# shibiaowan/SHARP

Measured on AMD Instinct MI355X. Metric: cells/sec end-to-end SHARP (fixed genes, n.RP); ARI vs reference labels, higher is better.
Workload: dtype f64

## Files before the change

include/sharp_hip.h:

```cpp
#ifndef SHARP_HIP_H
#define SHARP_HIP_H

#ifdef __cplusplus
extern "C" {
#endif

#define SHARP_OK 0
#define SHARP_ERR 1
#define SHARP_ERR_ARG 2
#define SHARP_ERR_NO_DEVICE 3
#define SHARP_WARN_RANGE 16
#define SHARP_WARN_NA_VOTE 32

const char *sharp_last_error(void);
int sharp_version(void);
int sharp_device_count(int *count);
int sharp_init(int device);
int sharp_shutdown(void);
int sharp_synchronize(void);
int sharp_reload_options(void);
int sharp_profile_enable(int on);
int sharp_profile_reset(void);
int sharp_profile_get(const char *name, double *total_ms, long long *launches);
int sharp_profile_dump(char *buf, int buflen);

int sharp_projector_create(int m, int p, int K, const double *seeds, int *handle);
int sharp_projector_destroy(int handle);
int sharp_projector_info(int handle, int *m, int *p, int *K, long long *nnz_total);
int sharp_projector_triplets(int handle, int k, int *gene, int *col, signed char *sign, long long *nnz);

int sharp_project(int proj, const double *X, int m, int n, long long ld, int log_flag, double *E);
int sharp_project_dev(int proj, const float *dX, int m, int n, long long ld, int log_flag,
                      double *dE, long long ldE);
int sharp_project_dev64(int proj, const double *dX, int m, int n, long long ld, int log_flag,
                        double *dE, long long ldE);

int sharp_get_opt_hclust(const double *mat, int n, int p, int hmethod, int N_cluster, int minN, int maxN,
                         double sil_thre, double height_Ntimes, int *f, int *v, double *msil, double *CHind,
                         double *maxsil, double *height, int *optN, int *nk, int *branch);

#define SHARP_DECISION_COLS 14
int sharp_decision_log(int enable);
int sharp_last_decisions(double *rows , int cap_rows, int *n_rows);

int sharp_getrowColor(const double *E, int n, int p, int hmethod, int indN_cluster, int minN, int maxN,
                      double sil_thre, double height_Ntimes, int *rowColor, double *maxsil);

int sharp_wMetaC(const int *nC, int N, int C, int hmethod, int enN_cluster, int minN, int maxN, double sil_thre,
                 double height_Ntimes, int *finalC, double *x0, int *ncl, double *w1_out, double *S_out, int *allC_out,
                 int *tf_out);

int sharp_sMetaC(const int *labels, const double *sE1, long long n, int p, int hmethod, int finalN_cluster, int minN,
                 int maxN, double sil_thre, double height_Ntimes, int *finalColor, int *tf_out, int *nC_out);

int sharp_SHARP_dev(const float *dX, int m, long long n, long long ld, int ensize_K, int reduced_ndim, int base_ncells,
                    int partition_ncells, int hmethod, int N_cluster, int enpN_cluster, int indN_cluster, int minN, int maxN,
                    double sil_thre, double height_Ntimes, int log_flag, int projector, double rN_seed, int *pred,
                    int *n_pred, double *viE, double *x0, int x0_cap_cols, int *x0_cols, int *p_used, int *K_used, int *path);
int sharp_SHARP_dev64(const double *dX, int m, long long n, long long ld, int ensize_K, int reduced_ndim, int base_ncells,
                      int partition_ncells, int hmethod, int N_cluster, int enpN_cluster, int indN_cluster, int minN, int maxN,
                      double sil_thre, double height_Ntimes, int log_flag, int projector, double rN_seed, int *pred,
                      int *n_pred, double *viE, double *x0, int x0_cap_cols, int *x0_cols, int *p_used, int *K_used, int *path);
int sharp_SHARP(const double *X, int m, long long n, long long ld, int ensize_K, int reduced_ndim, int base_ncells,
                int partition_ncells, int hmethod, int N_cluster, int enpN_cluster, int indN_cluster, int minN, int maxN,
                double sil_thre, double height_Ntimes, int log_flag, int projector, double rN_seed, int *pred,
                int *n_pred, double *viE, double *x0, int x0_cap_cols, int *x0_cols, int *p_used, int *K_used, int *path);

int sharp_x_storage(void);
int sharp_x_wire(void);

int sharp_last_rpinfo(int *n, int *K, int *p, int *enrp, double *indE);

int sharp_trim(void);

int sharp_csc_to_dense_dev(const int *colptr, const int *rowidx, const double *val, int m, long long n, float *dX, long long ld);
int sharp_csc_packed_expand_dev(const long long *d_colptr, const void *d_idx, int idx_bits, const void *d_val, int val_bits, int m,
                                long long n, void *dX, long long ld, int dx_is_f64);
int sharp_SHARP_csc(const int *colptr, const int *rowidx, const double *val, int m, long long n, int ensize_K, int reduced_ndim,
                    int base_ncells, int partition_ncells, int hmethod, int N_cluster, int enpN_cluster, int indN_cluster,
                    int minN, int maxN, double sil_thre, double height_Ntimes, int log_flag, int projector, double rN_seed,
                    int *pred, int *n_pred, double *viE, double *x0, int x0_cap_cols, int *x0_cols, int *p_used, int *K_used,
                    int *path);

int sharp_SHARP_unlimited_dev(const float *const *dX_blocks, const long long *ncb, const long long *ldb, int nblocks, int m,
// ... 181 lines not shown
int sharp_expr_stats_sub_csc(const int *const *colptr, const int *const *rowidx, const double *const *val, const long long *ncb, int nblocks,
                             int m, double normalize_total, int log1p, double *mean, double *var, long long *nnz, double *cell_sum,
                             const int *genes, int n_genes);
int sharp_expr_pca_transform_sub_csc(const int *const *colptr, const int *const *rowidx, const double *const *val, const long long *ncb,
                                     int nblocks, int m, double normalize_total, int log1p, const double *loadings, const double *center,
                                     const double *scale, int n_components, double *scores, const int *genes, int n_genes);
int sharp_expr_hvg_csc(const int *const *colptr, const int *const *rowidx, const double *const *val, const long long *ncb, int nblocks, int m,
                       int n_top_genes, double span, double *means, double *variances, double *variances_expected, double *variances_norm,
                       int *rank, int *highly_variable, int *genes, int *n_selected, int *q, int *degree_counts);
int sharp_hvg_loess(const double *x, const double *y, int npts, double span, double *fit, double *bandwidth, int *degree);

int sharp_harmony(const double *Z, long long n, int d, const int *batch, int n_batches, int n_clusters, double sigma, double theta, double lam,
                  int max_iter, int max_iter_cluster, int n_blocks, double epsilon_cluster, double epsilon_harmony, int init_iter, long long seed,
                  double *Z_corr, double *Y, double *objective, int *rounds, int *n_iter, int *converged, double *R);
int sharp_harmony_assign(const double *Zhat, const double *Y, const int *batch, const double *P, long long n, int d, int K, int B, long long i0,
                         long long i1, double sigma, int argmax, double *R, int *a);
int sharp_harmony_sums(const double *R, const double *X, const int *batch, long long n, int d, int K, int B, long long seed, int n_blocks, double *O,
                       double *S);
int sharp_harmony_correct(const double *Z, const double *R, const int *batch, const double *W, long long n, int d, int K, int B, double *Z_corr);
int sharp_harmony_ridge(const double *N, const double *S, int B, int K, int d, double lam, double *W);
int sharp_harmony_caps(int *slab, int *lds_tile);

int sharp_doublet_plan(long long n, double sim_doublet_ratio, int n_neighbors, long long *n_sim, int *n_neighbors_out, int *k_adj);
int sharp_doublet_pairs(long long n, long long n_sim, long long seed, long long *parents);
int sharp_doublet_synth_csc(const int *const *colptr, const int *const *rowidx, const double *const *val, const long long *ncb, int nblocks,
                            int m, const long long *parents, long long n_sim, int max_doublets_per_slab, long long capacity,
                            long long *colptr_out, int *rowidx_out, double *val_out, double *cell_sum_out);
int sharp_doublet_project_csc(const int *const *colptr, const int *const *rowidx, const double *const *val, const long long *ncb, int nblocks,
                              int m, const long long *parents, long long n_sim, double normalize_total, int log1p, const double *loadings,
                              const double *center, const double *scale, int n_components, const int *genes, int n_genes,
                              int max_doublets_per_slab, double *scores);
int sharp_doublet_neighbor_counts(const int *index, long long rows, int K, long long n_obs, int *counts);
int sharp_doublet_score_table(int k_adj, double r, double expected_doublet_rate, double *table);
int sharp_doublet_threshold(const double *scores_obs, long long n, const double *scores_sim, long long n_sim, double threshold_in,
                            double *threshold, int *found, int *predicted, double *rates, int *passes);
int sharp_scrublet_csc(const int *const *colptr, const int *const *rowidx, const double *const *val, const long long *ncb, int nblocks, int m,
                       double sim_doublet_ratio, double expected_doublet_rate, int n_neighbors, int n_prin_comps, int n_top_genes,
                       const int *genes, int n_genes, const double *fit_scores, const double *fit_loadings, const double *fit_center,
                       const double *fit_scale, double normalize_total, int log1p, int scale, double threshold, int nn_method,
                       const double *nn_args, long long seed, int max_doublets_per_slab, double *doublet_scores, double *doublet_scores_sim,
                       int *predicted, double *threshold_out, int *threshold_found, double *rates, int *n_neighbors_out, int *k_adj_out,
                       long long *parents, int *genes_out, int *n_genes_out, int *neighbor_counts, double *sim_pca);

int sharp_synth_fill_dev(unsigned seed, int m, long long cell0, int ncell, int G, int nmark,
                         float *dX, long long ld);
int sharp_synth_labels(unsigned seed, long long cell0, int ncell, int G, int *labels);

int sharp_gemm_tn_f64(const double *At, const double *Bt, double *C, int M, int N, int K, int epilogue, int symmetric, int fast);

int sharp_gemm_tn_f64_batch(int count, const int *M, const int *N, const int *K, const double *At, const double *Bt, int epilogue,
                            int symmetric, int fast, int nn_square, int want_nn, int polite, int ldc_pad, double *C, double *nn);
int sharp_row_prep_batch(int count, const int *n, const int *p, const long long *lds, const int *mode, const double *src,
                         int all_feature_rows, double *Cr, double *Ct, double *nrm, double *D);

int sharp_get_opt_hclust_batch(int count, const int *n, const int *p, const int *kind, const int *hmethod, const int *N_cluster,
                               const int *minN, const int *maxN, const double *sil_thre, const double *height_Ntimes, const double *mats,
                               int want_v, int nested, int *f, int *v, double *msil, double *CHind, double *height, int *optN, int *nk,
                               int *branch, int *rc, int *sequential);
int sharp_hclust_batch_plan(int *rows, int cap_rows, int *n_rows);

int sharp_wMetaC_batch(int count, const int *N, const int *C, const int *hmethod, const int *enN_cluster, const int *minN, const int *maxN,
                       const double *sil_thre, const double *height_Ntimes, const int *labels, const long long *cap, int *rc, int *allC,
                       int *ncl, int *finalC, double *w1, double *S, int *tf, double *x0);
int sharp_cluster_means(const double *E, long long ld, int n, int p, const int *uid, int nC, double *means, long long cap);
int sharp_ensemble_mean(const double *E, long long ldE, int n, int p, int K, double *viE, long long cap);

int sharp_dev_alloc(long long bytes, void **dptr);
int sharp_dev_free(void *dptr);
int sharp_dev_upload(void *dptr, const void *host, long long bytes);
int sharp_dev_download(void *host, const void *dptr, long long bytes);

void sharp_C_init(int *device, int *status);
void sharp_C_shutdown(int *status);
void sharp_C_trim(int *status);
void sharp_C_reload_options(int *status);
void sharp_C_device_count(int *count, int *status);
void sharp_C_last_error(char **msg, int *len);
void sharp_C_projector_create(int *m, int *p, int *K, double *seeds, int *handle, int *status);
void sharp_C_projector_destroy(int *handle, int *status);
void sharp_C_projector_triplets(int *handle, int *k, int *gene, int *col, int *sign, double *nnz, int *status);
void sharp_C_project(int *proj, double *X, int *m, int *n, int *log_flag, double *E, int *status);
void sharp_C_get_opt_hclust(double *mat, int *n, int *p, int *hmethod, int *N_cluster, int *minN, int *maxN, double *sil_thre,
                            double *height_Ntimes, int *flashmark, int *f, int *v, double *msil, double *CHind, double *maxsil,
                            double *height, int *optN, int *nk, int *branch, int *want, int *status);
void sharp_C_getrowColor(double *E, int *n, int *p, int *hmethod, int *indN_cluster, int *minN, int *maxN, double *sil_thre,
                         double *height_Ntimes, int *flashmark, int *rowColor, double *maxsil, int *status);
void sharp_C_wMetaC(int *nC, int *N, int *C, int *hmethod, int *enN_cluster, int *minN, int *maxN, double *sil_thre,
                    double *height_Ntimes, int *finalC, double *x0, int *ncl, int *want, int *status);
void sharp_C_sMetaC(int *labels, double *sE1, double *n, int *p, int *hmethod, int *finalN_cluster, int *minN, int *maxN,
                    double *sil_thre, double *height_Ntimes, int *finalColor, int *tf, int *nC, int *status);
void sharp_C_SHARP(double *X, int *m, double *n, int *ensize_K, int *reduced_ndim, int *base_ncells, int *partition_ncells, int *hmethod,
                   int *N_cluster, int *enpN_cluster, int *indN_cluster, int *minN, int *maxN, double *sil_thre, double *height_Ntimes,
                   int *flashmark, int *log_flag, int *projector, double *rN_seed, int *pred, double *viE, double *x0, int *x0_cap_cols,
                   int *info, int *want, int *status);
void sharp_C_SHARP_csc(int *colptr, int *rowidx, double *val, int *m, double *n, int *ensize_K, int *reduced_ndim, int *base_ncells,
                       int *partition_ncells, int *hmethod, int *N_cluster, int *enpN_cluster, int *indN_cluster, int *minN, int *maxN,
                       double *sil_thre, double *height_Ntimes, int *flashmark, int *log_flag, int *projector, double *rN_seed, int *pred,
                       double *viE, double *x0, int *x0_cap_cols, int *info, int *want, int *status);
void sharp_C_last_rpinfo(int *dims, int *enrp, double *indE, int *want, int *status);
void sharp_C_SHARP_unlimited(double *Xcat, int *nblocks, double *ncb, int *m, int *ensize_K, int *N_cluster, int *minN, int *maxN,
                             double *rN_seed, int *pred, double *viE, int *info, int *want, int *status);
void sharp_C_unlimited_view_dim(int *kdim, int *status);
void sharp_C_decision_log(int *enable, int *status);
void sharp_C_last_decisions(double *rows, int *cap_rows, int *n_rows, int *status);
void sharp_C_SHARP_unlimited_multi(double *Xcat, int *nblocks, double *ncb, int *m, int *ensize_K, int *N_cluster, int *minN, int *maxN,
                                   double *rN_seed, int *devices, int *ndevices, int *pred, double *viE, int *info, int *want, int *status);
// ... 103 lines not shown
```

sharp_amd/_abi.py:

```python
import ctypes as C

RETURN = {"i": C.c_int, "v": None, "s": C.c_char_p}
ARGUMENT = {"i": C.c_int, "u": C.c_uint, "l": C.c_longlong, "d": C.c_double, "p": C.c_void_p}

SIGNATURES = {
    "sharp_last_error": "s:",
    "sharp_version": "i:",
    "sharp_device_count": "i:p",
    "sharp_init": "i:i",
    "sharp_shutdown": "i:",
    "sharp_synchronize": "i:",
    "sharp_reload_options": "i:",
    "sharp_profile_enable": "i:i",
    "sharp_profile_reset": "i:",
    "sharp_profile_get": "i:ppp",
    "sharp_profile_dump": "i:pi",
    "sharp_projector_create": "i:iiipp",
    "sharp_projector_destroy": "i:i",
    "sharp_projector_info": "i:ipppp",
    "sharp_projector_triplets": "i:iipppp",
    "sharp_project": "i:ipiilip",
    "sharp_project_dev": "i:ipiilipl",
    "sharp_project_dev64": "i:ipiilipl",
    "sharp_get_opt_hclust": "i:piiiiiiddppppppppp",
    "sharp_decision_log": "i:i",
    "sharp_last_decisions": "i:pip",
    "sharp_getrowColor": "i:piiiiiiddpp",
    "sharp_wMetaC": "i:piiiiiiddppppppp",
    "sharp_sMetaC": "i:ppliiiiiddppp",
    "sharp_SHARP_dev": "i:pilliiiiiiiiiiddiidppppipppp",
    "sharp_SHARP_dev64": "i:pilliiiiiiiiiiddiidppppipppp",
    "sharp_SHARP": "i:pilliiiiiiiiiiddiidppppipppp",
    "sharp_x_storage": "i:",
    "sharp_x_wire": "i:",
    "sharp_last_rpinfo": "i:ppppp",
    "sharp_trim": "i:",
    "sharp_csc_to_dense_dev": "i:pppilpl",
    "sharp_csc_packed_expand_dev": "i:ppipiilpli",
    "sharp_SHARP_csc": "i:pppiliiiiiiiiiiddiidppppipppp",
    "sharp_SHARP_unlimited_dev": "i:pppiiiiiidppp",
    "sharp_SHARP_unlimited": "i:ppiiiiiidppp",
    "sharp_SHARP_unlimited_multi": "i:ppiiiiiidpipppp",
    "sharp_SHARP_unlimited_csc": "i:ppppiiiiiidpppp",
    "sharp_SHARP_unlimited_csc_multi": "i:ppppiiiiiidpipppp",
    "sharp_SHARP_unlimited_multi_dev": "i:pppppiiiiiidpipppp",
    "sharp_multi_timeline": "i:pip",
    "sharp_SHARP_unlimited_view": "i:ppiiiiiidpppp",
    "sharp_SHARP_unlimited_view_dev": "i:pppiiiiiidpppp",
    "sharp_unlimited_view_dim": "i:i",
    "sharp_SHARP_unlimited_viewk_dev": "i:pppiiiiiidpppip",
    "sharp_unlimited_block_dev": "i:pilliiidpppip",
    "sharp_unlimited_block_dev64": "i:pilliiidpppip",
    "sharp_unlimited_blocks_dev": "i:ppppiiiiidpppip",
    "sharp_SHARP_unlimited2": "i:ppiiiiiiiiiiiddidpppp",
    "sharp_SHARP_unlimited2_dev": "i:pppiiiiiiiiiiiddidpppp",
    "sharp_unlimited_block_view_dev": "i:pilliiidipppipp",
    "sharp_unlimited_block_viewk_dev": "i:pilliiidipppipidp",
    "sharp_unlimited_block_viewk_dev64": "i:pilliiidipppipidp",
    "sharp_unlimited_merge": "i:ppiiliiipp",
    "sharp_unlimited_next_block_dev": "i:pll",
    "sharp_marker_genes": "i:pillpidip",
    "sharp_marker_genes_dev": "i:pillpidip",
    "sharp_marker_genes_blocks_dev": "i:pppiipidip",
    "sharp_marker_genes_blocks_csc": "i:ppppiipidip",
    "sharp_tsne": "i:pliliiiiiiiddiiiddddpdppp",
    "sharp_tsne_prepare": "i:pliliiiiipp",
    "sharp_tsne_knn": "i:plilipp",
    "sharp_tsne_affinities": "i:plildlpppp",
    "sharp_tsne_gradient": "i:ppplipp",
    "sharp_tsne_bh": "i:pliliiiiiiiddiiiddddpdppp",
    "sharp_tsne_gradient_bh": "i:ppplipdpp",
    "sharp_tsne_neighbors": "i:ppliiiiddiiiddddpdppp",
    "sharp_tsne_dist": "i:piiiddiiiddddpdppp",
    "sharp_tsne_knn_dist": "i:piipp",
# ... 14 lines not shown
    "sharp_umap_transform": "i:ipllididdlppp",
    "sharp_knn_cross": "i:iplliipp",
    "sharp_umap_transform_weights": "i:ipplippp",
    "sharp_umap_transform_epochs": "i:ipplipiiididdl",
    "sharp_dist": "i:piilidp",
    "sharp_hclust_dist": "i:piippp",
    "sharp_hclust": "i:piilidippp",
    "sharp_cutree": "i:pipip",
    "sharp_silhouette_dist": "i:pipipp",
    "sharp_silhouette": "i:plilidpipp",
    "sharp_calinski_harabasz": "i:plilpiip",
    "sharp_neighbor_ranks": "i:plilipip",
    "sharp_louvain_graph": "i:ppplddiiidpipppppp",
    "sharp_louvain_neighbors": "i:ppliiddiiidpipppppp",
    "sharp_louvain_quantise": "i:ppplppp",
    "sharp_louvain_move": "i:ppplpddiip",
    "sharp_louvain_modularity": "i:pppplpdp",
    "sharp_louvain_aggregate": "i:ppplppppppp",
    "sharp_louvain_row_caps": "i:pp",
    "sharp_snn_graph": "i:plidlppppp",
    "sharp_snn_row_caps": "i:pp",
    "sharp_louvain_snn": "i:plidddiiidpipppppp",
    "sharp_expr_pca_csc": "i:ppppiiiiidiilpppppppp",
    "sharp_expr_stats_csc": "i:ppppiidipppp",
    "sharp_expr_pca_transform_csc": "i:ppppiidipppip",
    "sharp_expr_spmm_cells": "i:ppppiidiipip",
    "sharp_expr_spmm_genes": "i:ppppiidiipip",
    "sharp_expr_orth": "i:plip",
    "sharp_expr_row_caps": "i:pp",
    "sharp_expr_pca_sub_csc": "i:ppppiiiiidiilpppppppppi",
    "sharp_expr_stats_sub_csc": "i:ppppiidipppppi",
    "sharp_expr_pca_transform_sub_csc": "i:ppppiidipppippi",
    "sharp_expr_hvg_csc": "i:ppppiiidpppppppppp",
    "sharp_hvg_loess": "i:ppidppp",
    "sharp_harmony": "i:plipiidddiiiddilppppppp",
    "sharp_harmony_assign": "i:ppppliiilldipp",
    "sharp_harmony_sums": "i:pppliiilipp",
    "sharp_harmony_correct": "i:ppppliiip",
    "sharp_harmony_ridge": "i:ppiiidp",
    "sharp_harmony_caps": "i:pp",
    "sharp_doublet_plan": "i:ldippp",
    "sharp_doublet_pairs": "i:lllp",
    "sharp_doublet_synth_csc": "i:ppppiiplilpppp",
    "sharp_doublet_project_csc": "i:ppppiipldipppipiip",
    "sharp_doublet_neighbor_counts": "i:plilp",
    "sharp_doublet_score_table": "i:iddp",
    "sharp_doublet_threshold": "i:plpldppppp",
    "sharp_scrublet_csc": "i:ppppiiddiiipippppdiidiplippppppppppppp",
    "sharp_synth_fill_dev": "i:uiliiipl",
    "sharp_synth_labels": "i:uliip",
    "sharp_gemm_tn_f64": "i:pppiiiiii",
    "sharp_gemm_tn_f64_batch": "i:ipppppiiiiiiipp",
    "sharp_row_prep_batch": "i:ipppppipppp",
    "sharp_get_opt_hclust_batch": "i:ippppppppppiipppppppppp",
    "sharp_hclust_batch_plan": "i:pip",
    "sharp_wMetaC_batch": "i:ipppppppppppppppppp",
    "sharp_cluster_means": "i:pliipipl",
    "sharp_ensemble_mean": "i:pliiipl",
    "sharp_dev_alloc": "i:lp",
    "sharp_dev_free": "i:p",
    "sharp_dev_upload": "i:ppl",
    "sharp_dev_download": "i:ppl",
    "sharp_C_init": "v:pp",
    "sharp_C_shutdown": "v:p",
    "sharp_C_trim": "v:p",
    "sharp_C_reload_options": "v:p",
    "sharp_C_device_count": "v:pp",
    "sharp_C_last_error": "v:pp",
    "sharp_C_projector_create": "v:pppppp",
    "sharp_C_projector_destroy": "v:pp",
    "sharp_C_projector_triplets": "v:ppppppp",
    "sharp_C_project": "v:ppppppp",
    "sharp_C_get_opt_hclust": "v:ppppppppppppppppppppp",
    "sharp_C_getrowColor": "v:ppppppppppppp",
    "sharp_C_wMetaC": "v:pppppppppppppp",
    "sharp_C_sMetaC": "v:pppppppppppppp",
    "sharp_C_SHARP": "v:pppppppppppppppppppppppppp",
    "sharp_C_SHARP_csc": "v:pppppppppppppppppppppppppppp",
    "sharp_C_last_rpinfo": "v:ppppp",
    "sharp_C_SHARP_unlimited": "v:pppppppppppppp",
    "sharp_C_unlimited_view_dim": "v:pp",
    "sharp_C_decision_log": "v:pp",
    "sharp_C_last_decisions": "v:pppp",
    "sharp_C_SHARP_unlimited_multi": "v:pppppppppppppppp",
    "sharp_C_SHARP_unlimited_csc": "v:pppppppppppppppppp",
    "sharp_C_SHARP_unlimited2": "v:pppppppppppppppppppppp",
    "sharp_C_unlimited_merge": "v:ppppppppppp",
    "sharp_C_marker_genes": "v:ppppppppp",
    "sharp_C_tsne": "v:pppppppppppppppppppppppppp",
    "sharp_C_tsne_neighbors": "v:ppppppppppppppppppppppp",
    "sharp_C_tsne_dist": "v:pppppppppppppppppppp",
    "sharp_C_tsne_knn": "v:ppppppp",
    "sharp_C_knn_descent": "v:ppppppppppppp",
    "sharp_C_tsne_bh": "v:pppppppppppppppppppppppppp",
    "sharp_C_umap": "v:pppppppppppppppppppppp",
    "sharp_C_umap_neighbors": "v:pppppppppppppppppp",
    "sharp_C_umap_ab": "v:ppppp",
    "sharp_C_umap_model_create": "v:ppppppppppp",
    "sharp_C_umap_model_free": "v:pp",
    "sharp_C_umap_transform": "v:ppppppppppppppp",
    "sharp_C_umap_components": "v:pppppp",
    "sharp_C_umap_spectral": "v:pppppppppppppp",
    "sharp_C_umap_init_info": "v:pppppp",
    "sharp_C_dist": "v:ppppppp",
    "sharp_C_hclust_dist": "v:ppppppp",
    "sharp_C_hclust": "v:pppppppppp",
# ... 20 lines not shown
```

sharp_amd/csrc/common.hpp:

```cpp
#pragma once
#include <hip/hip_runtime.h>
#include <functional>

#include <cstdint>
#include <cstdio>
#include <map>
#include <stdexcept>
#include <string>
#include <vector>

#include "../../include/sharp_hip.h"

namespace sharp {

struct Error : std::runtime_error {
    int code;
    Error(int c, const std::string &m) : std::runtime_error(m), code(c) {}
};

void set_error(const std::string &msg);

#define SHARP_HIP_CHECK(expr)                                                                   \
    do {                                                                                        \
        hipError_t _e = (expr);                                                                 \
// ... 8 lines not shown
    } while (0)

#define SHARP_API_BEGIN try {
#define SHARP_API_END                                        \
    }                                                        \
    catch (const sharp::Error &e) {                          \
        sharp::set_error(e.what());                          \
        return e.code;                                       \
    }                                                        \
    catch (const std::exception &e) {                        \
        sharp::set_error(e.what());                          \
        return SHARP_ERR;                                    \
    }                                                        \
    return SHARP_OK;
inline int api_guarded(const std::function<void()> &step) {
    SHARP_API_BEGIN
    step();
    SHARP_API_END
}

struct XRef {
    const void *p = nullptr;
    bool f64 = false;
    int log_fix_bits = 44;
    XRef() = default;
    XRef(const float *q) : p(q), f64(false) {}
    XRef(const double *q) : p(q), f64(true) {}
    const float *f32() const { return static_cast<const float *>(p); }
    const double *d64() const { return static_cast<const double *>(p); }
};

struct Knobs {
    bool rp_dual = true;
    int rp_two_streams = -1;
    int rp_ahead = 2;
    int rp_chunk = 0;
    int rp_cp_wgs = 8;
    int rp_ap_wgs = 4;
    int rp_kernel = 0;
    int rp_pc_wgs = 2;
    int rp_pc_shape = 0;
    int x_storage = 0;
    bool block_prefetch = true;
    bool unlimited_batch = true;
    int unlimited_window_mb = 0;
    int ml_min_levels = 0;
    bool hc_mono = false, hc_seq = false;
    int hc_split = -1;
    int hc_ranges = 0, hc_wpt = 0, hc_finish_at = 15, hc_chunk = 0;
    int tail_threads = 4;
    bool tail_priority = true;
    bool dist_i8 = false;
    bool stats_sums = true;
    bool stats_lane = true;
    bool hc_tri = false;
    bool hc_prep_early = true;
    bool hc_pipe = true;
    bool mean_early = false;
    int gemm_slice = 8;
    bool proj_host = false;
    int hc_front = 0;
    bool hc_nn_gemm = true;
    bool hc_half = false;
    int host_threads = 0;
    int upload_threads = 0;
    std::vector<int> devices;
    int front_overlap = 0;
    int hc_first_chunk = 0;
    int host_group = 1;
    bool decision_log = false;
    bool free_later = true;
    bool step_marks = false;
    int rp_shape = 0;
};
const Knobs &knobs();
void reload_knobs();
void step_mark(const char *label, int id = -1);
void step_marks_dump();
#ifdef SHARP_LAB
inline const char *lab_env(const char *name) { return getenv(name); }
#endif

struct KernelStat {
    double ms = 0;
    long long launches = 0;
};

struct Ctx {
    bool ready = false;
    int device = -1;
    hipStream_t stream = nullptr;
    hipStream_t main_stream = nullptr;
    int rp_wgs_cap = 0;
    bool polite = false;
    hipStream_t stream2 = nullptr;
    std::vector<hipStream_t> aux;
    hipStream_t aux_stream(int i);
    int num_cu = 256;
    size_t lds_per_block = 65536;
    bool profiling = false;
    std::map<std::string, KernelStat> stats;
    struct Pending { hipEvent_t a, b; std::string name; hipStream_t st; };
    std::vector<Pending> pending;
    std::vector<hipEvent_t> event_pool;
    hipEvent_t get_event();
    void resolve_pending();
// ... 117 lines not shown
```

sharp_amd/csrc/driver.hip:

```cpp
#include <algorithm>
#include <cmath>
#include <cstring>
#include <numeric>
#include <random>
#include <thread>
#include <condition_variable>
#include <future>
#include <mutex>
#include <vector>

#include "driver.hpp"
#include "meta.hpp"
#include "projector.hpp"
#include "rrng.hpp"
#include "upload.hpp"

namespace sharp {

struct SharpOut {
    std::vector<int> pred;
    int n_pred = 0;
    struct View {
        double *p = nullptr;
        const double *staged = nullptr;
        hipEvent_t staged_done = nullptr;
        void download(double *h, size_t count) const {
            if (staged) {
                SHARP_HIP_CHECK(hipEventSynchronize(staged_done));
                const size_t piece = (count + 15) / 16;
                const double *src = staged;
                host_parallel_for(16, 16, [&](int t) {
                    const size_t lo = std::min(count, piece * static_cast<size_t>(t)), hi = std::min(count, lo + piece);
                    if (hi > lo) memcpy(h + lo, src + lo, (hi - lo) * sizeof(double));
                });
                return;
            }
            SHARP_HIP_CHECK(hipMemcpyAsync(h, p, count * sizeof(double), hipMemcpyDeviceToHost, ctx().stream));
            SHARP_HIP_CHECK(hipStreamSynchronize(ctx().stream));
        }
    } viE;
    std::vector<double> x0;
    int x0_cols = 0;
    int p = 0, K = 0, path = 0, rc = 0;
};

namespace {

struct DriverWs {
    DevBuf<double> E, Eb, viE_sh, viE_out;
    DevBuf<int> pos, posb;
    hipEvent_t mean_go = nullptr, mean_done = nullptr;
    hipStream_t mean_stream = nullptr;
    DevBuf<double> Ebatch;
    DevBuf<int> posbatch;
    DevBuf<double> fold_means, block_means;
    double *view_pinned = nullptr;
    size_t view_pinned_n = 0;
    hipEvent_t view_done = nullptr;
    std::vector<hipEvent_t> front_ev;
};
DriverWs &dws() { return per_slot<DriverWs>(); }

struct LastSmall { bool valid = false; int n = 0, K = 0, p = 0; long long ldE = 0; std::vector<int> enrp; };
LastSmall &last_small() { return per_slot<LastSmall>(); }

void merge_small(std::vector<int> &lab) {
    int mx = 0;
    for (int v : lab) mx = std::max(mx, v);
    std::vector<long long> cnt(mx + 1, 0);
    for (int v : lab) ++cnt[v];
    int mn = -1;
    for (int q = 1; q <= mx; ++q) if (cnt[q] > 0 && cnt[q] < 10) { mn = q; break; }
    if (mn >= 0) for (int &v : lab) if (cnt[v] < 10) v = mn;
}
int relabel_first(std::vector<int> &lab) {
    int mx = 0;
    for (int v : lab) mx = std::max(mx, v);
    std::vector<int> map(mx + 1, 0);
    int k = 0;
    for (int &v : lab) { if (!map[v]) map[v] = ++k; v = map[v]; }
    return k;
}

std::shared_ptr<Projector> projector_for(const SharpArgs &a, int m, int p, int K, const std::function<void()> *after_draw = nullptr) {
    if (a.projector) {
        auto pr = get_projector(a.projector);
        SHARP_REQUIRE(pr->m == m && pr->p == p && pr->K >= K, "rM does not match the data (genes, reduced.ndim, ensize.K)");
        return pr;
    }
    std::vector<double> seeds(K);
    for (int k = 0; k < K; ++k) seeds[k] = (a.rN_seed == 0.5) ? 0.5 : 50 + a.rN_seed + (k + 1);
    return build_projector(m, p, K, seeds.data(), after_draw);
}

__host__ __device__ inline double r_round1(double x) {
    if (!(x == x) || x == 0.0 || x - x != 0.0) return x;
    const double sgn = x < 0.0 ? -1.0 : 1.0;
    x = x < 0.0 ? -x : x;
    if (x >= 1e14) return sgn * x;
    const double x10 = 10.0 * x, i10 = floor(x10), xd = i10 / 10.0, xu = ceil(x10) / 10.0;
    const double du = xu - x, dd = x - xd;
    return sgn * ((dd < du || (dd == du && fmod(i10, 2.0) == 0.0)) ? xd : xu);
}
__global__ void round1_kernel(double *__restrict__ E, long long count) {
    for (long long q = blockIdx.x * static_cast<long long>(blockDim.x) + threadIdx.x; q < count; q += static_cast<long long>(gridDim.x) * blockDim.x)
        E[q] = r_round1(E[q]);
}
// ... 13 lines not shown
void sharp_small_dev(XRef dX, int m, int n, long long ld, const SharpArgs &a, int K, int p, HcParams base, SharpOut &out) {
    last_small().valid = false;
    auto pr = projector_for(a, m, p, K);
    const long long ldE = static_cast<long long>(pr->K) * p;
    DevBuf<double> &E = dws().E;
    E.ensure(static_cast<size_t>(n) * ldE);
    project_dev(*pr, dX, m, n, ld, a.flag, E.p, ldE, nullptr);
    std::vector<HcTask> tasks(K);
    HcParams bp = base; bp.N_cluster = a.indN;
    for (int k = 0; k < K; ++k) {
        tasks[k].d_mat = E.p + static_cast<long long>(k) * p; tasks[k].ld = ldE; tasks[k].n = n; tasks[k].p = p; tasks[k].prm = bp;
        tasks[k].prm.dec_level = 0; tasks[k].prm.dec_k = k;
    }
    std::vector<HcResult> hr;
    get_opt_hclust_batch(tasks, false, hr);
    std::vector<int> enrp(static_cast<size_t>(n) * K);
    for (int k = 0; k < K; ++k) { out.rc |= hr[k].rc; for (int i = 0; i < n; ++i) enrp[static_cast<size_t>(k) * n + i] = colour_of(hr[k].f[i]); }
    { LastSmall &L = last_small(); L.n = n; L.K = K; L.p = p; L.ldE = ldE; L.enrp = enrp; }
    WmTask wt; wt.nC = enrp.data(); wt.N = n; wt.C = K; wt.prm = base; wt.prm.N_cluster = a.N_cluster;
    wt.prm.dec_level = 1;
    std::vector<WmTask> wts{wt};
    std::vector<WmResult> wr;
    wmetac_batch(wts, a.want_x0, false, wr);
    out.rc |= wr[0].rc;
    out.pred = wr[0].finalC;
    if (a.want_viE || true) { dws().viE_out.ensure(static_cast<size_t>(n) * p); out.viE.p = dws().viE_out.p; ensemble_mean_dev(E.p, ldE, n, p, K, out.viE.p); }
    if (a.N_cluster <= 0 && n > 10000) merge_small(out.pred);
    out.n_pred = relabel_first(out.pred);
    if (a.want_x0) { out.x0 = wr[0].x0; out.x0_cols = wr[0].ncl; }
    stream_sync();
    last_small().valid = true;
}

static std::vector<int> fold_starts(int n, int ng) {
    const int T = (n + ng - 1) / ng;
    std::vector<int> st(T + 1, 0);
    if (T == 1) { st[1] = n; return st; }
    for (int t = 0; t < T - 2; ++t) st[t + 1] = (t + 1) * ng;
    const int nt = n - (T - 2) * ng;
    st[T - 1] = (T - 2) * ng + std::min(nt / 2, ng);
    st[T] = n;
    return st;
}

struct LargeFront {
    XRef dX; int m = 0, n = 0; long long ld = 0; int K = 0, p = 0, ng = 0, flag = 0, projector = 0; double rN_seed = 0; bool fpart = false;
    HcParams bp;
    bool shuffle = false;
    std::vector<int> reind, fst, pos;
    int T = 0;
    std::shared_ptr<Projector> pr;
    long long ldE = 0;
    double *E = nullptr; int *dpos = nullptr;
    std::vector<HcTask> tasks;
    std::shared_ptr<HcPrefetch> hc;
    bool matches(XRef X, int m_, int n_, long long ld_, int K_, int p_, int ng_, const SharpArgs &a, const HcParams &b) const {
        return dX.p == X.p && dX.f64 == X.f64 && m == m_ && n == n_ && ld == ld_ && K == K_ && p == p_ && ng == ng_ && flag == a.flag &&
               projector == a.projector && rN_seed == a.rN_seed && fpart == a.fpart && bp.hmethod == b.hmethod && bp.N_cluster == b.N_cluster &&
               bp.minN == b.minN && bp.maxN == b.maxN && bp.sil_thre == b.sil_thre && bp.height_Ntimes == b.height_Ntimes;
    }
};
namespace {
struct PendingFront { std::unique_ptr<LargeFront> f; hipStream_t stream = nullptr; hipEvent_t main_done = nullptr; int parity = 0;
                      unsigned long long born = 0, calls = 0; };
PendingFront &pending_front() { return per_slot<PendingFront>(); }
}

void drain_side_streams() {
    PendingFront &PF = pending_front();
    if (PF.stream) (void)hipStreamSynchronize(PF.stream);
    if (dws().mean_stream) (void)hipStreamSynchronize(dws().mean_stream);
}
void drop_pending_front() {
    PendingFront &PF = pending_front();
    if (PF.stream) (void)hipStreamSynchronize(PF.stream);
    PF.f.reset();
}

struct Shuffle { std::vector<int> reind, pos; };
static Shuffle make_shuffle(int n, bool random_seed) {
    Shuffle S;
    RRng rng(random_seed ? static_cast<uint32_t>(std::random_device{}()) : 50u);
    S.reind = rng.permutation(n);
    S.pos.assign(n, 0);
    for (int i = 0; i < n; ++i) S.pos[S.reind[i] - 1] = i;
    return S;
}
namespace {
struct ShuffleAhead { int n = 0; std::future<Shuffle> fut; };
ShuffleAhead &shuffle_ahead_slot() { return per_slot<ShuffleAhead>(); }
}
void shuffle_ahead(long long n, double rN_seed) {
    ShuffleAhead &H = shuffle_ahead_slot();
    H.n = 0; H.fut = std::future<Shuffle>();
    if (n >= 100000 || n < 5000 || rN_seed == 0.5) return;
    H.n = static_cast<int>(n);
    H.fut = std::async(std::launch::async, make_shuffle, static_cast<int>(n), false);
}

static void large_front(LargeFront &F, const SharpArgs &a, bool ahead, double *E_into = nullptr, int *pos_into = nullptr,
                        const Shuffle *same_size = nullptr) {
    const int n = F.n, m = F.m, K = F.K, p = F.p;
    F.shuffle = n < 100000;
    std::vector<int> &pos = F.pos;
    std::future<Shuffle> shuf;
    if (F.shuffle) {
        ShuffleAhead &H = shuffle_ahead_slot();
        if (same_size && a.rN_seed != 0.5 && static_cast<int>(same_size->pos.size()) == n) { F.reind = same_size->reind; pos = same_size->pos; }
        else if (H.n == n && H.fut.valid() && a.rN_seed != 0.5) { shuf = std::move(H.fut); H.n = 0; }
        else shuf = std::async(std::launch::async, make_shuffle, n, a.rN_seed == 0.5);
    } else pos.assign(n, 0);
    F.fst = fold_starts(n, F.ng);
    F.T = static_cast<int>(F.fst.size()) - 1;
    unsigned ahead_tok = 0u;
    const bool may_go_ahead = !a.projector && !ahead && knobs().rp_ahead > 0;
    const std::function<void()> start_compaction = [&] { if (may_go_ahead && !ahead_tok) ahead_tok = rp_compact_ahead(F.dX, m, n, F.ld, a.flag); };
    if (knobs().rp_ahead >= 2) start_compaction();
    { HostTimer ht("projector_build"); F.pr = projector_for(a, m, p, K, &start_compaction); }
    F.ldE = static_cast<long long>(F.pr->K) * p;
    if (shuf.valid()) { Shuffle S = shuf.get(); F.reind = std::move(S.reind); pos = std::move(S.pos); }
    if (E_into) {
        F.E = E_into; F.dpos = F.shuffle ? pos_into : nullptr;
        if (F.shuffle) SHARP_HIP_CHECK(hipMemcpyAsync(pos_into, pos.data(), static_cast<size_t>(n) * sizeof(int), hipMemcpyHostToDevice, ctx().stream));
    } else {
        DevBuf<double> &E = ahead ? dws().Eb : dws().E;
        { HostTimer ht("alloc_E"); E.ensure(static_cast<size_t>(n) * F.ldE); }
        DevBuf<int> &dpos = ahead ? dws().posb : dws().pos;
        if (F.shuffle) { dpos.ensure(n); dpos.upload(pos.data(), n); }
        F.E = E.p; F.dpos = F.shuffle ? dpos.p : nullptr;
    }
    project_dev(*F.pr, F.dX, m, n, F.ld, a.flag, F.E, F.ldE, F.dpos, ahead_tok);
    if (a.fpart) {
        Ctx &c = ctx();
        hipLaunchKernelGGL(round1_kernel, dim3(c.num_cu * 8), dim3(256), 0, c.stream, F.E, static_cast<long long>(n) * F.ldE);
        launch_check("round1_kernel");
    }
    F.tasks.assign(static_cast<size_t>(K) * F.T, HcTask());
    for (int k = 0; k < K; ++k)
        for (int t = 0; t < F.T; ++t) {
            HcTask &tk = F.tasks[static_cast<size_t>(k) * F.T + t];
            tk.d_mat = F.E + static_cast<long long>(F.fst[t]) * F.ldE + static_cast<long long>(k) * p;
            tk.ld = F.ldE; tk.n = F.fst[t + 1] - F.fst[t]; tk.p = p; tk.prm = F.bp;
            tk.prm.dec_level = 0; tk.prm.dec_k = k; tk.prm.dec_fold = t;
        }
}

static void enqueue_ensemble_mean(const double *E, long long ldE, int n, int p, int K, double *viE_sh, hipEvent_t after) {
    Ctx &c = ctx();
    hipEvent_t &mean_done = dws().mean_done;
    hipStream_t &ms = dws().mean_stream;
    if (!mean_done) {
        SHARP_HIP_CHECK(hipEventCreateWithFlags(&mean_done, hipEventDisableTiming));
        SHARP_HIP_CHECK(hipEventCreateWithFlags(&dws().mean_go, hipEventDisableTiming));
        int lo = 0, hi = 0;
        SHARP_HIP_CHECK(hipDeviceGetStreamPriorityRange(&lo, &hi));
        SHARP_HIP_CHECK(hipStreamCreateWithPriority(&ms, hipStreamNonBlocking, hi));
    }
    SHARP_HIP_CHECK(hipEventRecord(dws().mean_go, c.stream));
    SHARP_HIP_CHECK(hipStreamWaitEvent(ms, dws().mean_go, 0));
    if (after) SHARP_HIP_CHECK(hipStreamWaitEvent(ms, after, 0));
    {
        StreamScope scope(ms);
        ensemble_mean_dev(E, ldE, n, p, K, viE_sh);
    }
    SHARP_HIP_CHECK(hipEventRecord(mean_done, ms));
}

static void large_tail(const LargeFront &F, const SharpArgs &a, int K, int p, const HcParams &base, const HcResult *hr, SharpOut &out) {
    const int n = F.n, T = F.T;
    const bool shuffle = F.shuffle;
    const std::vector<int> &reind = F.reind, &fst = F.fst;
    const long long ldE = F.ldE;
    struct { double *p; } E{F.E};
    struct { int *p; } dpos{F.dpos};
    DevBuf<double> &viE_sh = dws().viE_sh;
    viE_sh.ensure(static_cast<size_t>(n) * p);
    hipEvent_t &mean_done = dws().mean_done;
    if (!hc_after_last_agglomeration_fired()) enqueue_ensemble_mean(E.p, ldE, n, p, K, viE_sh.p, nullptr);
    bool view_sent = false;
    if (a.view_to_host && !a.fpart) {
        DriverWs &W = dws();
        const size_t cnt = static_cast<size_t>(n) * p;
        if (W.view_pinned_n < cnt) {
            if (W.view_pinned) (void)hipHostFree(W.view_pinned);
            W.view_pinned = nullptr; W.view_pinned_n = 0;
            SHARP_HIP_CHECK(hipHostMalloc(reinterpret_cast<void **>(&W.view_pinned), cnt * sizeof(double), hipHostMallocDefault));
            W.view_pinned_n = cnt;
        }
        if (!W.view_done) SHARP_HIP_CHECK(hipEventCreateWithFlags(&W.view_done, hipEventDisableTiming));
        W.viE_out.ensure(cnt);
        {
            StreamScope scope(W.mean_stream);
            if (shuffle) {
                hipLaunchKernelGGL(gather_rows_kernel, dim3(ctx().num_cu * 8), dim3(256), 0, W.mean_stream, viE_sh.p, dpos.p, static_cast<long long>(n), p, W.viE_out.p);
                launch_check("gather_rows_kernel");
            } else {
                SHARP_HIP_CHECK(hipMemcpyAsync(W.viE_out.p, viE_sh.p, cnt * 8, hipMemcpyDeviceToDevice, W.mean_stream));
            }
            SHARP_HIP_CHECK(hipMemcpyAsync(W.view_pinned, W.viE_out.p, cnt * 8, hipMemcpyDeviceToHost, W.mean_stream));
        }
        SHARP_HIP_CHECK(hipEventRecord(W.view_done, W.mean_stream));
        out.viE.p = W.viE_out.p; out.viE.staged = W.view_pinned; out.viE.staged_done = W.view_done;
        view_sent = true;
    }
    std::vector<std::vector<int>> enrp(T);
    for (int q = 0; q < K * T; ++q) out.rc |= hr[q].rc;
    {
    HostTimer ht("tail_enrp");
    host_parallel_for(T, 16, [&](int t) {
        const int nt = fst[t + 1] - fst[t];
        enrp[t].resize(static_cast<size_t>(nt) * K);
        for (int k = 0; k < K; ++k) {
            const HcResult &r = hr[static_cast<size_t>(k) * T + t];
            for (int i = 0; i < nt; ++i) enrp[t][static_cast<size_t>(k) * nt + i] = colour_of(r.f[i]);
        }
    });
    }
    std::vector<WmTask> wts(T);
    for (int t = 0; t < T; ++t) {
        wts[t].nC = enrp[t].data(); wts[t].N = fst[t + 1] - fst[t]; wts[t].C = K;
        wts[t].prm = base; wts[t].prm.N_cluster = a.enpN;
        wts[t].prm.dec_level = 1; wts[t].prm.dec_fold = t;
    }
    std::vector<WmResult> wr;
    { HostTimer ht("wmetac_total"); wmetac_batch(wts, a.want_x0, false, wr); }
    step_mark("  tail: per-fold wMetaC done, folds", T);
    SHARP_HIP_CHECK(hipStreamWaitEvent(ctx().stream, mean_done, 0));
    std::vector<int> Slab(n);
    std::vector<int> stf;
    std::vector<int> uid(n);
    int nCu = 0;
// ... 49 lines not shown
        out.x0.assign(static_cast<size_t>(n) * sn, 0.0);
        out.x0_cols = sn;
        for (int t = 0; t < T; ++t) {
            const int nt = fst[t + 1] - fst[t], ncl = wr[t].ncl;
            for (int q = 0; q < ncl; ++q) {
                const int dstc = stf[col0[t] + q] - 1;
                for (int i = 0; i < nt; ++i) {
                    const int cell = shuffle ? reind[fst[t] + i] - 1 : fst[t] + i;
                    out.x0[static_cast<size_t>(dstc) * n + cell] += wr[t].x0[static_cast<size_t>(q) * nt + i];
                }
            }
        }
    }
    if (!view_sent) {
        dws().viE_out.ensure(static_cast<size_t>(n) * p); out.viE.p = dws().viE_out.p;
        if (shuffle) {
            Ctx &c = ctx();
            hipLaunchKernelGGL(gather_rows_kernel, dim3(c.num_cu * 8), dim3(256), 0, c.stream, viE_sh.p, dpos.p, static_cast<long long>(n), p, out.viE.p);
            launch_check("gather_rows_kernel");
        } else {
            SHARP_HIP_CHECK(hipMemcpyAsync(out.viE.p, viE_sh.p, static_cast<size_t>(n) * p * 8, hipMemcpyDeviceToDevice, ctx().stream));
        }
    }
    if (a.N_cluster <= 0 && n > 10000) merge_small(out.pred);
    out.n_pred = relabel_first(out.pred);
    stream_sync();
}

static void sharp_large_dev_body(XRef dX, int m, int n, long long ld, const SharpArgs &a, int K, int p, int ng, HcParams base, SharpOut &out);
void sharp_large_dev(XRef dX, int m, int n, long long ld, const SharpArgs &a, int K, int p, int ng, HcParams base, SharpOut &out) {
    try {
        sharp_large_dev_body(dX, m, n, ld, a, K, p, ng, base, out);
    } catch (...) {
        drop_pending_front();
        rp_compact_ahead_drop();
        if (ctx_unchecked().stream2) (void)hipStreamSynchronize(ctx_unchecked().stream2);
        if (ctx_unchecked().stream) (void)hipStreamSynchronize(ctx_unchecked().stream);
        throw;
    }
}
static void sharp_large_dev_body(XRef dX, int m, int n, long long ld, const SharpArgs &a, int K, int p, int ng, HcParams base, SharpOut &out) {
    HostTimer ht_all("sharp_large_total");
    last_small().valid = false;
    HcParams bp = base; bp.N_cluster = a.indN;
    if (a.fpart) bp.maxN = 40;
    std::unique_ptr<LargeFront> Fp;
    PendingFront &PF = pending_front();
    const unsigned long long call_no = ++PF.calls;
    if (PF.f) {
        if (PF.born + 1 == call_no && PF.f->matches(dX, m, n, ld, K, p, ng, a, bp)) {
            Fp = std::move(PF.f);
            std::swap(dws().E, dws().Eb);
            std::swap(dws().pos, dws().posb);
        } else {
            SHARP_HIP_CHECK(hipStreamSynchronize(PF.stream));
            PF.f.reset();
        }
    }
    if (!Fp) {
        Fp.reset(new LargeFront);
        Fp->dX = dX; Fp->m = m; Fp->n = n; Fp->ld = ld; Fp->K = K; Fp->p = p; Fp->ng = ng; Fp->flag = a.flag; Fp->projector = a.projector;
        Fp->rN_seed = a.rN_seed; Fp->fpart = a.fpart; Fp->bp = bp;
        large_front(*Fp, a, false);
    }
    LargeFront &F = *Fp;
    hipEvent_t after_agglo = nullptr;
    if (F.hc && a.next_dX.p) { HostTimer ht("base_clustering_total"); after_agglo = hc_prefetch_agglomerate(*F.hc); }
    if (a.next_dX.p && a.projector && knobs().block_prefetch) {
        const int nn = static_cast<int>(a.next_n);
        const int Tn = (nn + ng - 1) / ng;
        if (a.next_n >= 5000 && a.next_n < (1LL << 31) && static_cast<long long>(K) * Tn <= ctx().num_cu && Tn > 1) {
            std::unique_ptr<LargeFront> N(new LargeFront);
            N->dX = a.next_dX; N->m = m; N->n = nn; N->ld = a.next_ld; N->K = K; N->p = p; N->ng = ng; N->flag = a.flag;
            N->projector = a.projector; N->rN_seed = a.rN_seed; N->fpart = a.fpart; N->bp = bp;
            if (a.maxN <= 0 && !a.fpart) N->bp.maxN = std::max(40, (nn + 4999) / 5000);
            try {
            if (!PF.stream) {
                int lo = 0, hi = 0;
                SHARP_HIP_CHECK(hipDeviceGetStreamPriorityRange(&lo, &hi));
                SHARP_HIP_CHECK(hipStreamCreateWithPriority(&PF.stream, hipStreamNonBlocking, lo));
            }
            {
                if (!F.hc) {
                    if (!PF.main_done) SHARP_HIP_CHECK(hipEventCreateWithFlags(&PF.main_done, hipEventDisableTiming));
                    SHARP_HIP_CHECK(hipEventRecord(PF.main_done, ctx().stream));
                    SHARP_HIP_CHECK(hipStreamWaitEvent(PF.stream, PF.main_done, 0));
                }
                StreamScope scope(PF.stream);
                struct Polite { Polite() { ctx().polite = true; } ~Polite() { ctx_unchecked().polite = false; } } polite;
                if (after_agglo) SHARP_HIP_CHECK(hipStreamWaitEvent(PF.stream, after_agglo, 0));
                large_front(*N, a, true);
                if (hc_prefetch_possible(N->tasks)) N->hc = hc_prefetch_begin(N->tasks, PF.parity ^= 1);
            }
            if (N->hc) { PF.f = std::move(N); PF.born = call_no; }
            else SHARP_HIP_CHECK(hipStreamSynchronize(PF.stream));
            } catch (...) {
                if (PF.stream) (void)hipStreamSynchronize(PF.stream);
                (void)hipGetLastError();
                PF.f.reset();
            }
        }
    }
    std::vector<HcResult> hr;
    {
        HostTimer ht("base_clustering_total");
        if (F.hc) { hc_set_after_last_agglomeration(nullptr); hc_prefetch_stamp_block(*F.hc, a.block); hc_prefetch_finish(*F.hc, false, hr); }
        else {
            dws().viE_sh.ensure(static_cast<size_t>(n) * p);
            const double *Ep = F.E;
            const long long ldEp = F.ldE;
            double *vsh = dws().viE_sh.p;
            if (knobs().mean_early) hc_set_after_last_agglomeration([=](hipEvent_t ev) { enqueue_ensemble_mean(Ep, ldEp, n, p, K, vsh, ev); });
            else hc_set_after_last_agglomeration(nullptr);
            for (HcTask &tk : F.tasks) tk.prm.dec_block = a.block;
            try { get_opt_hclust_batch(F.tasks, false, hr); } catch (...) { hc_set_after_last_agglomeration(nullptr); throw; }
        }
    }
    large_tail(F, a, K, p, base, hr.data(), out);
    hc_set_after_last_agglomeration(nullptr);
}

void sharp_front_dev(XRef dX, int m, long long n_, long long ld, SharpArgs a, SharpOut &out) {
    SHARP_REQUIRE(dX.p, "No expression data is provided!");
    SHARP_REQUIRE(n_ >= 3 && n_ < (1LL << 31) && m >= 2, "SHARP: need at least 3 cells and 2 genes");
    const int n = static_cast<int>(n_);
    if (a.rN_seed != 0.5) SHARP_REQUIRE(std::fmod(a.rN_seed, 1.0) == 0.0, "The rN.seed should be an integer!");
    int p = a.reduced_ndim > 0 ? a.reduced_ndim : static_cast<int>(std::ceil(std::log2(static_cast<double>(n)) / (0.2 * 0.2)));
    int base_ncells = a.base_ncells > 0 ? a.base_ncells : 5000;
    int part = a.partition_ncells > 0 ? a.partition_ncells : 2000;
    HcParams base;
    base.hmethod = a.hmethod > 0 ? a.hmethod : 1;
    base.minN = a.minN > 0 ? a.minN : 2;
    base.maxN = a.maxN > 0 ? a.maxN : std::max(40, (n + 4999) / 5000);
    base.sil_thre = a.sil_thre >= 0 ? a.sil_thre : 0.35;
    base.height_Ntimes = a.height_Ntimes > 0 ? a.height_Ntimes : 2.0;
    base.dec_block = a.block;
    int K = a.K;
    if (a.N_cluster > 0 && n < base_ncells) {
        a.indN = a.N_cluster;
        base_ncells = (n + 1) / 2;
        part = (n + 1) / 2;
        if (K <= 0) K = 15;
    }
    if (a.fpart) {
        if (K <= 0) K = 5;
        SHARP_REQUIRE(part >= 3 && part <= kHcMaxN, "partition.ncells must be between 3 and 16384");
        out.path = 1;
        sharp_large_dev(dX, m, n, ld, a, K, p, part, base, out);
    } else if (n < base_ncells) {
        if (K <= 0) K = 15;
        SHARP_REQUIRE(n <= kHcMaxN, "SHARP_small: more than 16384 cells in one unpartitioned clustering task");
        out.path = 0;
        sharp_small_dev(dX, m, n, ld, a, K, p, base, out);
    } else {
        if (K <= 0) K = 5;
        SHARP_REQUIRE(part >= 3 && part <= kHcMaxN, "partition.ncells must be between 3 and 16384");
        out.path = 1;
        sharp_large_dev(dX, m, n, ld, a, K, p, part, base, out);
    }
    out.p = p; out.K = K;
}

struct ViewProj { std::shared_ptr<Projector> pr; int p = 0, kdim = 0; double seed = 0; DevBuf<double> out, pad; };

static void unlimited_block_summary(const SharpOut &o, long long nb, int p, BlockTable &t, double *viE_host, const ViewCall &view) {
// ... 90 lines not shown
            SHARP_HIP_CHECK(hipStreamSynchronize(ctx().stream));
            ctx().resolve_pending();
        } catch (...) {
            Ctx &hc = ctx_unchecked();
            if (hc.stream) (void)hipStreamSynchronize(hc.stream);
            if (hc.stream2) (void)hipStreamSynchronize(hc.stream2);
            try { drain_side_streams(); } catch (...) {}
            std::lock_guard<std::mutex> lk(mu);
            if (!err) err = std::current_exception();
        }
    }
    void may_run(int r) {
        { std::lock_guard<std::mutex> lk(mu); ready = r; }
        cv.notify_all();
    }
    void finish() {
        { std::lock_guard<std::mutex> lk(mu); stop = true; }
        cv.notify_all();
        for (std::thread &t : helpers) if (t.joinable()) t.join();
    }
    void join(std::exception_ptr window_err) {
        finish();
        if (prof) {
            for (int s : tslot) {
                bind_slot(s);
                std::map<std::string, KernelStat> ts;
                ts.swap(ctx_unchecked().stats);
                bind_slot(owner);
                for (const auto &kv : ts) { KernelStat &d = mc.stats[kv.first]; d.ms += kv.second.ms; d.launches += kv.second.launches; }
            }
        }
        if (window_err) std::rethrow_exception(window_err);
        if (err) std::rethrow_exception(err);
    }
};
}

void unlimited_batch_window(const XRef *dX, const long long *ncb, const long long *ldb, int b0, int b1, int m, int p, int proj, int K,
                            double rN_seed, double *const *viE_of, const ViewCall &view, BlockTable *tables, const int *gids) {
    FreeLater park_frees;
    PendingFront &PF = pending_front();
    hc_set_after_last_agglomeration(nullptr);
    if (PF.f) { SHARP_HIP_CHECK(hipStreamSynchronize(PF.stream)); PF.f.reset(); }
    const int nbk = b1 - b0;
    std::vector<std::unique_ptr<LargeFront>> F(nbk);
    std::vector<SharpArgs> A(nbk);
    std::vector<HcParams> base(nbk);
    long long rows = 0;
    for (int q = 0; q < nbk; ++q) rows += ncb[b0 + q];
    const long long ldE = static_cast<long long>(get_projector(proj)->K) * p;
    DriverWs &W = dws();
    W.Ebatch.ensure(static_cast<size_t>(rows) * ldE);
    W.posbatch.ensure(static_cast<size_t>(rows));
    last_small().valid = false;
    std::vector<HcTask> tasks;
    std::vector<size_t> first(nbk + 1, 0);
    std::vector<long long> row0(nbk + 1, 0);
#ifdef SHARP_LAB
    const int fo = knobs().front_overlap;
#else
    constexpr int fo = 0;
#endif
    for (int q = 0; q < nbk; ++q) {
        const int n = static_cast<int>(ncb[b0 + q]);
        SharpArgs &a = A[q];
        a.K = K; a.reduced_ndim = p; a.flag = 1; a.projector = proj; a.rN_seed = rN_seed; a.want_viE = true;
        HcParams &bs = base[q];
        bs.hmethod = 1; bs.minN = 2; bs.maxN = std::max(40, (n + 4999) / 5000); bs.sil_thre = 0.35; bs.height_Ntimes = 2.0;
        a.block = gids ? gids[b0 + q] : b0 + q; bs.dec_block = a.block;
        HcParams bp = bs; bp.N_cluster = a.indN;
        F[q].reset(new LargeFront);
        LargeFront &f = *F[q];
        f.dX = dX[b0 + q]; f.m = m; f.n = n; f.ld = ldb[b0 + q]; f.K = K; f.p = p; f.ng = 2000; f.flag = a.flag; f.projector = proj;
        f.rN_seed = rN_seed; f.fpart = false; f.bp = bp;
        row0[q + 1] = row0[q] + n;
    }
    int fronts_done = 0;
    Shuffle same_size;
    const auto front_of = [&](int q) {
        if (fo >= 2 && q >= 2) ctx().rp_wgs_cap = 1;
        large_front(*F[q], A[q], false, W.Ebatch.p + row0[q] * ldE, W.posbatch.p + row0[q], &same_size);
        ctx().rp_wgs_cap = 0;
        if (F[q]->shuffle && static_cast<int>(same_size.pos.size()) != F[q]->n) { same_size.reind = F[q]->reind; same_size.pos = F[q]->pos; }
    };
    std::function<hipEvent_t(size_t)> prepare;
    if (fo <= 0) {
        for (int q = 0; q < nbk; ++q) {
            front_of(q);
            tasks.insert(tasks.end(), F[q]->tasks.begin(), F[q]->tasks.end());
            first[q + 1] = tasks.size();
            for (size_t i = first[q]; i < first[q + 1]; ++i) tasks[i].prm.dec_block = A[q].block;
        }
        fronts_done = nbk;
    } else {
        for (int q = 0; q < nbk; ++q) {
            const LargeFront &f = *F[q];
            const std::vector<int> fst = fold_starts(f.n, f.ng);
            const int T = static_cast<int>(fst.size()) - 1;
            const double *E0 = W.Ebatch.p + row0[q] * ldE;
            for (int k = 0; k < K; ++k)
                for (int t = 0; t < T; ++t) {
                    HcTask tk;
                    tk.d_mat = E0 + static_cast<long long>(fst[t]) * ldE + static_cast<long long>(k) * p;
                    tk.ld = ldE; tk.n = fst[t + 1] - fst[t]; tk.p = p; tk.prm = f.bp;
                    tk.prm.dec_level = 0; tk.prm.dec_k = k; tk.prm.dec_fold = t; tk.prm.dec_block = A[q].block;
                    tasks.push_back(tk);
                }
            first[q + 1] = tasks.size();
        }
        prepare = [&](size_t upto) -> hipEvent_t {
            while (fronts_done < nbk && first[fronts_done] < upto) {
                const int q = fronts_done++;
                front_of(q);
                SHARP_REQUIRE(F[q]->tasks.size() == first[q + 1] - first[q] && F[q]->tasks[0].d_mat == tasks[first[q]].d_mat, "SHARP_unlimited: a block's tasks are not where its front put them");
                while (W.front_ev.size() <= static_cast<size_t>(q)) { hipEvent_t e; SHARP_HIP_CHECK(hipEventCreateWithFlags(&e, hipEventDisableTiming)); W.front_ev.push_back(e); }
                SHARP_HIP_CHECK(hipEventRecord(W.front_ev[q], ctx().stream));
            }
            return W.front_ev[fronts_done - 1];
        };
    }
    std::vector<HcResult> hr;
    const std::function<void(int)> tail_of = [&](int q) {
        SharpOut o;
        o.path = 1;
        step_mark("tail begins, block", b0 + q);
        large_tail(*F[q], A[q], K, p, base[q], hr.data() + first[q], o);
        o.p = p; o.K = K;
        step_mark("tail's labels ready, block", b0 + q);
        unlimited_block_summary(o, ncb[b0 + q], p, tables[q], viE_of ? viE_of[b0 + q] : nullptr, view);
        step_mark("tail delivered, block", b0 + q);
        F[q].reset();
    };
    std::unique_ptr<TailHelpers> helpers;
    if (knobs().tail_threads > 0 && nbk >= 2) helpers.reset(new TailHelpers(nbk, tail_of));
// ... 84 lines not shown
    return sharp_run_block(r, m, n, ld, ensize_K, reduced_ndim, base_ncells, partition_ncells, hmethod, N_cluster, enpN_cluster,
                           indN_cluster, minN, maxN, sil_thre, height_Ntimes, log_flag, projector, rN_seed, pred, n_pred, viE, x0,
                           x0_cap_cols, x0_cols, p_used, K_used, path);
}

int sharp_SHARP(const double *X, int m, long long n, long long ld, int ensize_K, int reduced_ndim, int base_ncells,
                int partition_ncells, int hmethod, int N_cluster, int enpN_cluster, int indN_cluster, int minN, int maxN,
                double sil_thre, double height_Ntimes, int log_flag, int projector, double rN_seed, int *pred, int *n_pred,
                double *viE, double *x0, int x0_cap_cols, int *x0_cols, int *p_used, int *K_used, int *path) {
    HostBlock &hb = host_block();
    const int rc = api_guarded([&] {
        ctx();
        if (!X || ld < m || n < 1) throw sharp::Error(SHARP_ERR_ARG, "No expression data is provided!");
        upload_block(X, m, n, ld, hb);
    });
    if (rc != SHARP_OK) return rc;
    return sharp_run_block(hb.ref(), m, n, hb.ld, ensize_K, reduced_ndim, base_ncells, partition_ncells, hmethod, N_cluster, enpN_cluster,
                           indN_cluster, minN, maxN, sil_thre, height_Ntimes, log_flag, projector, rN_seed, pred, n_pred, viE, x0,
                           x0_cap_cols, x0_cols, p_used, K_used, path);
}

int sharp_x_storage(void) { return upload_last_storage(); }
int sharp_x_wire(void) { return upload_last_wire(); }

int sharp_last_rpinfo(int *n, int *K, int *p, int *enrp, double *indE) {
    SHARP_API_BEGIN
    ctx();
    LastSmall &L = last_small();
    SHARP_REQUIRE(L.valid, "sharp_last_rpinfo: the last SHARP call did not take the SHARP_small path (allrpinfo exists there only, R/SHARP.R:446)");
    if (n) *n = L.n;
    if (K) *K = L.K;
    if (p) *p = L.p;
    if (enrp) std::copy(L.enrp.begin(), L.enrp.end(), enrp);
    if (indE) {
        const size_t w = static_cast<size_t>(L.K) * L.p * sizeof(double);
        SHARP_HIP_CHECK(hipMemcpy2DAsync(indE, w, dws().E.p, static_cast<size_t>(L.ldE) * sizeof(double), w, static_cast<size_t>(L.n),
                                         hipMemcpyDeviceToHost, ctx().stream));
        stream_sync();
    }
    SHARP_API_END
}

int sharp_trim(void) {
    SHARP_API_BEGIN
    ctx();
    for_each_ready_slot([] {
        SHARP_HIP_CHECK(hipDeviceSynchronize());
        drop_pending_front();
        host_block().release();
        { HostBlockPair &hp = per_slot<HostBlockPair>(); for (HostBlock &h : hp.hb) h.release(); }
        upload_release_staging();
        dws().Ebatch.release();
        dws().posbatch.release();
        if (dws().view_pinned) { (void)hipHostFree(dws().view_pinned); dws().view_pinned = nullptr; dws().view_pinned_n = 0; }
        rp_pc_trim();
        rp_trim();
        if (cur_slot() != 0) { hc_release_workspaces(); dws().E.release(); dws().Eb.release(); dws().viE_sh.release(); dws().viE_out.release(); }
    });
    pool_clear();
    SHARP_API_END
}

int sharp_csc_to_dense_dev(const int *colptr, const int *rowidx, const double *val, int m, long long n, float *dX, long long ld) {
    SHARP_API_BEGIN
    ctx();
    SHARP_REQUIRE(dX && ld >= m && m > 0 && n >= 0, "sharp_csc_to_dense_dev: bad block");
    upload_csc_into_f32(colptr, rowidx, val, m, n, dX, ld);
    SHARP_API_END
}

int sharp_csc_packed_expand_dev(const long long *d_colptr, const void *d_idx, int idx_bits, const void *d_val, int val_bits, int m,
                                long long n, void *dX, long long ld, int dx_is_f64) {
    SHARP_API_BEGIN
    ctx();
    SHARP_REQUIRE(d_colptr && dX && m > 0 && n >= 0 && ld >= m, "sharp_csc_packed_expand_dev: bad block");
    SHARP_REQUIRE((idx_bits == 16 && m <= 65536) || idx_bits == 32, "sharp_csc_packed_expand_dev: row indices of 16 (at most 65 536 genes) or 32 bits");
    SHARP_REQUIRE(val_bits == 8 || val_bits == 16 || val_bits == 32 || val_bits == 64, "sharp_csc_packed_expand_dev: values of 8 or 16 (unsigned integers), 32 (float) or 64 (double) bits");
    SHARP_REQUIRE(val_bits != 64 || dx_is_f64, "sharp_csc_packed_expand_dev: 64-bit values need an fp64 block");
    expand_packed_csc_dev(d_colptr, d_idx, idx_bits, d_val, val_bits, m, n, dX, ld, dx_is_f64 != 0);
    SHARP_API_END
}

int sharp_SHARP_csc(const int *colptr, const int *rowidx, const double *val, int m, long long n, int ensize_K, int reduced_ndim,
                    int base_ncells, int partition_ncells, int hmethod, int N_cluster, int enpN_cluster, int indN_cluster, int minN,
                    int maxN, double sil_thre, double height_Ntimes, int log_flag, int projector, double rN_seed, int *pred,
                    int *n_pred, double *viE, double *x0, int x0_cap_cols, int *x0_cols, int *p_used, int *K_used, int *path) {
    HostBlock &hb = host_block();
    const int rc = api_guarded([&] {
        ctx();
        if (m <= 0 || n <= 0) throw sharp::Error(SHARP_ERR_ARG, "No expression data is provided!");
        upload_block_csc(colptr, rowidx, val, m, n, hb);
    });
    if (rc != SHARP_OK) return rc;
    return sharp_run_block(hb.ref(), m, n, hb.ld, ensize_K, reduced_ndim, base_ncells, partition_ncells, hmethod, N_cluster, enpN_cluster,
                           indN_cluster, minN, maxN, sil_thre, height_Ntimes, log_flag, projector, rN_seed, pred, n_pred, viE, x0,
                           x0_cap_cols, x0_cols, p_used, K_used, path);
}

}
```

sharp_amd/csrc/hclust.hip:

```cpp
#include "hclust_task.hpp"

#include <algorithm>
#include <array>
#include <climits>
#include <cmath>
#include <cstring>
#include <limits>

#include "linalg.hpp"

namespace sharp {

namespace {

template <typename T>
struct PinnedBuf {
    T *p = nullptr;
    size_t n = 0;
    PinnedBuf() = default;
    PinnedBuf(const PinnedBuf &) = delete;
    PinnedBuf &operator=(const PinnedBuf &) = delete;
    ~PinnedBuf() { if (p) (void)hipHostFree(p); }
    void ensure(size_t count) {
        if (count <= n) return;
// ... 72 lines not shown
    bool mid_recorded = false;
    struct Range { int t0, t1; int off[5], cnt[5]; int off8 = 0; bool any_sym, any_feat; };
    std::vector<Range> ranges;
};
enum : int { PH_DIST = 1, PH_AGGLO = 2, PH_STATS = 4, PH_ALL = 7 };
struct PipeEvents {
    hipEvent_t in = nullptr, out[8] = {nullptr}, gemm[6] = {nullptr}, hc[6] = {nullptr}, done[6] = {nullptr}, prep[6] = {nullptr};
};
PipeEvents &pipe_events() {
    PipeEvents &e = per_slot<PipeEvents>();
    if (!e.in) {
        SHARP_HIP_CHECK(hipEventCreateWithFlags(&e.in, hipEventDisableTiming));
        for (auto &x : e.out) SHARP_HIP_CHECK(hipEventCreateWithFlags(&x, hipEventDisableTiming));
        for (int q = 0; q < 6; ++q) {
            SHARP_HIP_CHECK(hipEventCreateWithFlags(&e.gemm[q], hipEventDisableTiming));
            SHARP_HIP_CHECK(hipEventCreateWithFlags(&e.hc[q], hipEventDisableTiming));
            SHARP_HIP_CHECK(hipEventCreateWithFlags(&e.done[q], hipEventDisableTiming));
            SHARP_HIP_CHECK(hipEventCreateWithFlags(&e.prep[q], hipEventDisableTiming));
        }
    }
    return e;
}

struct BatchPlan { std::vector<std::array<int, kHcPlanCols>> rows; };
BatchPlan &batch_plan() { return per_slot<BatchPlan>(); }
void plan_add(ChunkJob &J, bool nested) {
    std::vector<std::array<int, kHcPlanCols>> &rows = batch_plan().rows;
    J.plan_row = static_cast<int>(rows.size());
    rows.push_back({static_cast<int>(J.i0), static_cast<int>(J.i1), J.slot, J.pipe, J.split, J.NS, J.ml, J.max_n, J.max_kpad, 0, 0,
                    J.max_n > HR_MAXN, nested, J.max_nk, 0, 0});
}

void setup_chunk(const std::vector<HcTask> &tasks, ChunkJob &J) {
    Ctx &c = ctx();
    Workspace &W = ws(J.slot);
    Workspace &W0 = ws(J.scratch_slot);
    PipeEvents &EV = pipe_events();
    const size_t i0 = J.i0;
    const int T = J.T = static_cast<int>(J.i1 - J.i0);
    std::vector<HcMeta> &metas = J.metas;
    metas.assign(T, HcMeta());
    hipStream_t chunk_stream = J.pipe ? c.aux_stream(J.slot) : c.stream;
    if (J.pipe) SHARP_HIP_CHECK(hipStreamWaitEvent(chunk_stream, J.input_ready ? J.input_ready : EV.in, 0));
    StreamScope chunk_scope(chunk_stream);
    long long oD = 0, oD0 = 0, oCr = 0, oCt = 0, oN = 0, oM = 0, oLab = 0, oK = 0, oCS = 0, oQ = 0, oOut = 0;
    int max_n = 0, max_p = 0, max_nk = 0, max_kpad = 0;
    for (int t = 0; t < T; ++t) {
        const HcTask &tk = tasks[i0 + t];
        HcMeta &M = metas[t];
        SHARP_REQUIRE(tk.n >= 3, "get_opt_hclust: need at least 3 observations");
        SHARP_REQUIRE(tk.n <= kHcMaxN, "get_opt_hclust: more than 16384 observations in one clustering task is not supported");
        SHARP_REQUIRE(tk.prm.hmethod >= 1 && tk.prm.hmethod <= 8, "get_opt_hclust: unknown agglomeration method");
        M.n = tk.n; M.p = tk.symmetric ? tk.n : tk.p; M.nld = static_cast<int>(rup(tk.n, 128));
        M.method = tk.prm.hmethod; M.symmetric = tk.symmetric ? (tk.distance ? 2 : 1) : 0; M.pad0 = 0;
        if (tk.prm.N_cluster > 0) {
            SHARP_REQUIRE(tk.prm.N_cluster >= 2, "The given N.cluster is less than 2, which is not suitable for clustering!");
            SHARP_REQUIRE(tk.prm.N_cluster <= tk.n - 1, "N.cluster must be smaller than the number of observations");
            M.kmin = M.kmax = tk.prm.N_cluster;
        } else {
            M.kmin = tk.prm.minN;
            M.kmax = std::min(tk.prm.maxN, tk.n - 1);
            SHARP_REQUIRE(M.kmin >= 2 && M.kmax >= M.kmin, "get_opt_hclust: empty range of cluster numbers (minN.cluster..maxN.cluster)");
        }
        M.nk = M.kmax - M.kmin + 1;
        M.kpad = static_cast<int>(rup(M.kmax, 16));
        M.oD = oD; oD += static_cast<long long>(M.nld) * M.nld;
        M.oD0 = oD0; if (M.symmetric == 1) oD0 += static_cast<long long>(M.nld) * M.nld;
        M.oCr = oCr; if (M.symmetric != 2) oCr += static_cast<long long>(M.n) * M.p;
        M.oCt = oCt; if (M.symmetric != 2) oCt += rup(M.p, 16) * M.nld;
        M.oNrm = oN; oN += M.n;
        M.oM = oM; oM += M.n;
        M.oLab = oLab; oLab += static_cast<long long>(M.nk) * M.n;
        M.oH = M.oT = M.oG = oK; oK += static_cast<long long>(M.nld) * M.kpad;
        M.oCSt = oCS; oCS += static_cast<long long>(M.p) * M.kpad;
        M.oQ = oQ; oQ += static_cast<long long>(M.kpad) * M.kpad;
        M.oOut = oOut; oOut += 2LL * M.nk;
        max_n = std::max(max_n, M.n); max_p = std::max(max_p, M.p); max_nk = std::max(max_nk, M.nk);
        max_kpad = std::max(max_kpad, M.kpad);
    }
    J.oOut = oOut; J.oM = oM; J.oLab = oLab; J.max_n = max_n; J.max_p = max_p; J.max_nk = max_nk; J.max_kpad = max_kpad;
    SHARP_REQUIRE(max_nk > ml_min_levels() ||
                  stats_lds_bytes(max_n, std::max(max_kpad, 64)) <= ST_LDS_MAX,
                  "get_opt_hclust: this many observations with this many candidate cluster numbers does not fit the silhouette kernel "
                  "(LDS: 8 B per observation rounded up to a power of two + 36 B per candidate cluster)");
    { HostTimer ht("hc_workspace_alloc");
    W.D.ensure(oD); W0.S0.ensure(oD); W0.S1.ensure(oD); W.D0.ensure(std::max<long long>(oD0, 1)); W.Cr.ensure(oCr); W.Ct.ensure(oCt); W.nrm.ensure(oN);
    W.height.ensure(oM); W.ia.ensure(oM); W.ib.ensure(oM); W.lab.ensure(oLab);
    W.H.ensure(oK); W.T.ensure(oK); W.G.ensure(oK); W.CSt.ensure(oCS); W.Q.ensure(oQ); W.out.ensure(oOut); }
    { HostTimer ht("hc_workspace_alloc");
    W.meta.ensure(T); W.prep.ensure(T); W.gemm.ensure(5 * static_cast<size_t>(T)); W.status.ensure(T); }
    {
        bool parts = knobs().hc_nn_gemm;
#ifdef SHARP_LAB
        if (knobs().dist_i8 && max_p <= 8192) parts = false;
#endif
        long long oNN = 0;
        if (parts) for (int t = 0; t < T; ++t) if (!metas[t].symmetric && metas[t].nld <= 2048) oNN += static_cast<long long>(metas[t].nld / 128) * metas[t].nld;
        if (oNN > 0) {
            W.nnp.ensure(oNN);
            oNN = 0;
            for (int t = 0; t < T; ++t) if (!metas[t].symmetric && metas[t].nld <= 2048) { metas[t].nn = W.nnp.p + oNN; oNN += static_cast<long long>(metas[t].nld / 128) * metas[t].nld; }
        }
    }
    W.meta.upload(metas.data(), T);

    int NS = T >= 194 ? 2 : 1;
    {
        const bool split = knobs().hc_split >= 0 ? knobs().hc_split == 1 : (T <= kHcSplitMaxTasks && max_n >= kHcSplitMinObs);
        J.split = split;
        if (!knobs().hc_seq && ((!knobs().hc_mono && split) || max_n > HR_MAXN)) NS = 1;
    }
    if (knobs().hc_ranges > 0) NS = std::max(1, std::min(8, knobs().hc_ranges));
    if (J.pipe || J.one_range) NS = 1;
    if (J.max_nk > ml_min_levels()) NS = 1;
    NS = std::min(NS, T);
    std::vector<RowPrepTask> &prep = J.prep;
    prep.assign(T, RowPrepTask());
    for (int t = 0; t < T; ++t) {
        const HcTask &tk = tasks[i0 + t];
        const HcMeta &M = metas[t];
        prep[t] = RowPrepTask{tk.d_mat, tk.ld, M.n, M.p, M.nld, static_cast<int>(rup(M.p, 16)), M.symmetric, W.Cr.p + M.oCr,
                              W.Ct.p + M.oCt, W.nrm.p + M.oNrm, W.D.p + M.oD};
    }
    W.prep.upload(prep.data(), T);
    typedef ChunkJob::Range Range;
    J.NS = NS;
    std::vector<Range> &ranges = J.ranges;
    ranges.assign(NS, Range());
    std::vector<GemmTask> &g = J.g;
    g.clear();
    g.reserve(5 * static_cast<size_t>(T));
    for (int s = 0; s < NS; ++s) {
        Range &R = ranges[s];
        R.t0 = static_cast<int>(static_cast<long long>(T) * s / NS);
        R.t1 = static_cast<int>(static_cast<long long>(T) * (s + 1) / NS);
        R.any_sym = R.any_feat = false;
        for (int kind = 0; kind < 5; ++kind) {
            R.off[kind] = static_cast<int>(g.size());
            for (int t = R.t0; t < R.t1; ++t) {
                const HcMeta &M = metas[t];
                R.any_sym |= M.symmetric != 0; R.any_feat |= M.symmetric == 0;
                switch (kind) {
                    case 0:
                        if (!M.symmetric) g.push_back(GemmTask{W.Ct.p + M.oCt, W.Ct.p + M.oCt, W.D.p + M.oD, M.n, M.n, M.p, M.nld, M.nld, M.nld, 1, 1, 1,
                                                               const_cast<double *>(M.nn), M.method == 8});
                        break;
                    case 1:
                        g.push_back(GemmTask{W.Cr.p + M.oCr, W.H.p + M.oH, W.CSt.p + M.oCSt, M.p, M.kpad, M.n, M.p, M.kpad, M.kpad, 0, 0, 0});
                        break;
                    case 2:
                        g.push_back(GemmTask{W.CSt.p + M.oCSt, W.Ct.p + M.oCt, W.G.p + M.oG, M.kpad, M.n, M.p, M.kpad, M.nld, M.nld, 0, 0, 0});
                        break;
                    case 3:
                        g.push_back(GemmTask{W.CSt.p + M.oCSt, W.CSt.p + M.oCSt, W.Q.p + M.oQ, M.kpad, M.kpad, M.p, M.kpad, M.kpad, M.kpad, 0, 0, 0});
                        break;
                    default:
                        if (M.symmetric == 1) g.push_back(GemmTask{W.H.p + M.oH, W.D0.p + M.oD0, W.T.p + M.oT, M.kpad, M.n, M.n, M.kpad, M.nld, M.nld, 0, 0, 0});
                        break;
                }
            }
            R.cnt[kind] = static_cast<int>(g.size()) - R.off[kind];
        }
    }
#ifdef SHARP_LAB
    J.i8 = knobs().dist_i8 && max_p <= 8192;
    if (J.i8) {
        std::vector<DistI8Task> d8;
        size_t oSl = 0, oSc = 0;
        for (int t = 0; t < T; ++t) if (!metas[t].symmetric) { oSl += dist_i8_slice_bytes(metas[t].nld, metas[t].p); oSc += metas[t].nld; }
        W.sl.ensure(std::max<size_t>(oSl, 1)); W.slscale.ensure(std::max<size_t>(oSc, 1));
        oSl = 0; oSc = 0;
        for (int s = 0; s < NS; ++s) {
            ranges[s].off8 = static_cast<int>(d8.size());
            for (int t = ranges[s].t0; t < ranges[s].t1; ++t) {
                const HcMeta &M = metas[t];
// ... 54 lines not shown
        hipStream_t st = NS > 1 ? c.aux_stream(s) : chunk_stream;
        StreamScope scope(st);
        const HcMeta *dmeta = W.meta.p + R.t0;
        const HcAggloRange agglo{dmeta, Ts, max_n, W.D.p, W0.S0.p, W0.S1.p, W.ia.p, W.ib.p, W.height.p, W.status.p + R.t0};
        auto launch_sequential = [&](bool fallback_only) {
            KernelTimer tm("hclust_sequential");
            unsigned char *gstate = nullptr;
            if (max_n > kHcLdsMaxN) {
                const size_t stride = hc_seq_state_bytes(max_n);
                W.seqstate.ensure(static_cast<size_t>(J.T) * stride);
                gstate = W.seqstate.p + static_cast<size_t>(R.t0) * stride;
            }
            hclust_sequential(agglo, fallback_only ? agglo.status : nullptr, gstate);
        };
        if (phases & PH_DIST) {
        if (NS > 1) SHARP_HIP_CHECK(hipStreamWaitEvent(st, ev_in, 0));
        if (J.pipe && !J.first) SHARP_HIP_CHECK(hipStreamWaitEvent(st, knobs().hc_prep_early ? EV.prep[J.prev_slot] : EV.gemm[J.prev_slot], 0));
        row_prep_batched(W.prep.p + R.t0, Ts, max_n, max_p, !R.any_sym);
        if (J.pipe) SHARP_HIP_CHECK(hipEventRecord(EV.prep[J.slot], st));
        if (J.pipe && !J.first) SHARP_HIP_CHECK(hipStreamWaitEvent(st, EV.gemm[J.prev_slot], 0));
#ifdef SHARP_LAB
        if (R.cnt[0] && J.i8) dist_i8_batched(W.i8.p + R.off8, R.cnt[0], max_n);
        else
#endif
        if (R.cnt[0]) gemm_tn_f64_batched(W.gemm.p + R.off[0], R.cnt[0], max_n, max_n, "corr_dist_gemm", true, true);
        if (J.pipe) SHARP_HIP_CHECK(hipEventRecord(EV.gemm[J.slot], st));
        if (R.any_sym) {
            KernelTimer tm("copy_d");
            hclust_copy_d(dmeta, Ts, W.D.p, W.D0.p);
        }
        }
        if (phases & PH_AGGLO) {
        if (J.pipe && !J.first) SHARP_HIP_CHECK(hipStreamWaitEvent(st, EV.hc[J.prev_slot], 0));
        {
            const bool use_rnn = !knobs().hc_seq;
            KernelTimer tm("hclust");
            HcAggloDid did;
            if (use_rnn && hclust_bulk_synchronous(agglo, J.split, W0.img, W0.remaining, J.mid_event, J.mid_round, &did)) J.mid_recorded = true;
            if (!use_rnn || !(J.pipe && J.has_next)) launch_sequential(use_rnn);
            else J.seq_pending = true;
            if (J.plan_row >= 0 && s == 0) {
                std::array<int, kHcPlanCols> &row = batch_plan().rows[J.plan_row];
                row[9] = J.seq_pending; row[10] = did.form; row[14] = did.wpt; row[15] = did.finish_at;
            }
        }
        if (J.pipe) SHARP_HIP_CHECK(hipEventRecord(EV.hc[J.slot], st));
        if (J.pipe && knobs().step_marks)
            SHARP_HIP_CHECK(hipLaunchHostFunc(st, [](void *) { step_mark("    (device) an agglomeration ends"); }, nullptr));
        }
        if (!(phases & PH_STATS)) continue;
        if (J.pipe && J.has_next) SHARP_HIP_CHECK(hipStreamWaitEvent(st, EV.gemm[J.next_slot], 0));
        if (J.pipe && J.next2_slot >= 0) SHARP_HIP_CHECK(hipStreamWaitEvent(st, EV.gemm[J.next2_slot], 0));
        if (J.seq_pending) { launch_sequential(true); J.seq_pending = false; }
        const HcStatsRange stats{dmeta, Ts, max_n, max_p, J.max_nk, max_kpad, R.any_sym, W.gemm.p, R.off, R.cnt, W.ia.p, W.ib.p, W.lab.p,
                                 W.H.p, W.Cr.p, W.CSt.p, W.T.p, W.G.p, W.Q.p, W.nrm.p, W.out.p};
        const HcManyLevels many{&J.metas, &J.mlmetas, W.mlmeta.p, J.oM, J.ml_off, J.ml_cnt, J.mlt_off, J.mlt_cnt, W.mlr1.p, W.mlr2.p, W.mlcntF.p,
                                W.mlcn2m.p, W.mlB.p, W.mlcn2F.p, W.mltot2.p, W.mlS.p};
        hclust_level_stats(stats, J.ml ? &many : nullptr);
        if (NS > 1) {
            SHARP_HIP_CHECK(hipEventRecord(ev_out[s], st));
            SHARP_HIP_CHECK(hipStreamWaitEvent(main_stream, ev_out[s], 0));
        }
    }
    if (J.pipe && (phases & PH_STATS)) SHARP_HIP_CHECK(hipEventRecord(EV.done[J.slot], chunk_stream));
    if (J.pipe && (phases & PH_STATS) && knobs().step_marks)
        SHARP_HIP_CHECK(hipLaunchHostFunc(chunk_stream, [](void *) { step_mark("    (device) a chunk's statistics end"); }, nullptr));
}

void finish_chunk(const std::vector<HcTask> &tasks, ChunkJob &J, bool want_v, std::vector<HcResult> &out, bool want_status) {
    Ctx &c = ctx();
    Workspace &W = ws(J.slot);
    const size_t i0 = J.i0;
    const int T = J.T;
    const long long oOut = J.oOut, oM = J.oM, oLab = J.oLab;
    const std::vector<HcMeta> &metas = J.metas;
    if (J.pipe) SHARP_HIP_CHECK(hipStreamWaitEvent(c.stream, pipe_events().done[J.slot], 0));
    W.h_out.ensure(std::max<long long>(oOut, 1)); W.h_height.ensure(std::max<long long>(oM, 1));
    double *h_out = W.h_out.p, *h_height = W.h_height.p;
    if (c.profiling || want_status) {
        std::vector<int> st(T, 1);
        if (!knobs().hc_seq) W.status.download(st.data(), T);
        int fallback = 0;
        for (int v : st) fallback += v != 0;
        if (c.profiling) {
            c.stats["host:hclust_tasks_bulk_synchronous"].launches += T - fallback;
            c.stats["host:hclust_tasks_sequential"].launches += fallback;
        }
        if (want_status) for (int t = 0; t < T; ++t) out[i0 + t].sequential = st[t] != 0;
    }
    HostTimer ht_tail("hc_download_select");
    W.out.download(h_out, oOut);
    W.height.download(h_height, oM);
    std::vector<int> chosen(T);
    std::vector<long long> poff(T);
    long long ptot = 0;
    for (int t = 0; t < T; ++t) { poff[t] = ptot; ptot += metas[t].n; }
    host_parallel_for(T, T >= 16 ? 16 : 1, [&](int t) {
        const HcTask &tk = tasks[i0 + t];
        const HcMeta &M = metas[t];
        HcResult &R = out[i0 + t];
        R.rc = 0; R.nk = M.nk;
        R.msil.assign(h_out + M.oOut, h_out + M.oOut + M.nk);
        R.CHind.assign(h_out + M.oOut + M.nk, h_out + M.oOut + 2 * M.nk);
        R.height.assign(h_height + M.oM, h_height + M.oM + M.n - 1);
        int oind = 1;
        if (tk.prm.N_cluster > 0) {
            R.branch = 0; R.maxsil = R.msil[0];
            R.CHind[0] = std::numeric_limits<double>::quiet_NaN();
// ... 446 lines not shown
```

sharp_amd/csrc/hclust_stats.hip:

```cpp
#include "hclust_task.hpp"

#include <algorithm>
#include <vector>

#include "linalg.hpp"

namespace sharp {

__global__ __launch_bounds__(HC_THREADS) void cutree_kernel(const HcMeta *__restrict__ metas, const int *__restrict__ ia_all,
                                                            const int *__restrict__ ib_all, int *__restrict__ lab_all) {
    const HcMeta M = metas[blockIdx.x];
    const int n = M.n;
    const int *ia = ia_all + M.oM, *ib = ib_all + M.oM;
    int *lab = lab_all + M.oLab;
    extern __shared__ __attribute__((aligned(16))) unsigned char sm[];
    unsigned char *lds_cursor = sm;
    CUTREE_ARRAYS(LDS_CARVE, n)
    const int tid = threadIdx.x;
    for (int i = tid; i < n; i += HC_THREADS) { absorbed[i] = 0x7fffffff; parent[i] = static_cast<uint16_t>(i); }
    __syncthreads();
    for (int s = tid; s < n - 1; s += HC_THREADS) { absorbed[ib[s] - 1] = s; parent[ib[s] - 1] = static_cast<uint16_t>(ia[s] - 1); }
    __syncthreads();
    const int chunk = (n + HC_THREADS - 1) / HC_THREADS;
    for (int L = 0; L < M.nk; ++L) {
        const int k = M.kmin + L;
        const int nm = n - k;
        const int b0 = tid * chunk, b1 = min(n, b0 + chunk);
        int local = 0;
        for (int i = b0; i < b1; ++i) local += (absorbed[i] >= nm);
        int inc = local;
        const int lane = tid & 63, w = tid >> 6;
#pragma unroll
        for (int o = 1; o < 64; o <<= 1) { const int t = __shfl_up(inc, o); if (lane >= o) inc += t; }
        if (lane == 63) wsum[w] = inc;
        __syncthreads();
        if (tid == 0) { int run = 0; for (int q = 0; q < HC_THREADS / 64; ++q) { const int t = wsum[q]; wsum[q] = run; run += t; } }
        __syncthreads();
        int run = wsum[w] + inc - local;
        for (int i = b0; i < b1; ++i) { if (absorbed[i] >= nm) rank[i] = static_cast<uint16_t>(++run); }
        __syncthreads();
        for (int i = tid; i < n; i += HC_THREADS) {
            int r = i;
            while (absorbed[r] < nm) r = parent[r];
            lab[static_cast<long long>(L) * n + i] = rank[r];
        }
        __syncthreads();
    }
}

__global__ void onehot_kernel(const HcMeta *__restrict__ metas, const int *__restrict__ lab_all, double *__restrict__ H_all) {
    const HcMeta M = metas[blockIdx.y];
    const int *lab = lab_all + M.oLab + static_cast<long long>(M.nk - 1) * M.n;
    double *H = H_all + M.oH;
    const long long tot = static_cast<long long>(M.n) * M.kpad;
    for (long long q = blockIdx.x * static_cast<long long>(blockDim.x) + threadIdx.x; q < tot;
         q += static_cast<long long>(gridDim.x) * blockDim.x) {
        const int i = static_cast<int>(q / M.kpad), c = static_cast<int>(q % M.kpad);
        H[q] = (lab[i] == c + 1) ? 1.0 : 0.0;
    }
}

__global__ __launch_bounds__(64 * SS_WAVES) void cluster_sums_kernel(const HcMeta *__restrict__ metas, const int *__restrict__ lab_all,
                                                                     const double *__restrict__ Cr_all, double *__restrict__ CSt_all) {
    const HcMeta M = metas[blockIdx.y];
    const int j0 = blockIdx.x * 64;
    if (j0 >= M.p) return;
    extern __shared__ __attribute__((aligned(16))) unsigned char ss_sm[];
    double *acc = reinterpret_cast<double *>(ss_sm);
    const int tid = threadIdx.x, lane = tid & 63;
    const int wave = __builtin_amdgcn_readfirstlane(tid >> 6);
    const int kpad = M.kpad, n = M.n, p = M.p;
    for (int q = tid; q < SS_WAVES * kpad * 64; q += 64 * SS_WAVES) acc[q] = 0.0;
    __syncthreads();
    const int *lab = lab_all + M.oLab + static_cast<long long>(M.nk - 1) * n;
    const double *Cr = Cr_all + M.oCr;
    const int j = j0 + lane;
    const bool live = j < p;
    double *mine = acc + static_cast<size_t>(wave) * kpad * 64 + lane;
    int i = wave;
    for (; i + 3 * SS_WAVES < n; i += 4 * SS_WAVES) {
        double x[4];
        int c[4];
#pragma unroll
        for (int u = 0; u < 4; ++u) {
            c[u] = __builtin_amdgcn_readfirstlane(lab[i + u * SS_WAVES]) - 1;
            x[u] = live ? Cr[static_cast<long long>(i + u * SS_WAVES) * p + j] : 0.0;
        }
#pragma unroll
        for (int u = 0; u < 4; ++u) mine[c[u] * 64] += x[u];
    }
    for (; i < n; i += SS_WAVES) {
        const int c = __builtin_amdgcn_readfirstlane(lab[i]) - 1;
        mine[c * 64] += live ? Cr[static_cast<long long>(i) * p + j] : 0.0;
    }
    __syncthreads();
    double *CSt = CSt_all + M.oCSt;
    for (int q = tid; q < kpad * 64; q += 64 * SS_WAVES) {
        const int c = q >> 6, l = q & 63;
        if (j0 + l >= p) continue;
        double v = acc[c * 64 + l];
#pragma unroll
        for (int w = 1; w < SS_WAVES; ++w) v += acc[(w * kpad + c) * 64 + l];
        CSt[static_cast<long long>(j0 + l) * kpad + c] = v;
    }
}

__global__ void copy_d_kernel(const HcMeta *__restrict__ metas, const double *__restrict__ Dall, double *__restrict__ D0all) {
    const HcMeta M = metas[blockIdx.y];
    if (M.symmetric != 1) return;
    const long long tot = static_cast<long long>(M.n) * M.nld;
    const double *D = Dall + M.oD;
    double *D0 = D0all + M.oD0;
    for (long long q = blockIdx.x * static_cast<long long>(blockDim.x) + threadIdx.x; q < tot;
         q += static_cast<long long>(gridDim.x) * blockDim.x)
        D0[q] = D[q];
}


__global__ __launch_bounds__(ST_THREADS) void stats_kernel(const HcMeta *__restrict__ metas, const int *__restrict__ lab_all,
                                                           const double *__restrict__ T_all, const double *__restrict__ G_all,
                                                           const double *__restrict__ Q_all, const double *__restrict__ nrm_all,
                                                           double *__restrict__ out_all, int count, int max_nk, int kcap) {
    const long long B = blockIdx.x;
    const long long per_group = 8LL * max_nk;
    const int zt = static_cast<int>(B / per_group) * 8 + static_cast<int>(B % 8);
    if (zt >= count) return;
    const HcMeta M = metas[zt];
    const int L = static_cast<int>((B % per_group) / 8);
    if (L >= M.nk) return;
    const int n = M.n, k = M.kmin + L, kf = M.kmax, kpad = M.kpad;
    const int *lab = lab_all + M.oLab + static_cast<long long>(L) * n;
    const int *labF = lab_all + M.oLab + static_cast<long long>(M.nk - 1) * n;
    const double *T = T_all + M.oT, *G = G_all + M.oG, *Q = Q_all + M.oQ, *nrm = nrm_all + M.oNrm;
    extern __shared__ __attribute__((aligned(16))) unsigned char sm[];
    int npow2 = 1; while (npow2 < n) npow2 <<= 1;
    double *sil = reinterpret_cast<double *>(sm);
    double *part = sil + npow2;
    double *cn2 = part + ST_THREADS;
    double *ctot = cn2 + kcap;
    int *cnt = reinterpret_cast<int *>(ctot + kcap);
    int *cntF = cnt + kcap;
    int *fm = cntF + kcap;
    int *start = fm + kcap;
    int *order = start + kcap + 1;
    const int tid = threadIdx.x;
    for (int c = tid; c < kcap; c += ST_THREADS) { cnt[c] = 0; cntF[c] = 0; }
    __syncthreads();
    for (int i = tid; i < n; i += ST_THREADS) {
        atomicAdd(&cnt[lab[i] - 1], 1);
        atomicAdd(&cntF[labF[i] - 1], 1);
// ... 318 lines not shown

void many_levels_stats(const HcStatsRange &r, const HcManyLevels &ml) {
    Ctx &c = ctx();
    hipStream_t st = c.stream;
    const int T = r.tasks, max_n = r.max_n, max_kpad = r.max_kpad;
    if (r.cnt[3]) gemm_tn_f64_batched(r.gemm + r.off[3], r.cnt[3], max_kpad, max_kpad, "cluster_gram_gemm");
    gemm_tn_f64_batched(r.gemm + ml.ml_off, ml.ml_cnt, max_n, max_kpad, "row_cluster_dot_gemm");
    if (ml.mlt_cnt) gemm_tn_f64_batched(r.gemm + ml.mlt_off, ml.mlt_cnt, max_n, max_kpad, "dist_cluster_sums_gemm");
    std::vector<int> h_ia(ml.oM), h_ib(ml.oM);
    SHARP_HIP_CHECK(hipMemcpyAsync(h_ia.data(), r.ia, ml.oM * sizeof(int), hipMemcpyDeviceToHost, st));
    SHARP_HIP_CHECK(hipMemcpyAsync(h_ib.data(), r.ib, ml.oM * sizeof(int), hipMemcpyDeviceToHost, st));
    SHARP_HIP_CHECK(hipStreamSynchronize(st));
    const std::vector<HcMeta> &metas = *ml.metas;
    const std::vector<MlMeta> &mlmetas = *ml.mlmetas;
    long long tot_levels = 0;
    for (int t = 0; t < T; ++t) tot_levels += metas[t].nk;
    std::vector<int> h_r1(tot_levels, 0), h_r2(tot_levels, 0);
    for (int t = 0; t < T; ++t) {
        const HcMeta &M = metas[t];
        const int *ia = h_ia.data() + M.oM, *ib = h_ib.data() + M.oM;
        std::vector<int> fin(M.n, 0);
        std::vector<char> absorbed(M.n, 0);
        for (int q = 0; q < M.n - M.kmax; ++q) absorbed[ib[q] - 1] = 1;
        int f = 0;
        for (int i = 0; i < M.n; ++i) if (!absorbed[i]) fin[i] = f++;
        for (int L = M.nk - 2; L >= 0; --L) {
            const int q = M.n - 1 - (M.kmin + L);
            h_r1[mlmetas[t].oMerge + L] = fin[ia[q] - 1];
            h_r2[mlmetas[t].oMerge + L] = fin[ib[q] - 1];
        }
    }
    SHARP_HIP_CHECK(hipMemcpyAsync(ml.r1, h_r1.data(), tot_levels * sizeof(int), hipMemcpyHostToDevice, st));
    SHARP_HIP_CHECK(hipMemcpyAsync(ml.r2, h_r2.data(), tot_levels * sizeof(int), hipMemcpyHostToDevice, st));
    KernelTimer tm("sil_ch_stats");
    const size_t lds_p = ml_prep_lds_bytes(max_kpad);
    allow_dynamic_lds(ml_prep_kernel, lds_p);
    hipLaunchKernelGGL(ml_prep_kernel, dim3(T), dim3(1024), lds_p, st, r.metas, ml.dml, r.lab, r.Q, ml.r1, ml.r2,
                       ml.cn2m, ml.B, ml.cntF, ml.cn2F, ml.tot2);
    launch_check("ml_prep_kernel");
    const size_t lds_c = ml_cells_lds_bytes(max_kpad);
    allow_dynamic_lds(ml_cells_kernel, lds_c);
    const size_t lds_l = ml_level_lds_bytes(max_n);
    allow_dynamic_lds(ml_level_kernel, lds_l);
    for (int t = 0; t < T; ++t) {
        const HcMeta &M = metas[t];
        const int blocks = std::min((M.n + ML_WAVES - 1) / ML_WAVES, c.num_cu * std::max(1, static_cast<int>(HR_LDS_CU / std::max<size_t>(lds_c, 1))));
        hipLaunchKernelGGL(ml_cells_kernel, dim3(blocks), dim3(64 * ML_WAVES), lds_c, st, r.metas, ml.dml, t, r.lab, r.T, r.G, r.nrm,
                           ml.r1, ml.r2, ml.cn2m, ml.cntF, ml.cn2F, ml.S);
        hipLaunchKernelGGL(ml_level_kernel, dim3(M.nk), dim3(ST_THREADS), lds_l, st, r.metas, ml.dml, t, ml.S, ml.B, r.out);
    }
    launch_check("ml_cells_kernel");
}

}

void hclust_level_stats(const HcStatsRange &r, const HcManyLevels *ml) {
    hipStream_t st = ctx().stream;
    const int Ts = r.tasks, max_n = r.max_n, max_p = r.max_p, max_nk = r.max_nk, max_kpad = r.max_kpad;
    {
        const size_t lds = cutree_lds_bytes(max_n);
        allow_dynamic_lds(cutree_kernel, lds);
        KernelTimer tm("cutree");
        hipLaunchKernelGGL(cutree_kernel, dim3(Ts), dim3(HC_THREADS), lds, st, r.metas, r.ia, r.ib, r.lab);
        launch_check("cutree_kernel");
    }
    const bool sums = knobs().stats_sums && !ml && max_kpad <= SS_KMAX;
    if (!sums || r.any_sym) {
        KernelTimer tm("onehot");
        hipLaunchKernelGGL(onehot_kernel, dim3(64, Ts), dim3(256), 0, st, r.metas, r.lab, r.H);
        launch_check("onehot_kernel");
    }
    if (sums) {
        KernelTimer tm("cluster_sums_gemm");
        const size_t lds = cluster_sums_lds_bytes(max_kpad);
        allow_dynamic_lds(cluster_sums_kernel, lds);
        hipLaunchKernelGGL(cluster_sums_kernel, dim3((max_p + 63) / 64, Ts), dim3(64 * SS_WAVES), lds, st, r.metas, r.lab, r.Cr, r.CSt);
        launch_check("cluster_sums_kernel");
    } else if (r.cnt[1]) gemm_tn_f64_batched(r.gemm + r.off[1], r.cnt[1], max_p, max_kpad, "cluster_sums_gemm");
    if (ml) { many_levels_stats(r, *ml); return; }
    if (r.cnt[2]) gemm_tn_f64_batched(r.gemm + r.off[2], r.cnt[2], max_kpad, max_n, "row_cluster_dot_gemm");
    if (r.cnt[3]) gemm_tn_f64_batched(r.gemm + r.off[3], r.cnt[3], max_kpad, max_kpad, "cluster_gram_gemm");
    if (r.cnt[4]) gemm_tn_f64_batched(r.gemm + r.off[4], r.cnt[4], max_kpad, max_n, "dist_cluster_sums_gemm");
    const int kcap = std::max(max_kpad, 64);
    const bool lane_form = knobs().stats_lane && max_kpad <= 64;
    const size_t lds = lane_form ? stats_lane_lds_bytes(max_n, kcap) : stats_lds_bytes(max_n, kcap);
    const auto kern = lane_form ? stats_lane_kernel : stats_kernel;
    allow_dynamic_lds(kern, lds);
    KernelTimer tm("sil_ch_stats");
    const long long blocks = static_cast<long long>((Ts + 7) / 8) * 8 * max_nk;
    hipLaunchKernelGGL(kern, dim3(static_cast<unsigned>(blocks)), dim3(ST_THREADS), lds, st, r.metas, r.lab, r.T,
                       r.G, r.Q, r.nrm, r.out, Ts, max_nk, kcap);
    launch_check("stats_kernel");
}

}
```

sharp_amd/csrc/hclust_task.hpp:

```cpp
#pragma once
#include <algorithm>

#include "hclust.hpp"

namespace sharp {

#define SHARP_HC_LOCAL __attribute__((visibility("hidden")))

struct HcMeta {
    int n, p, nld, kmin, kmax, nk, kpad, method;
    int symmetric, pad0;
    long long oD, oD0;
    long long oCr, oCt, oNrm;
    long long oM;
    long long oLab;
    long long oH, oT, oG;
    long long oCSt, oQ;
    long long oOut;
    const double *nn;
};
struct MlMeta {
    long long oS;
    long long oMerge;
    long long oFin;
};

constexpr int HC_THREADS = 512;
constexpr double HC_INF = 1.0e300;
constexpr int HR_MAXN = 4096;
constexpr size_t HR_LDS_CU = 160 * 1024;
constexpr int ST_THREADS = 512;
constexpr size_t ST_LDS_MAX = 160 * 1024;
constexpr int SS_WAVES = 2, SS_KMAX = 144;
constexpr int ML_WAVES = 3;

template <typename K>
static inline void allow_dynamic_lds(K kern, size_t bytes) {
    SHARP_HIP_CHECK(hipFuncSetAttribute(reinterpret_cast<const void *>(kern), hipFuncAttributeMaxDynamicSharedMemorySize, static_cast<int>(bytes)));
}

__host__ __device__ inline int hc_npow2(int n) { int p = 1; while (p < n) p <<= 1; return p; }

#define LDS_CARVE(type, name, count) \
    [[maybe_unused]] type *name = reinterpret_cast<type *>(lds_cursor); lds_cursor = reinterpret_cast<unsigned char *>(name + (count));
#define LDS_COUNT(type, name, count) lds_bytes += sizeof(type) * static_cast<size_t>(count);

#define HC_SEQ_STATE_ARRAYS(X, n, nal)                                                                                      \
    X(double, disnn, nal)                                                                                                   \
    X(double, pv, 32)                                                                                                       \
    X(int, nn, nal)                                                                                                         \
    X(int, membr, nal)                                                                                                      \
    X(int, list, nal)                                                                                                       \
    X(int, pi, 32)                                                                                                          \
    X(int, cnt, 2)                                                                                                          \
    X(unsigned char, flag, n)
#define HC_SEQ_SCRATCH_ARRAYS(X, n)                                                                                         \
    X(unsigned char, flag_pad, (((n) + 7) & ~7) - (n))                             \
    X(double, pvB, 32)                                                                                                      \
    X(int, piB, 32)
inline size_t hc_seq_state_bytes(int max_n) {
    const int nal = (max_n + 1) & ~1;
    size_t lds_bytes = 0;
    HC_SEQ_STATE_ARRAYS(LDS_COUNT, max_n, nal)
    HC_SEQ_SCRATCH_ARRAYS(LDS_COUNT, max_n)
    const size_t slack = 32 - (((max_n + 7) & ~7) - max_n);
    return (lds_bytes + slack + 15) / 16 * 16;
}

#define HR_STATE_ARRAYS(X, nal, nwave)                                                                                      \
    X(double, dnnA, 2 * (nal))                                          \
    X(uint16_t, cidA, 2 * (nal))                                                    \
    X(uint16_t, cszA, 2 * (nal))                                                                \
    X(uint16_t, nn, nal)                                                                                                    \
    X(uint16_t, partner, nal)                                                     \
    X(uint16_t, pseq, nal)                                                               \
    X(uint16_t, oldidx, nal)                                                                    \
    X(uint16_t, newidx, nal)                                                        \
    X(uint16_t, plist, nal)                                                                 \
    X(uint16_t, colmap, nal)           \
    X(int, ctl, 16)                             \
                                         \
    X(int, wsum, (nwave) + 1)                                                                                               \
    X(unsigned char, tie, nal)
inline size_t hr_image_bytes(int max_n) {
    const int nal = (max_n + 3) & ~3;
    size_t lds_bytes = 0;
    HR_STATE_ARRAYS(LDS_COUNT, nal, 1024 / 64)
    const size_t slack = 64;
    return std::max((lds_bytes + slack + 15) / 16 * 16, static_cast<size_t>(hc_npow2(max_n - 1)) * 16);
}

#define CUTREE_ARRAYS(X, n)                                                                                                 \
    X(int, absorbed, n)                                             \
    X(int, wsum, HC_THREADS / 64 + 1)                                                                                       \
    X(uint16_t, parent, n)                                                                      \
    X(uint16_t, rank, n)
inline size_t cutree_lds_bytes(int max_n) {
    size_t lds_bytes = 0;
    CUTREE_ARRAYS(LDS_COUNT, max_n)
    return lds_bytes + 16;
}

inline size_t cluster_sums_lds_bytes(int kpad) { return static_cast<size_t>(SS_WAVES) * kpad * 64 * 8; }

inline size_t stats_lds_bytes(int max_n, int kcap) {
    int npow2 = 1; while (npow2 < max_n) npow2 <<= 1;
    return static_cast<size_t>(npow2) * 8 + ST_THREADS * 8 + 2 * static_cast<size_t>(kcap) * 8 + (5 * static_cast<size_t>(kcap) + 8) * 4;
}

#define ML_PREP_ARRAYS(X, kf)                                                                                               \
    X(double, cn2, kf)                                                                                                      \
    X(double, ctot, kf)                                                                                                     \
    X(double, part, 1024)                                                                                                   \
    X(int, cnt, kf)
inline size_t ml_prep_lds_bytes(int kpad) {
    size_t lds_bytes = 0;
    ML_PREP_ARRAYS(LDS_COUNT, kpad)
    return lds_bytes + 64;
}

#define ML_CELLS_ARRAYS(X, kf)                                                                                              \
    X(double, st, kf)                        \
    X(double, sg, kf)                                                         \
    X(uint16_t, cnt, kf)                                                                                                    \
    X(uint16_t, live, kf)                                                 \
    X(uint16_t, pos, kf)
__host__ __device__ inline size_t ml_cells_wave_bytes(int kf) {
    size_t lds_bytes = 0;
    ML_CELLS_ARRAYS(LDS_COUNT, kf)
    return (lds_bytes + 15) & ~static_cast<size_t>(15);
}
inline size_t ml_cells_lds_bytes(int kpad) { return ml_cells_wave_bytes(kpad) * ML_WAVES; }

#define ML_LEVEL_ARRAYS(X, npow2)                                                                                           \
    X(double, sil, npow2)                                                                                                   \
    X(double, part, ST_THREADS)
inline size_t ml_level_lds_bytes(int max_n) {
    const int npow2 = hc_npow2(max_n);
    size_t lds_bytes = 0;
    ML_LEVEL_ARRAYS(LDS_COUNT, npow2)
    return lds_bytes;
}

struct HcAggloRange {
    const HcMeta *metas;
    int tasks, max_n;
    double *D, *S0, *S1;
    int *ia, *ib;
    double *height;
    int *status;
};
struct HcAggloDid {
    int form = 0;
    int wpt = 0;
    int finish_at = 0;
};
SHARP_HC_LOCAL bool hclust_bulk_synchronous(const HcAggloRange &r, bool split, DevBuf<unsigned char> &img, DevBuf<int> &remaining,
                                            hipEvent_t mid_event, int mid_round, HcAggloDid *did = nullptr);
SHARP_HC_LOCAL void hclust_sequential(const HcAggloRange &r, const int *only_if, unsigned char *gstate);

struct GemmTask;
struct HcStatsRange {
    const HcMeta *metas;
    int tasks, max_n, max_p, max_nk, max_kpad;
    bool any_sym;
    const GemmTask *gemm;
    const int *off, *cnt;
    const int *ia, *ib;
    int *lab;
    double *H, *Cr, *CSt, *T, *G, *Q, *nrm, *out;
};
struct HcManyLevels {
    const std::vector<HcMeta> *metas;
    const std::vector<MlMeta> *mlmetas;
    const MlMeta *dml;
    long long oM;
    int ml_off, ml_cnt, mlt_off, mlt_cnt;
    int *r1, *r2, *cntF;
    double *cn2m, *B, *cn2F, *tot2, *S;
};
SHARP_HC_LOCAL void hclust_copy_d(const HcMeta *metas, int tasks, const double *D, double *D0);
SHARP_HC_LOCAL void hclust_level_stats(const HcStatsRange &r, const HcManyLevels *ml);
SHARP_HC_LOCAL void hclust_pack_labels(const HcMeta *metas, int tasks, const int *lab, const int *chosen, const long long *dst_off, int *dst);

SHARP_HC_LOCAL void select_level(const HcParams &prm, int n, int nk, const double *msil, const double *CH, const double *height,
                                 int &oind, int &branch, int &rc);
SHARP_HC_LOCAL double host_ch_euclid(const double *y, int n, int p, const int *cl, int g);

}
```

sharp_amd/csrc/linalg.hip:

```cpp
#include "linalg.hpp"
#include "graph.hpp"

#include <algorithm>
#include <cstring>
#include <string>
#include <type_traits>
#include <vector>

namespace sharp {

typedef __attribute__((address_space(1))) const double *gcdp;
typedef __attribute__((address_space(1))) double *gdp;


typedef double v4f64 __attribute__((ext_vector_type(4)));

__device__ __forceinline__ void lds_barrier() { asm volatile("s_waitcnt lgkmcnt(0)\n\ts_barrier" ::: "memory"); }

constexpr int GT = 64, GK = 16, GLD = 80;

__global__ __launch_bounds__(256) void gemm_tn_f64_kernel(const GemmTask *__restrict__ tasks) {
    const GemmTask t = tasks[blockIdx.z];
    const int m0 = blockIdx.y * GT, n0 = blockIdx.x * GT;
    if (m0 >= t.M || n0 >= t.N) return;
// ... 222 lines not shown
        for (int i = 0; i < 4; ++i) {
            const bool mirror = t.symmetric && (n0 > m0 || wn * 2 + j > wm * 4 + i);
#pragma unroll
            for (int r = 0; r < 4; ++r) {
                const int row = m0 + wr + i * 16 + (lane >> 4) + 4 * r;
                if (i < ni && j < nj && mirror && row < t.M && col < t.N) {
                    const double v = acc[i][j][r];
                    b = fmin(b, t.nn_square ? v * v : v);
                }
            }
        }
        b = fmin(b, __shfl_xor(b, 16));
        b = fmin(b, __shfl_xor(b, 32));
        if (lane < 16) cols_s[wm * FT + wc + j * 16 + lane] = b;
    }
    __syncthreads();
    if (tid < FT) {
        double b = fmin(fmin(rows_s[tid], rows_s[FT + tid]), fmin(rows_s[2 * FT + tid], rows_s[3 * FT + tid]));
        if (ti == tj) b = fmin(b, fmin(cols_s[tid], cols_s[FT + tid]));
        if (m0 + tid < t.M) ((gdp)t.nn)[static_cast<long long>(tj) * t.ldc + m0 + tid] = b;
    } else if (tid < 2 * FT && ti != tj) {
        const int cc = tid - FT;
        if (n0 + cc < t.N) ((gdp)t.nn)[static_cast<long long>(ti) * t.ldc + n0 + cc] = fmin(cols_s[cc], cols_s[FT + cc]);
    }
}

void gemm_tn_f64_batched(const GemmTask *d_tasks, int count, int max_M, int max_N, const char *timer_name, bool fast, bool symmetric) {
    if (count <= 0 || max_M <= 0 || max_N <= 0) return;
    Ctx &c = ctx();
    KernelTimer tm(timer_name);
    for (int z0 = 0; z0 < count; z0 += 65535) {
        const int nz = std::min(65535, count - z0);
        if (fast) {
            const int ntm = (max_M + FT - 1) / FT, ntn = (max_N + FT - 1) / FT;
            const int tiles_max = symmetric ? ntn * (ntn + 1) / 2 : ntm * ntn;
            const long long blocks = static_cast<long long>((nz + 7) / 8) * 8 * tiles_max;
            long long slice = blocks;
            if (c.polite) {
                const int per_cu = knobs().gemm_slice;
                if (per_cu > 0) slice = static_cast<long long>(c.num_cu) * per_cu;
            }
            for (long long b0 = 0; b0 < blocks; b0 += slice)
                hipLaunchKernelGGL(gemm_tn_f64_fast_kernel, dim3(static_cast<unsigned>(std::min(slice, blocks - b0))), dim3(512), 0, c.stream,
                                   d_tasks + z0, nz, tiles_max, b0);
        }
        else
            hipLaunchKernelGGL(gemm_tn_f64_kernel, dim3((max_N + GT - 1) / GT, (max_M + GT - 1) / GT, nz), dim3(256), 0, c.stream,
                               d_tasks + z0);
        launch_check("gemm_tn_f64_kernel");
    }
}

constexpr int RP_MAXV = 8;

__device__ __forceinline__ bool fused_rows(const RowPrepTask &t) { return t.mode == 0 && t.p <= 64 * RP_MAXV; }

__global__ __launch_bounds__(256) void row_prep_kernel(const RowPrepTask *__restrict__ tasks, int skip_fused) {
    const RowPrepTask t = tasks[blockIdx.y];
    const int lane = threadIdx.x & 63;
    const int row = blockIdx.x * 4 + (threadIdx.x >> 6);
    if (row >= t.n) return;
    gcdp x = (gcdp)t.src + static_cast<long long>(row) * t.lds;
    gdp cr = (gdp)t.Cr + static_cast<long long>(row) * t.p;
    const int p = t.p;
    if (fused_rows(t) && skip_fused) return;
    if (t.mode == 2) {
        gdp drow = (gdp)t.D + static_cast<long long>(row) * t.nld;
        for (int q = lane; q < p; q += 64) drow[q] = q == row ? 0.0 : x[q];
        return;
    }
    if (t.mode == 0 && p <= 64 * RP_MAXV) {
        double xv[RP_MAXV];
#pragma unroll
        for (int u = 0; u < RP_MAXV; ++u) { const int q = lane + 64 * u; xv[u] = x[q < p ? q : 0]; }
        double s = 0.0;
#pragma unroll
        for (int u = 0; u < RP_MAXV; ++u) if (lane + 64 * u < p) s += xv[u];
        const double mean = wave_sum(s) / p;
        double ss = 0.0;
#pragma unroll
        for (int u = 0; u < RP_MAXV; ++u) if (lane + 64 * u < p) { const double c = xv[u] - mean; ss += c * c; }
        const double sd = sqrt(wave_sum(ss) / static_cast<double>(p - 1 > 1 ? p - 1 : 1));
        double s2 = 0.0;
#pragma unroll
        for (int u = 0; u < RP_MAXV; ++u) if (lane + 64 * u < p) { xv[u] = (xv[u] - mean) / sd; s2 += xv[u]; }
        const double mean2 = wave_sum(s2) / p;
        double n2 = 0.0;
#pragma unroll
        for (int u = 0; u < RP_MAXV; ++u) if (lane + 64 * u < p) { xv[u] -= mean2; n2 += xv[u] * xv[u]; }
        const double nr = sqrt(wave_sum(n2));
#pragma unroll
        for (int u = 0; u < RP_MAXV; ++u) if (lane + 64 * u < p) cr[lane + 64 * u] = xv[u] / nr;
        if (lane == 0) ((gdp)t.nrm)[row] = 1.0;
        return;
    }
    double s = 0.0;
    for (int q = lane; q < p; q += 64) s += x[q];
    const double mean = wave_sum(s) / p;
    if (t.mode == 0) {
        double ss = 0.0;
        for (int q = lane; q < p; q += 64) { const double c = x[q] - mean; ss += c * c; }
        const double sd = sqrt(wave_sum(ss) / static_cast<double>(p - 1 > 1 ? p - 1 : 1));
        double s2 = 0.0;
        for (int q = lane; q < p; q += 64) s2 += (x[q] - mean) / sd;
        const double mean2 = wave_sum(s2) / p;
        double n2 = 0.0;
        for (int q = lane; q < p; q += 64) { const double c = (x[q] - mean) / sd - mean2; n2 += c * c; }
        const double nr = sqrt(wave_sum(n2));
        for (int q = lane; q < p; q += 64) cr[q] = ((x[q] - mean) / sd - mean2) / nr;
        if (lane == 0) ((gdp)t.nrm)[row] = 1.0;
    } else {
        double n2 = 0.0;
        for (int q = lane; q < p; q += 64) { const double c = x[q] - mean; n2 += c * c; cr[q] = c; }
        const double nr = sqrt(wave_sum(n2));
        if (lane == 0) ((gdp)t.nrm)[row] = nr;
        gdp drow = (gdp)t.D + static_cast<long long>(row) * t.nld;
        for (int q = lane; q < p; q += 64) {
            double d;
            if (q == row) d = 0.0;
            else if (q < row) d = 1.0 - x[q];
            else d = 1.0 - ((gcdp)t.src)[static_cast<long long>(q) * t.lds + row];
            drow[q] = d;
        }
    }
}

__global__ __launch_bounds__(256) void transpose_kernel(const RowPrepTask *__restrict__ tasks, int skip_fused) {
    const RowPrepTask t = tasks[blockIdx.z];
    if ((fused_rows(t) && skip_fused) || t.mode == 2) return;
    __shared__ double tile[32][33];
    const int r0 = blockIdx.y * 32, q0 = blockIdx.x * 32;
    if (r0 >= t.nld || q0 >= t.p_pad) return;
    const int tx = threadIdx.x & 31, ty = threadIdx.x >> 5;
    for (int j = ty; j < 32; j += 8) {
        const int r = r0 + j, q = q0 + tx;
        tile[j][tx] = (r < t.n && q < t.p) ? ((gcdp)t.Cr)[static_cast<long long>(r) * t.p + q] : 0.0;
    }
    __syncthreads();
    for (int j = ty; j < 32; j += 8) {
        const int q = q0 + j, r = r0 + tx;
        if (q < t.p_pad && r < t.nld) ((gdp)t.Ct)[static_cast<long long>(q) * t.nld + r] = (r < t.n && q < t.p) ? tile[tx][j] : 0.0;
    }
}

constexpr int RT_ROWS = 16;
__global__ __launch_bounds__(256) void row_prep_t_kernel(const RowPrepTask *__restrict__ tasks) {
    const RowPrepTask t = tasks[blockIdx.y];
    const int r0 = blockIdx.x * RT_ROWS;
    if (!fused_rows(t) || r0 >= t.nld) return;
    extern __shared__ double rt_tile[];
    const int p = t.p, ldt = t.p_pad + 1;
    const int lane = threadIdx.x & 63, wave = threadIdx.x >> 6;
    for (int i = wave; i < RT_ROWS; i += 4) {
        const int row = r0 + i;
        double *trow = rt_tile + i * ldt;
        if (row >= t.n) {
            for (int q = lane; q < t.p_pad; q += 64) trow[q] = 0.0;
            continue;
        }
        gcdp x = (gcdp)t.src + static_cast<long long>(row) * t.lds;
        gdp cr = (gdp)t.Cr + static_cast<long long>(row) * t.p;
        double xv[RP_MAXV];
#pragma unroll
        for (int u = 0; u < RP_MAXV; ++u) { const int q = lane + 64 * u; xv[u] = x[q < p ? q : 0]; }
        double s = 0.0;
#pragma unroll
        for (int u = 0; u < RP_MAXV; ++u) if (lane + 64 * u < p) s += xv[u];
        const double mean = wave_sum(s) / p;
        double ss = 0.0;
#pragma unroll
        for (int u = 0; u < RP_MAXV; ++u) if (lane + 64 * u < p) { const double c = xv[u] - mean; ss += c * c; }
        const double sd = sqrt(wave_sum(ss) / static_cast<double>(p - 1 > 1 ? p - 1 : 1));
        double s2 = 0.0;
#pragma unroll
        for (int u = 0; u < RP_MAXV; ++u) if (lane + 64 * u < p) { xv[u] = (xv[u] - mean) / sd; s2 += xv[u]; }
        const double mean2 = wave_sum(s2) / p;
        double n2 = 0.0;
#pragma unroll
        for (int u = 0; u < RP_MAXV; ++u) if (lane + 64 * u < p) { xv[u] -= mean2; n2 += xv[u] * xv[u]; }
        const double nr = sqrt(wave_sum(n2));
#pragma unroll
        for (int u = 0; u < RP_MAXV; ++u) {
            const int q = lane + 64 * u;
            if (q < p) { const double v = xv[u] / nr; cr[q] = v; trow[q] = v; }
            else if (q < t.p_pad) trow[q] = 0.0;
        }
        if (lane == 0) ((gdp)t.nrm)[row] = 1.0;
    }
    __syncthreads();
    const int i = threadIdx.x & (RT_ROWS - 1);
    for (int q = threadIdx.x / RT_ROWS; q < t.p_pad; q += 256 / RT_ROWS)
        ((gdp)t.Ct)[static_cast<long long>(q) * t.nld + r0 + i] = rt_tile[i * ldt + q];
}

void row_prep_batched(const RowPrepTask *d_tasks, int count, int max_n, int max_p, bool all_feature_rows) {
    if (count <= 0 || max_n <= 0) return;
    Ctx &c = ctx();
    KernelTimer tm("row_prep");
    const bool fused = max_p <= 64 * RP_MAXV;
    for (int z0 = 0; z0 < count; z0 += 65535) {
        const int nz = std::min(65535, count - z0);
        const int nld_max = (max_n + 127) / 128 * 128;
        if (fused) {
            const size_t lds = static_cast<size_t>(RT_ROWS) * ((max_p + 15) / 16 * 16 + 1) * sizeof(double);
            SHARP_HIP_CHECK(hipFuncSetAttribute(reinterpret_cast<const void *>(row_prep_t_kernel), hipFuncAttributeMaxDynamicSharedMemorySize,
                                                static_cast<int>(lds)));
            hipLaunchKernelGGL(row_prep_t_kernel, dim3(nld_max / RT_ROWS, nz), dim3(256), lds, c.stream, d_tasks + z0);
            launch_check("row_prep_t_kernel");
            if (all_feature_rows) continue;
        }
        hipLaunchKernelGGL(row_prep_kernel, dim3((max_n + 3) / 4, nz), dim3(256), 0, c.stream, d_tasks + z0, fused ? 1 : 0);
        launch_check("row_prep_kernel");
        hipLaunchKernelGGL(transpose_kernel, dim3((max_p + 15 + 31) / 32, (nld_max + 31) / 32, nz), dim3(256), 0, c.stream, d_tasks + z0, fused ? 1 : 0);
        launch_check("transpose_kernel");
    }
}

}

using namespace sharp;

extern "C" {

int sharp_gemm_tn_f64(const double *At, const double *Bt, double *C, int M, int N, int K, int epilogue, int symmetric, int fast) {
    SHARP_API_BEGIN
    ctx();
    SHARP_REQUIRE(At && Bt && C && M > 0 && N > 0 && K > 0, "sharp_gemm_tn_f64: bad arguments");
    SHARP_REQUIRE(!symmetric || (M == N), "sharp_gemm_tn_f64: symmetric needs M == N");
    const long long lda = fast ? (M + 127) / 128 * 128 : M, ldb = fast ? (N + 127) / 128 * 128 : N;
    const int Kp = fast ? (K + 15) / 16 * 16 : K;
    std::vector<double> ha(static_cast<size_t>(Kp) * lda, 0.0), hb(static_cast<size_t>(Kp) * ldb, 0.0);
    for (int k = 0; k < K; ++k) {
        for (int i = 0; i < M; ++i) ha[static_cast<size_t>(k) * lda + i] = At[static_cast<size_t>(k) * M + i];
        for (int j = 0; j < N; ++j) hb[static_cast<size_t>(k) * ldb + j] = Bt[static_cast<size_t>(k) * N + j];
    }
    DevBuf<double> dA(ha.size()), dB(hb.size()), dC(static_cast<size_t>(M) * N);
    dA.upload(ha.data(), ha.size());
// ... 45 lines not shown
    std::vector<size_t> oA(count + 1, 0), oB(count + 1, 0), dA(count + 1, 0), dB(count + 1, 0), oC(count + 1, 0), oNN(count + 1, 0);
    int max_M = 0, max_N = 0;
    for (int t = 0; t < count; ++t) {
        SHARP_REQUIRE(M[t] >= 1 && N[t] >= 1 && K[t] >= 1, w + ": M, N and K of every task must be at least 1");
        SHARP_REQUIRE(!symmetric || M[t] == N[t], w + ": symmetric needs M == N in every task");
        const size_t lda = fast ? rup_ll(M[t], 128) : M[t], ldb = fast ? rup_ll(N[t], 128) : N[t], Kp = fast ? rup_ll(K[t], 16) : K[t];
        const size_t ldc = ldc_pad ? rup_ll(N[t], 128) : N[t];
        oA[t + 1] = oA[t] + static_cast<size_t>(K[t]) * M[t];
        oB[t + 1] = oB[t] + static_cast<size_t>(K[t]) * N[t];
        dA[t + 1] = dA[t] + Kp * lda;
        dB[t + 1] = dB[t] + (symmetric ? 0 : Kp * ldb);
        oC[t + 1] = oC[t] + static_cast<size_t>(M[t]) * ldc;
        oNN[t + 1] = oNN[t] + (want_nn ? ldc / 128 * ldc : 0);
        max_M = std::max(max_M, M[t]); max_N = std::max(max_N, N[t]);
    }
    SHARP_REQUIRE(dA[count] + dB[count] + oC[count] + oNN[count] <= (size_t(1) << 31), w + ": more than 16 GB of operands and results");
    std::vector<double> ha(dA[count], 0.0), hb(dB[count], 0.0);
    for (int t = 0; t < count; ++t) {
        const size_t lda = fast ? rup_ll(M[t], 128) : M[t], ldb = fast ? rup_ll(N[t], 128) : N[t];
        for (int k = 0; k < K[t]; ++k) {
            std::copy_n(At + oA[t] + static_cast<size_t>(k) * M[t], M[t], ha.data() + dA[t] + k * lda);
            if (!symmetric) std::copy_n(Bt + oB[t] + static_cast<size_t>(k) * N[t], N[t], hb.data() + dB[t] + k * ldb);
        }
    }
    DevBuf<double> bufA(ha.size()), bufB(hb.size()), bufC, bufNN;
    bufA.upload(ha.data(), ha.size());
    if (!hb.empty()) bufB.upload(hb.data(), hb.size());
    alloc_sentinel(bufC, oC[count]);
    alloc_sentinel(bufNN, oNN[count]);
    std::vector<GemmTask> tasks(count);
    for (int t = 0; t < count; ++t) {
        const long long lda = fast ? rup_ll(M[t], 128) : M[t], ldb = fast ? rup_ll(N[t], 128) : N[t];
        const long long ldc = ldc_pad ? rup_ll(N[t], 128) : N[t];
        const double *a = bufA.p + dA[t];
        tasks[t] = GemmTask{a, symmetric ? a : bufB.p + dB[t], bufC.p + oC[t], M[t], N[t], K[t], lda, symmetric ? lda : ldb, ldc,
                            epilogue, symmetric, fast, want_nn ? bufNN.p + oNN[t] : nullptr, nn_square};
    }
    DevBuf<GemmTask> dt(count);
    dt.upload(tasks.data(), count);
    {
        struct Polite {
            const bool on;
            explicit Polite(bool o) : on(o) { if (on) ctx().polite = true; }
            ~Polite() { if (on) ctx_unchecked().polite = false; }
        } scope(polite != 0);
        gemm_tn_f64_batched(dt.p, count, max_M, max_N, "test_gemm_batch", fast != 0, symmetric != 0);
    }
    bufC.download(C, oC[count]);
    if (want_nn) bufNN.download(nn, oNN[count]);
    stream_sync();
    SHARP_API_END
}

int sharp_row_prep_batch(int count, const int *n, const int *p, const long long *lds, const int *mode, const double *src,
                         int all_feature_rows, double *Cr, double *Ct, double *nrm, double *D) {
    SHARP_API_BEGIN
    ctx();
    const std::string w = "sharp_row_prep_batch";
    SHARP_REQUIRE(count >= 1, w + ": count must be at least 1");
    SHARP_REQUIRE(n && p && lds && mode && src && Cr && Ct && nrm && D, w + ": null argument");
    std::vector<size_t> oS(count + 1, 0), oCr(count + 1, 0), oCt(count + 1, 0), oN(count + 1, 0), oD(count + 1, 0);
    int max_n = 0, max_p = 0;
    for (int t = 0; t < count; ++t) {
        SHARP_REQUIRE(n[t] >= 1 && p[t] >= 1 && lds[t] >= p[t], w + ": every task needs n >= 1, p >= 1 and lds >= p");
        SHARP_REQUIRE(mode[t] >= 0 && mode[t] <= 2, w + ": mode must be 0, 1 or 2");
        SHARP_REQUIRE(mode[t] == 0 || n[t] == p[t], w + ": modes 1 and 2 take a square matrix (n == p)");
        SHARP_REQUIRE(!all_feature_rows || (mode[t] == 0 && p[t] <= 64 * RP_MAXV), w + ": all_feature_rows needs mode 0 and p <= 512 in every task");
        const size_t nld = rup_ll(n[t], 128), p_pad = rup_ll(p[t], 16);
        oS[t + 1] = oS[t] + static_cast<size_t>(n[t]) * lds[t];
        oCr[t + 1] = oCr[t] + static_cast<size_t>(n[t]) * p[t];
        oCt[t + 1] = oCt[t] + p_pad * nld;
        oN[t + 1] = oN[t] + n[t];
        oD[t + 1] = oD[t] + nld * nld;
        max_n = std::max(max_n, n[t]); max_p = std::max(max_p, p[t]);
    }
    SHARP_REQUIRE(oS[count] + oCr[count] + oCt[count] + oD[count] <= (size_t(1) << 31), w + ": more than 16 GB of inputs and results");
    DevBuf<double> dS(oS[count]), dCr, dCt, dN, dD;
    dS.upload(src, oS[count]);
    alloc_sentinel(dCr, oCr[count]);
    alloc_sentinel(dCt, oCt[count]);
    alloc_sentinel(dN, oN[count]);
    alloc_sentinel(dD, oD[count]);
    std::vector<RowPrepTask> tasks(count);
    for (int t = 0; t < count; ++t)
        tasks[t] = RowPrepTask{dS.p + oS[t], lds[t], n[t], p[t], static_cast<int>(rup_ll(n[t], 128)), static_cast<int>(rup_ll(p[t], 16)), mode[t],
                               dCr.p + oCr[t], dCt.p + oCt[t], dN.p + oN[t], dD.p + oD[t]};
    DevBuf<RowPrepTask> dt(count);
    dt.upload(tasks.data(), count);
    row_prep_batched(dt.p, count, max_n, max_p, all_feature_rows != 0);
    dCr.download(Cr, oCr[count]);
    dCt.download(Ct, oCt[count]);
    dN.download(nrm, oN[count]);
    dD.download(D, oD[count]);
    SHARP_API_END
}

}
```

sharp_amd/csrc/linalg.hpp:

```cpp
#pragma once
#include "common.hpp"

namespace sharp {

struct GemmTask {
    const double *At;
    const double *Bt;
    double *C;
    int M, N, K;
    long long lda, ldb, ldc;
    int epilogue;
    int symmetric;
    int fast;
    double *nn = nullptr;
    int nn_square = 0;
};

void gemm_tn_f64_batched(const GemmTask *d_tasks, int count, int max_M, int max_N, const char *timer_name, bool fast = false,
                         bool symmetric = false);

struct RowPrepTask {
    const double *src;
    long long lds;
    int n, p, nld;
    int p_pad;
    int mode;
    double *Cr;
    double *Ct;
    double *nrm;
    double *D;
};
void row_prep_batched(const RowPrepTask *d_tasks, int count, int max_n, int max_p, bool all_feature_rows = false);


#ifdef SHARP_LAB
constexpr int kDistI8Slices = 7;
struct DistI8Task {
    const double *Cr;
    double *D;
    signed char *sl;
    double *scale;
    int n, p, nld, ksteps;
};
size_t dist_i8_slice_bytes(int nld, int p);
void dist_i8_batched(const DistI8Task *d_tasks, int count, int max_n);
void dist_i8_slices(const DistI8Task *d_tasks, int count, int max_n);
void dist_i8_products(const DistI8Task *d_tasks, int count, int max_n);
#endif

}
```

sharp_amd/csrc/projector.hpp:

```cpp
#pragma once
#include <cstdint>
#include <memory>
#include <vector>

#include "common.hpp"

namespace sharp {

struct ProjectorGroup {
    int k0 = 0, kcount = 0;
    int ncomp = 0;
    long long nnz = 0;
    double mean_len = 0;
    int max_len = 0;
    int gw = 16;
    int slots = 4;
    int span() const { return slots * gw; }
    int neg_base = 0;
    int acc_slots() const { return neg_base ? 2 * neg_base : ncomp; }
    long long nseg = 0;
    DevBuf<uint16_t> ent;
    int novf = 0;
    DevBuf<uint32_t> ovf_gene;
    DevBuf<uint2> ovf_info;
// ... 12 lines not shown
    DevBuf<uint32_t> d_hits;
    DevBuf<unsigned int> d_nhits;
    std::vector<unsigned int> h_nhits;
    long long nnz_total() const { long long s = 0; for (auto &g : groups) s += g.nnz; return s; }
    ~Projector() { if (device_built) (void)hipDeviceSynchronize(); }
    Projector() = default;
    Projector(const Projector &) = delete;
    Projector &operator=(const Projector &) = delete;
};

constexpr uint32_t kCodeNeg = 4u, kCodeMore = 2u, kCodePad = 0xfff8u;
constexpr int kDumpSlots = 16;
constexpr int kMaxCompPerGroup = 8191 - kDumpSlots;
__host__ __device__ inline uint16_t pad_code(int ncomp, uint32_t l) { return static_cast<uint16_t>((static_cast<uint32_t>(ncomp) + l) << 3); }
__host__ __device__ inline bool lane_live(uint32_t pair01) { return pair01 < (kCodePad << 16); }

int dual_neg_base(int ncomp);
inline int code_lanes(int np, int nn, int slots) { return (np + slots - 1) / slots + (nn + slots - 1) / slots; }

#ifdef __HIPCC__
template <int SLOTS> struct RowWord;
template <> struct RowWord<4> { uint32_t x, y; };
template <> struct RowWord<2> { uint32_t x; };
template <int SLOTS>
__device__ __forceinline__ RowWord<SLOTS> load_row_word(const void *p) {
    RowWord<SLOTS> r;
    if constexpr (SLOTS == 4) { const uint2 t = *reinterpret_cast<const uint2 *>(p); r.x = t.x; r.y = t.y; }
    else r.x = *reinterpret_cast<const uint32_t *>(p);
    return r;
}
template <uint32_t ACC_LDS, int SLOTS, bool SIGNED>
__device__ __forceinline__ void scatter_row_word(RowWord<SLOTS> c, unsigned long long v) {
    typedef __attribute__((address_space(3))) unsigned long long lds_u64;
    if (lane_live(c.x)) {
        uint32_t w[SLOTS];
        w[0] = c.x & 0xfff8u;
        w[1] = SIGNED ? ((c.x >> 16) & 0xfff8u) : (c.x >> 16);
        if constexpr (SLOTS == 4) {
            w[2] = SIGNED ? (c.y & 0xfff8u) : (c.y & 0xffffu);
            w[3] = SIGNED ? ((c.y >> 16) & 0xfff8u) : (c.y >> 16);
        }
#pragma unroll
        for (int q = 0; q < SLOTS; ++q)
            __hip_atomic_fetch_add(reinterpret_cast<lds_u64 *>(static_cast<uintptr_t>(ACC_LDS + w[q])), v, __ATOMIC_RELAXED, __HIP_MEMORY_SCOPE_WORKGROUP);
    }
}
__device__ __forceinline__ uint32_t lds_address(const void *p) {
    return static_cast<uint32_t>(reinterpret_cast<uintptr_t>((__attribute__((address_space(3))) const void *)p));
}
#endif

constexpr int RP_FIX_BITS = 44;
std::shared_ptr<Projector> build_projector(int m, int p, int K, const double *seeds, const std::function<void()> *after_draw = nullptr);
void project_dev(const Projector &pr, XRef dX, int m, int n, long long ld, int log_flag, double *dE, long long ldE,
                 const int *d_row_map, unsigned ahead_token = 0);
unsigned rp_compact_ahead(XRef dX, int m, int n, long long ld, int log_flag);
void rp_compact_ahead_drop();
void rp_trim();
bool rp_pc_eligible(XRef X, int m, long long ld);
void project_dev_pc(const Projector &pr, const ProjectorGroup &g, XRef dX, int m, int n, long long ld, int log_flag, int fix_bits,
                    double *dE, long long ldE, const int *d_row_map);
void rp_pc_trim();
void project_dev_dense(const Projector &pr, XRef dX, int m, int n, long long ld, int log_flag, double *dE, long long ldE,
                       const int *d_row_map);
float device_absmax(XRef X, int m, long long n, long long ld);
XRef dev64_ref(const double *dX, int m, long long n, long long ld);
int register_projector(std::shared_ptr<Projector> pr);
std::shared_ptr<Projector> get_projector(int handle);
void drop_projector(int handle);

}
```

sharp_amd/csrc/rp.hip:

```cpp
#include "projector.hpp"
#include "upload.hpp"

#include <cmath>
#include <cstring>
#include <cstdlib>
#include <string>

namespace sharp {

constexpr int RP_THREADS = 512;
constexpr int RP_NV = 2;
constexpr int RP_STEP = RP_THREADS * 4 * RP_NV;
constexpr int RP_CAP = 2048;

struct __attribute__((aligned(16))) NzSlot {
    uint32_t gene;
    uint32_t xbits;
    long long fix;
};

template <bool VEC>
__device__ __forceinline__ float4 rp_load4(const float *col, int g0, int gend) {
    float4 v = make_float4(0.f, 0.f, 0.f, 0.f);
    if (VEC) {
        if (g0 + 3 < gend) {
            typedef float f4 __attribute__((ext_vector_type(4)));
            const f4 t = __builtin_nontemporal_load(reinterpret_cast<const f4 *>(col + g0));
            return make_float4(t.x, t.y, t.z, t.w);
        }
    }
    if (g0 < gend) v.x = col[g0];
    if (g0 + 1 < gend) v.y = col[g0 + 1];
    if (g0 + 2 < gend) v.z = col[g0 + 2];
    if (g0 + 3 < gend) v.w = col[g0 + 3];
    return v;
}

struct RpStepVals { float4 v[RP_NV]; };

template <bool VEC>
__device__ __forceinline__ RpStepVals rp_load_step(const float *col, int s, int step_len, int m, int tid) {
    RpStepVals r;
    const int g_begin = s * step_len;
    const int g_end = min(m, g_begin + step_len);
#pragma unroll
    for (int j = 0; j < RP_NV; ++j) r.v[j] = rp_load4<VEC>(col, g_begin + 4 * (tid + j * RP_THREADS), g_end);
    return r;
}

template <int GW, int SLOTS, bool VEC>
__global__ __launch_bounds__(RP_THREADS, 4) void rp_scatter_kernel(
    const float *__restrict__ X, int m, int n, long long ld, int log_flag, double fix_scale, double inv_fix,
// ... 178 lines not shown
    mx.zero();
    {
        KernelTimer t("rp_absmax");
        hipLaunchKernelGGL(absmax64_kernel, dim3(c.num_cu * 4), dim3(256), 0, c.stream, dX, m, static_cast<int>(n), ld, mx.p);
        launch_check("absmax64_kernel");
    }
    unsigned long long bits = 0;
    mx.download(&bits, 1);
    double f;
    memcpy(&f, &bits, 8);
    SHARP_REQUIRE(std::isfinite(f), "SHARP: the expression block holds NA / NaN / Inf");
    if (f > 3.4028234663852886e38) r.log_fix_bits = 41;
    return r;
}

template <int GW, int SLOTS, bool VEC>
static void launch_rp(const ProjectorGroup &g, const Projector &pr, const float *dX, int m, int n, long long ld,
                      int log_flag, int fix_bits, double *dE, long long ldE, const int *row_map) {
    Ctx &c = ctx();
    const size_t lds = RP_CAP * sizeof(NzSlot) + static_cast<size_t>(g.acc_slots() + kDumpSlots) * 8;
    const int nsteps = (m + RP_STEP - 1) / RP_STEP;
    const int step_len = ((m + nsteps - 1) / nsteps + 3) / 4 * 4;
    auto kern = rp_scatter_kernel<GW, SLOTS, VEC>;
    {
        hipFuncAttributes fa;
        SHARP_HIP_CHECK(hipFuncGetAttributes(&fa, reinterpret_cast<const void *>(kern)));
        SHARP_REQUIRE(fa.sharedSizeBytes == 0, "rp_scatter_kernel: static LDS in front of the dynamic block");
    }
    SHARP_HIP_CHECK(hipFuncSetAttribute(reinterpret_cast<const void *>(kern), hipFuncAttributeMaxDynamicSharedMemorySize,
                                        static_cast<int>(lds)));
    int per_cu = 1;
    SHARP_HIP_CHECK(hipOccupancyMaxActiveBlocksPerMultiprocessor(&per_cu, reinterpret_cast<const void *>(kern), RP_THREADS, lds));
    per_cu = std::max(1, std::min(per_cu, 4));
    long long blocks = std::min<long long>(n, static_cast<long long>(c.num_cu) * per_cu);
    const double fix_scale = std::ldexp(1.0, fix_bits), inv_fix = std::ldexp(1.0, -fix_bits);
    const double out_scale = 1.0 / std::sqrt(static_cast<double>(pr.p));
    KernelTimer t("rp_stage");
    hipLaunchKernelGGL(kern, dim3(static_cast<unsigned>(blocks)), dim3(RP_THREADS), lds, c.stream, dX, m, n, ld, log_flag,
                       fix_scale, inv_fix, pr.val, out_scale, g.ent.p, g.ovf_slot.p, g.ovf_info.p, g.novf, g.ncomp, g.neg_base, dE, ldE, g.k0 * pr.p,
                       nsteps, step_len, row_map);
    launch_check("rp_scatter_kernel");
}

#ifdef SHARP_LAB
void project_dev_split(const Projector &pr, const ProjectorGroup &g, XRef dX, int m, int n, long long ld, int log_flag,
                       int fix_bits, double *dE, long long ldE, const int *d_row_map, unsigned ahead_token);
#else
unsigned rp_compact_ahead(XRef, int, int, long long, int) { return 0; }
void rp_compact_ahead_drop() {}
void rp_trim() {}
#endif

void project_dev(const Projector &pr, XRef X, int m, int n, long long ld, int log_flag, double *dE, long long ldE,
                 const int *d_row_map, unsigned ahead_token) {
    struct DropAhead { ~DropAhead() { rp_compact_ahead_drop(); } } drop_ahead;
    const float *dX = X.f32();
    SHARP_REQUIRE(m == pr.m, "project: gene count differs from the projector's");
    SHARP_REQUIRE(ld >= m, "project: leading dimension smaller than m");
    SHARP_REQUIRE(ldE >= static_cast<long long>(pr.K) * pr.p, "project: ldE smaller than K*p");
    if (n <= 0) return;
    ctx();
    {
        if (knobs().rp_kernel == 2 || (knobs().rp_kernel == 0 && m <= 16)) {
            project_dev_dense(pr, X, m, n, ld, log_flag, dE, ldE, d_row_map);
            return;
        }
    }
    int fix_bits = std::min(RP_FIX_BITS, X.log_fix_bits);
    if (!log_flag) {
        const float f = device_absmax(X, m, n, ld);
        SHARP_REQUIRE(std::isfinite(f), "project: non-finite expression value");
        int e = 0;
        std::frexp(static_cast<double>(f), &e);
        fix_bits = std::min(52, 62 - 12 - std::max(e, 0));
    }
    const bool vec = (ld % (X.f64 ? 2 : 4) == 0) && ((reinterpret_cast<uintptr_t>(X.p) & 15u) == 0);
    SHARP_REQUIRE(!X.f64 || (vec && m >= 8 && m <= (1 << 20)), "project: an fp64 block must be 16-byte aligned with an even leading dimension");
    for (const auto &g : pr.groups) {
        const int gw = g.gw;
#define SHARP_RP_CASE(GWV, SL)                                                                          \
    if (vec) launch_rp<GWV, SL, true>(g, pr, dX, m, n, ld, log_flag, fix_bits, dE, ldE, d_row_map);      \
    else launch_rp<GWV, SL, false>(g, pr, dX, m, n, ld, log_flag, fix_bits, dE, ldE, d_row_map)
        const bool fused = knobs().rp_kernel == 1;
        if (rp_pc_eligible(X, m, ld)) {
            project_dev_pc(pr, g, X, m, n, ld, log_flag, fix_bits, dE, ldE, d_row_map);
            continue;
        }
#ifdef SHARP_LAB
        if (vec && m >= 8 && m <= (1 << 20) && (X.f64 || !fused)) {
            project_dev_split(pr, g, X, m, n, ld, log_flag, fix_bits, dE, ldE, d_row_map, ahead_token);
            continue;
        }
#else
        (void)fused; (void)ahead_token;
#endif
        SHARP_REQUIRE(!X.f64, "project: an fp64 block needs at least 17 genes (the producer / consumer kernel) or the dense form");
        if (gw == 16 && g.slots == 4) { SHARP_RP_CASE(16, 4); }
        else if (gw == 16) { SHARP_RP_CASE(16, 2); }
        else if (gw == 8) { SHARP_RP_CASE(8, 4); }
        else { SHARP_RP_CASE(4, 4); }
#undef SHARP_RP_CASE
    }
}

__host__ __device__ inline uint32_t synth_mix(uint32_t x) {
    x ^= x >> 16; x *= 0x7feb352du; x ^= x >> 15; x *= 0x846ca68bu; x ^= x >> 16;
    return x;
}
__host__ __device__ inline int synth_cluster(uint32_t seed, uint32_t cell, int G) {
    const uint32_t h = synth_mix(cell * 0x9e3779b9u + seed * 0x85ebca6bu + 0x1234567u);
    unsigned long long tot = 0, cur = 1ull << 20;
    for (int c = 0; c < G; ++c) { tot += cur; cur = cur * 82 / 100; }
    const unsigned long long u = (static_cast<unsigned long long>(h) * tot) >> 32;
    unsigned long long acc = 0;
    cur = 1ull << 20;
    for (int c = 0; c < G; ++c) { acc += cur; if (u < acc) return c; cur = cur * 82 / 100; }
    return G - 1;
}
__host__ __device__ inline float synth_value(uint32_t seed, uint32_t gene, uint32_t cell, int cl, int G, int nmark) {
    const uint32_t hg = synth_mix(gene * 0x27d4eb2fu + seed);
    const uint32_t h = synth_mix(synth_mix(gene * 0x9e3779b1u + seed) ^ (cell * 0x85ebca77u + 0xc2b2ae3du));
    const uint32_t u = h >> 8;
    const bool marker = (static_cast<int>(gene / static_cast<uint32_t>(nmark)) == cl) && (gene < static_cast<uint32_t>(G * nmark));
    const uint32_t lvl = hg & 3u;
    const uint32_t z_base[4] = {16106127u, 15770583u, 15435038u, 14763950u};
    const uint32_t z_mark[4] = {3355443u, 2516582u, 2013266u, 1677722u};
    const uint32_t z = marker ? z_mark[lvl] : z_base[lvl];
    if (u < z) return 0.0f;
    uint32_t r = synth_mix(h ^ 0x68bc21ebu);
    int cnt = 1;
    const uint32_t thr = marker ? 0xD0000000u : 0x50000000u;
    while (r < thr && cnt < 64) { ++cnt; r = synth_mix(r + 0x9e3779b9u); }
    return static_cast<float>(cnt);
}

__global__ void synth_fill_kernel(uint32_t seed, int m, long long cell0, int ncell, int G, int nmark, float *X, long long ld) {
    const long long cell = blockIdx.y;
    if (cell >= ncell) return;
    const uint32_t gcell = static_cast<uint32_t>(cell0 + cell);
    const int cl = synth_cluster(seed, gcell, G);
    float *col = X + cell * ld;
    for (int g = blockIdx.x * blockDim.x + threadIdx.x; g < m; g += gridDim.x * blockDim.x)
        col[g] = synth_value(seed, static_cast<uint32_t>(g), gcell, cl, G, nmark);
}

}

using namespace sharp;

extern "C" {

int sharp_project_dev(int proj, const float *dX, int m, int n, long long ld, int log_flag, double *dE, long long ldE) {
    SHARP_API_BEGIN
    auto pr = get_projector(proj);
    project_dev(*pr, dX, m, n, ld, log_flag, dE, ldE, nullptr);
    SHARP_API_END
}

int sharp_project_dev64(int proj, const double *dX, int m, int n, long long ld, int log_flag, double *dE, long long ldE) {
    SHARP_API_BEGIN
    auto pr = get_projector(proj);
    project_dev(*pr, dev64_ref(dX, m, n, ld), m, n, ld, log_flag, dE, ldE, nullptr);
    SHARP_API_END
}

int sharp_project(int proj, const double *X, int m, int n, long long ld, int log_flag, double *E) {
    SHARP_API_BEGIN
    auto pr = get_projector(proj);
    SHARP_REQUIRE(X && E, "sharp_project: null buffer");
    SHARP_REQUIRE(ld >= m, "sharp_project: ld < m");
    HostBlock hb;
    upload_block(X, m, n, ld, hb);
    const long long ldE = static_cast<long long>(pr->K) * pr->p;
    DevBuf<double> dE(static_cast<size_t>(ldE) * n);
    project_dev(*pr, hb.ref(), m, n, hb.ld, log_flag, dE.p, ldE, nullptr);
    dE.download(E, static_cast<size_t>(ldE) * n);
    SHARP_API_END
}

int sharp_synth_fill_dev(unsigned seed, int m, long long cell0, int ncell, int G, int nmark, float *dX, long long ld) {
    SHARP_API_BEGIN
    SHARP_REQUIRE(G >= 1 && G <= 64 && nmark >= 1 && ld >= m, "sharp_synth_fill_dev: bad arguments");
    if (ncell > 0) {
        Ctx &c = ctx();
        KernelTimer t("synth_fill");
        for (int c0 = 0; c0 < ncell; c0 += 65535) {
            const int nc = std::min(65535, ncell - c0);
            hipLaunchKernelGGL(synth_fill_kernel, dim3((m + 1023) / 1024, nc), dim3(256), 0, c.stream, seed, m, cell0 + c0, nc,
                               G, nmark, dX + static_cast<long long>(c0) * ld, ld);
            launch_check("synth_fill_kernel");
        }
    }
    SHARP_API_END
}

int sharp_synth_labels(unsigned seed, long long cell0, int ncell, int G, int *labels) {
    SHARP_API_BEGIN
    for (int i = 0; i < ncell; ++i) labels[i] = synth_cluster(seed, static_cast<uint32_t>(cell0 + i), G);
    SHARP_API_END
}

}
```

sharp_amd/csrc/rp3.hip:

```cpp
#include "rp_shared.hpp"

#include <cmath>
#include <cstdlib>

namespace sharp {

constexpr int PC_TAB = 1024;
constexpr uint32_t kPcGeneMask = 0xfffffu, kPcFull = 0x80000000u, kPcOne = 0x3F800000u;
constexpr uint32_t kPcBadMask = 0xFC00FFFFu;
typedef __attribute__((address_space(3))) uint32_t pc_lds_u32;
typedef __attribute__((address_space(1))) uint32_t pc_glb_u32;
typedef __attribute__((address_space(1))) long long pc_glb_i64;
typedef __attribute__((address_space(3))) long long pc_lds_i64;
__device__ __forceinline__ void pc_put_word(uint32_t *lst, uint32_t *swb, uint32_t lcap, uint32_t pos, uint32_t word) {
    if (pos < lcap) *(pc_lds_u32 *)(lst + pos) = word;
    else *(pc_glb_u32 *)(swb + pos) = word;
}
__device__ __forceinline__ uint32_t pc_get_word(const uint32_t *lst, const uint32_t *swb, uint32_t lcap, uint32_t pos) {
    uint32_t w;
    if (pos < lcap) w = *(const pc_lds_u32 *)(lst + pos);
    else w = __builtin_nontemporal_load((const pc_glb_u32 *)(swb + pos));
    return w;
}

__global__ void rp_pc_fixtab_kernel(double fix_scale, int log_flag, long long *__restrict__ tab) {
    const int i = blockIdx.x * blockDim.x + threadIdx.x;
    if (i >= PC_TAB) return;
    const double x = static_cast<double>(__uint_as_float((static_cast<uint32_t>(i) << 16) + kPcOne));
    const double f = log_flag == 2 ? log10(1.0 + x) : (log_flag ? log2(1.0 + x) : x);
    tab[i] = __double2ll_rn(f * fix_scale);
}

struct PcParams {
    const void *X;
    int m;
    long long ld;
    long long cell0;
    int ncell, log_flag;
    double fix_scale;
    const long long *fixtab;
    const uint16_t *ent;
    unsigned int dummy_seg;
    const uint2 *ovf_slot;
    int ncomp, neg_base;
    double inv_fix, val, out_scale;
    double *E;
    long long ldE;
    int comp0;
    const int *row_map;
    int lcap;
    int cap;
    uint32_t *sw;
    long long *st;
};

typedef uint32_t pc_u4 __attribute__((ext_vector_type(4)));
template <typename T> struct PcUnit { pc_u4 r[CpLayout<T>::LOADS]; };
__device__ __forceinline__ float pc_val(const PcUnit<float> &u, int q) { return __uint_as_float(u.r[q >> 2][q & 3]); }
__device__ __forceinline__ double pc_val(const PcUnit<double> &u, int q) {
    return __hiloint2double(static_cast<int>(u.r[q >> 1][2 * (q & 1) + 1]), static_cast<int>(u.r[q >> 1][2 * (q & 1)]));
}
template <typename T>
__device__ __forceinline__ void pc_issue(PcUnit<T> &u, const T *unit, int lim, int lane) {
    constexpr int V = CpLayout<T>::VEC, L = CpLayout<T>::LOADS;
#define SHARP_PC_LD(j, base, imm) asm volatile("global_load_dwordx4 %0, %1, %2 offset:%3 nt" : "=v"(u.r[j]) : "v"(voff), "s"(base), "n"(imm))
    if (lim >= CP_UNIT) {
        const uint32_t voff = static_cast<uint32_t>(lane) * 16u;
        SHARP_PC_LD(0, unit, 0); SHARP_PC_LD(1, unit, 1024); SHARP_PC_LD(2, unit, 2048); SHARP_PC_LD(3, unit, 3072);
        if constexpr (L == 8) {
            const T *hi = unit + 4096 / static_cast<int>(sizeof(T));
            SHARP_PC_LD(4, hi, 0); SHARP_PC_LD(5, hi, 1024); SHARP_PC_LD(6, hi, 2048); SHARP_PC_LD(7, hi, 3072);
        }
    } else {
#pragma unroll
        for (int j = 0; j < L; ++j) {
            const int g = V * (lane + 64 * j);
            const uint32_t voff = static_cast<uint32_t>(g + V - 1 < lim ? g : 0) * static_cast<uint32_t>(sizeof(T));
            SHARP_PC_LD(j, unit, 0);
        }
    }
#undef SHARP_PC_LD
}
template <int N>
__device__ __forceinline__ void pc_wait(PcUnit<float> &u) {
    asm volatile("s_waitcnt vmcnt(%4)" : "+v"(u.r[0]), "+v"(u.r[1]), "+v"(u.r[2]), "+v"(u.r[3]) : "n"(N));
}
template <int N>
__device__ __forceinline__ void pc_wait(PcUnit<double> &u) {
    asm volatile("s_waitcnt vmcnt(%8)" : "+v"(u.r[0]), "+v"(u.r[1]), "+v"(u.r[2]), "+v"(u.r[3]), "+v"(u.r[4]), "+v"(u.r[5]), "+v"(u.r[6]), "+v"(u.r[7]) : "n"(N));
}

template <typename T, int GW, int SLOTS, int MODE, int PC_THREADS, int NP, int D>
__global__ __launch_bounds__(PC_THREADS, 2 * (PC_THREADS / 64) / 4) void rp_pc_kernel(const PcParams P) {
    extern __shared__ __attribute__((aligned(16))) unsigned char smem[];
    constexpr bool DUAL = MODE == 1;
    constexpr bool WIDE = std::is_same<T, double>::value;
    constexpr int PC_NW = PC_THREADS / 64;
    constexpr int NC = PC_NW - NP, SPAN = SLOTS * GW, U = GW;
    typedef RowWord<SLOTS> Row;
    unsigned long long *acc = reinterpret_cast<unsigned long long *>(smem);
    const int tid = threadIdx.x, lane = tid & 63;
    const int wave = __builtin_amdgcn_readfirstlane(tid >> 6);
    const int nslots = (DUAL ? 2 * P.neg_base : P.ncomp) + kDumpSlots;
    uint32_t *ctl = reinterpret_cast<uint32_t *>(acc + nslots);
    uint32_t *lists = ctl + 8;
    long long *lterms = reinterpret_cast<long long *>(lists + 2 * P.lcap);
    for (int c = tid; c < nslots; c += PC_THREADS) acc[c] = 0ull;
    if (tid < 8) ctl[tid] = 0u;
    __syncthreads();
    const int G = static_cast<int>(gridDim.x);
    const int nmine = (P.ncell - static_cast<int>(blockIdx.x) + G - 1) / G;
    auto cell_of = [&](int j) __attribute__((always_inline)) -> long long { return P.cell0 + static_cast<long long>(blockIdx.x) + static_cast<long long>(j) * G; };
    uint32_t *const sw = P.sw + static_cast<size_t>(blockIdx.x) * 2 * P.cap;
    long long *const st = P.st + static_cast<size_t>(blockIdx.x) * 2 * P.cap;

    auto cell_end = [&](int it) __attribute__((always_inline)) {
        asm volatile("s_waitcnt lgkmcnt(0)\n\ts_barrier" ::: "memory");
        if (it >= 0 && wave >= NP) {
            const long long row = static_cast<long long>(static_cast<int>(ctl[2]));
            double *erow = P.E + row * P.ldE + P.comp0;
            for (int c = tid - NP * 64; c < P.ncomp; c += PC_THREADS - NP * 64) {
                long long a = static_cast<long long>(atomicExch(&acc[c], 0ull));
                if constexpr (DUAL) a -= static_cast<long long>(atomicExch(&acc[P.neg_base + c], 0ull));
                __builtin_nontemporal_store(P.out_scale * (P.val * (static_cast<double>(a) * P.inv_fix)), &erow[c]);
            }
            if (tid == NP * 64) ctl[it & 1] = 0u;
        }
        asm volatile("s_waitcnt lgkmcnt(0)\n\ts_barrier" ::: "memory");
    };

    if (wave >= NP) {
        const int cw = wave - NP;
        const int lg = lane % GW;
        const unsigned char *entb = reinterpret_cast<const unsigned char *>(P.ent);
        cell_end(-1);
        const uint32_t *lst = lists;
        const uint32_t *swb = sw;
        const long long *stb = st;
        const long long *ltm = lterms;
        int nnz = 0, nb = 0;
        const int gcap = P.lcap;
        uint32_t gC = 0u, gL = 0u, wR = 0u;
        long long fC = 0ll, fL = 0ll;
        Row cd[U], cdn[U];
        auto load_word = [&](int bt) __attribute__((always_inline)) -> uint32_t {
            const int e = (bt << 6) + lane;
            const int ec = e < nnz ? e : 0;
            if ((bt << 6) + 64 <= gcap) return *(const pc_lds_u32 *)(lst + ec);
            return pc_get_word(lst, swb, static_cast<uint32_t>(gcap), static_cast<uint32_t>(ec));
        };
        auto decode = [&](int bt, uint32_t w, uint32_t &g, long long &f) __attribute__((always_inline)) {
            const int e = (bt << 6) + lane;
            long long ff = P.fixtab[(w >> 20) & 0x3ffu];
            if (__ballot((w & kPcFull) != 0u) != 0ull) {
                if (w & kPcFull) {
                    const int ec = e < nnz ? e : 0;
                    if constexpr (WIDE) {
                        long long bits;
                        if (ec < gcap) bits = *(const pc_lds_i64 *)(ltm + ec);
                        else bits = __builtin_nontemporal_load((const pc_glb_i64 *)(stb + ec));
                        const double x = __longlong_as_double(bits);
                        const double fv = P.log_flag == 2 ? log10(1.0 + x) : (P.log_flag ? log2(1.0 + x) : x);
                        ff = __double2ll_rn(fv * P.fix_scale);
                    } else {
                        ff = __builtin_nontemporal_load((const pc_glb_i64 *)(stb + ec));
                    }
                }
            }
            g = e < nnz ? (w & kPcGeneMask) : P.dummy_seg;
            f = e < nnz ? ff : 0ll;
        };
        auto load_lists = [&](uint32_t g, Row (&dst)[U]) __attribute__((always_inline)) {
            const uint32_t gofs = g * static_cast<uint32_t>(SPAN * 2);
            static_for<U>([&](auto uc) {
                constexpr int u = decltype(uc)::value;
                dst[u] = load_row_word<SLOTS>(entb + (group_bcast<GW, u>(gofs) + static_cast<uint32_t>(2 * SLOTS * lg)));
            });
// ... 233 lines not shown
#define SHARP_PC_A_NP 2
#define SHARP_PC_A_D 3
#endif
    const int threads = shape_b ? SHARP_PC_B_THREADS : 512;
    const void *kern = nullptr;
    if constexpr (std::is_same<T, double>::value) kern = reinterpret_cast<const void *>(rp_pc_kernel<T, GW, SLOTS, MODE, 512, 2, 2>);
    else kern = shape_b ? reinterpret_cast<const void *>(rp_pc_kernel<T, GW, SLOTS, MODE, SHARP_PC_B_THREADS, SHARP_PC_B_NP, SHARP_PC_B_D>)
                        : reinterpret_cast<const void *>(rp_pc_kernel<T, GW, SLOTS, MODE, 512, SHARP_PC_A_NP, SHARP_PC_A_D>);
    const size_t acc_bytes = static_cast<size_t>(g.acc_slots() + kDumpSlots) * 8 + 32;
    const size_t budget = 80 * 1024;
    SHARP_REQUIRE(acc_bytes + 2 * 64 * 12 <= budget, "rp_pc_kernel: the accumulators leave no LDS for the entry lists");
    constexpr bool wide = std::is_same<T, double>::value;
    const size_t per_entry = wide ? 12 : 4;
    int lcap = static_cast<int>((budget - acc_bytes) / (2 * per_entry) / 64 * 64);
    lcap = std::min(lcap, (P.m + 63) / 64 * 64);
    P.lcap = lcap;
    const size_t lds = acc_bytes + static_cast<size_t>(lcap) * 2 * per_entry;
    SHARP_HIP_CHECK(hipFuncSetAttribute(kern, hipFuncAttributeMaxDynamicSharedMemorySize, static_cast<int>(lds)));
    {
        hipFuncAttributes fa;
        SHARP_HIP_CHECK(hipFuncGetAttributes(&fa, kern));
        SHARP_REQUIRE(fa.sharedSizeBytes == 0, "rp_pc_kernel: static LDS in front of the accumulators");
    }
    int per_cu = 1;
    SHARP_HIP_CHECK(hipOccupancyMaxActiveBlocksPerMultiprocessor(&per_cu, kern, threads, lds));
    per_cu = std::max(1, std::min(per_cu, 2));
    per_cu = std::min(per_cu, std::max(1, knobs().rp_pc_wgs));
    if (c.rp_wgs_cap > 0) per_cu = std::min(per_cu, c.rp_wgs_cap);
    const int grid = c.num_cu * per_cu;
    P.cap = (P.m + 3) / 4 * 4;
    W.sw.ensure(static_cast<size_t>(c.num_cu) * 2 * 2 * P.cap);
    W.st.ensure(static_cast<size_t>(c.num_cu) * 2 * 2 * P.cap);
    P.sw = W.sw.p;
    P.st = W.st.p;
    const long long slice = c.polite ? static_cast<long long>(grid) * 16 : static_cast<long long>(n);
    for (long long c0 = 0; c0 < n; c0 += slice) {
        P.cell0 = c0;
        P.ncell = static_cast<int>(std::min<long long>(slice, n - c0));
        const int blocks = std::min(P.ncell, grid);
        void *args[] = {&P};
        SHARP_HIP_CHECK(hipLaunchKernel(kern, dim3(static_cast<unsigned>(blocks)), dim3(static_cast<unsigned>(threads)), args, lds, st));
        launch_check("rp_pc_kernel");
    }
}
}

bool rp_pc_eligible(XRef X, int m, long long ld) {
    const bool vec = (ld % (X.f64 ? 2 : 4) == 0) && ((reinterpret_cast<uintptr_t>(X.p) & 15u) == 0);
    const int k = knobs().rp_kernel;
    return (k == 0 || k == 3 || k == 4 || (X.f64 && k != 2)) && vec && m > 16 && m <= (1 << 20);
}

void project_dev_pc(const Projector &pr, const ProjectorGroup &g, XRef dX, int m, int n, long long ld, int log_flag, int fix_bits,
                    double *dE, long long ldE, const int *d_row_map) {
    Ctx &c = ctx();
    PcWs &W = pws();
    const double fix_scale = std::ldexp(1.0, fix_bits), inv_fix = std::ldexp(1.0, -fix_bits);
    if (W.fixtab.n == 0 || W.fixtab_key != fix_scale || W.fixtab_mode != log_flag) {
        W.fixtab.ensure(PC_TAB);
        hipLaunchKernelGGL(rp_pc_fixtab_kernel, dim3(PC_TAB / 256), dim3(256), 0, c.stream, fix_scale, log_flag, W.fixtab.p);
        launch_check("rp_pc_fixtab_kernel");
        W.fixtab_key = fix_scale;
        W.fixtab_mode = log_flag;
    }
    PcParams P;
    P.X = dX.p; P.m = m; P.ld = ld; P.cell0 = 0; P.ncell = n; P.log_flag = log_flag; P.fix_scale = fix_scale; P.fixtab = W.fixtab.p;
    P.ent = g.ent.p; P.dummy_seg = static_cast<unsigned int>(g.nseg); P.ovf_slot = g.ovf_slot.p; P.ncomp = g.ncomp; P.neg_base = g.neg_base;
    P.inv_fix = inv_fix; P.val = pr.val; P.out_scale = 1.0 / std::sqrt(static_cast<double>(pr.p));
    P.E = dE; P.ldE = ldE; P.comp0 = g.k0 * pr.p; P.row_map = d_row_map;
    P.lcap = 0; P.cap = 0; P.sw = nullptr; P.st = nullptr;
    KernelTimer t("rp_stage");
    KernelTimer t2("rp_pc");
    const int mode = g.neg_base > 0 ? 1 : 0;
#define SHARP_PCL(TT, GWV, SL, MD) launch_pc<TT, GWV, SL, MD>(g, pr, P, n, c.stream)
#define SHARP_PCM(TT, GWV, SL) { if (mode == 1) SHARP_PCL(TT, GWV, SL, 1); else SHARP_PCL(TT, GWV, SL, 0); }
#define SHARP_PCT(TT)                                        \
    if (g.gw == 16 && g.slots == 4) SHARP_PCM(TT, 16, 4)     \
    else if (g.gw == 16) SHARP_PCM(TT, 16, 2)                \
    else if (g.gw == 8) SHARP_PCM(TT, 8, 4)                  \
    else SHARP_PCM(TT, 4, 4)
    if (dX.f64) { SHARP_PCT(double) } else { SHARP_PCT(float) }
#undef SHARP_PCM
#undef SHARP_PCT
#undef SHARP_PCL
}

void rp_pc_trim() {
    PcWs &W = pws();
    W.sw.release();
    W.st.release();
}

}
```

sharp_amd/csrc/runtime.hip:

```cpp
#include <cstring>
#include <ctime>
#include <atomic>
#include <condition_variable>
#include <exception>
#include <pthread.h>
#include <mutex>
#include <thread>
#include <unistd.h>
#include <sstream>
#include <tuple>
#include <vector>
#include <cstdio>

#include "common.hpp"

namespace sharp {

static thread_local std::string g_last_error;
static thread_local int t_slot = 0;
static Ctx g_ctxs[kMaxSlots];

void set_error(const std::string &msg) { g_last_error = msg; }

int cur_slot() { return t_slot; }
// ... 239 lines not shown
        std::lock_guard<std::mutex> lk(P.mu);
        if (P.held + cap_bytes <= kPoolMaxHeld) { P.blocks.insert({{dev, cap_bytes}, p}); P.held += cap_bytes; return; }
    }
    (void)hipFree(p);
}
void pool_clear() {
    BlockPool &P = block_pool();
    std::lock_guard<std::mutex> lk(P.mu);
    for (auto &kv : P.blocks) (void)hipFree(kv.second);
    P.blocks.clear(); P.held = 0;
}

HostTimer::HostTimer(const char *n) : name(n), t0(0), on(false) {
    Ctx &c = ctx_unchecked();
    if (c.ready && c.profiling) { on = true; t0 = now_s(); }
}
HostTimer::~HostTimer() {
    if (!on) return;
    Ctx &c = ctx_unchecked();
    auto &s = c.stats[std::string("host:") + name];
    s.ms += (now_s() - t0) * 1e3;
    s.launches += 1;
}

}

namespace sharp {
static Knobs read_knobs() {
    Knobs v;
    auto env = [](const char *name) { return getenv(name); };
    auto num = [&](const char *name, int dflt) { const char *e = env(name); return e && *e ? atoi(e) : dflt; };
    if (const char *kv = env("SHARP_RP_KERNEL")) v.rp_kernel = !strcmp(kv, "fused") ? 1 : !strcmp(kv, "dense") ? 2 : !strcmp(kv, "pc") ? 4 : 0;
    if (const char *xs = env("SHARP_X_STORAGE")) v.x_storage = !strcmp(xs, "fp32") ? 32 : !strcmp(xs, "fp64") ? 64 : 0;
    v.host_threads = num("SHARP_HOST_THREADS", 0);
    v.upload_threads = num("SHARP_UPLOAD_THREADS", 0);
    v.tail_threads = num("SHARP_TAIL_THREADS", 4);
    v.unlimited_batch = num("SHARP_UNLIMITED_BATCH", 1) != 0;
    v.unlimited_window_mb = num("SHARP_UNLIMITED_WINDOW_MB", 0);
    v.block_prefetch = num("SHARP_NO_BLOCK_PREFETCH", 0) == 0;
    v.decision_log = num("SHARP_DECISION_LOG", 0) != 0;
    v.host_group = num("SHARP_HOST_GROUP", 1);
    v.step_marks = num("SHARP_STEP_MARKS", 0) != 0;
    v.hc_seq = num("SHARP_HC_SEQ", 0) == 1;
    v.hc_mono = num("SHARP_HC_MONO", 0) == 1;
    v.hc_split = num("SHARP_HC_SPLIT", -1);
    v.hc_pipe = num("SHARP_HC_PIPE", 1) != 0;
    v.hc_chunk = num("SHARP_HC_CHUNK", 0);
    v.hc_first_chunk = num("SHARP_HC_FIRST_CHUNK", 0);
    v.hc_ranges = num("SHARP_HC_RANGES", 0);
    v.hc_wpt = num("SHARP_HC_WPT", 0);
    v.hc_finish_at = num("SHARP_HC_FINISH_AT", 15);
    v.hc_nn_gemm = num("SHARP_HC_NN_GEMM", 1) != 0;
    v.stats_lane = num("SHARP_STATS_LANE", 1) != 0;
    v.ml_min_levels = num("SHARP_ML_MIN_LEVELS", 0);
    v.proj_host = num("SHARP_PROJ_HOST", 0) == 1;
    v.rp_pc_wgs = std::max(1, num("SHARP_RP_PC_WGS", 2));
    v.gemm_slice = num("SHARP_GEMM_SLICE", 8);
#ifdef SHARP_LAB
    if (const char *kv = env("SHARP_RP_KERNEL")) { if (!strcmp(kv, "sparse")) v.rp_kernel = 3; else if (!strcmp(kv, "split")) v.rp_kernel = 5; }
    v.rp_dual = num("SHARP_RP_DUAL", 1) != 0;
    { const int ser = num("SHARP_RP_SERIAL", -1); v.rp_two_streams = ser < 0 ? -1 : (ser == 0 ? 1 : 0); }
    v.rp_chunk = num("SHARP_RP_CHUNK", 0);
    v.rp_ahead = num("SHARP_RP_AHEAD", 2);
    v.rp_cp_wgs = std::max(1, num("SHARP_RP_CP_WGS", 8));
    v.rp_ap_wgs = std::max(1, num("SHARP_RP_AP_WGS", 4));
    v.rp_shape = num("SHARP_RP_SHAPE", 0);
    if (const char *ps = env("SHARP_RP_PC_SHAPE")) v.rp_pc_shape = (*ps == 'a' || *ps == 'A') ? 1 : (*ps == 'b' || *ps == 'B') ? 2 : 0;
    v.mean_early = num("SHARP_MEAN_EARLY", 0) != 0;
    v.hc_prep_early = num("SHARP_HC_PREP_EARLY", 1) != 0;
    v.hc_tri = num("SHARP_HC_TRI", 0) != 0;
    v.hc_front = num("SHARP_HC_FRONT", 0);
    v.hc_half = num("SHARP_HC_HALF", 0) != 0;
    v.stats_sums = num("SHARP_STATS_SUMS", 1) != 0;
    v.dist_i8 = num("SHARP_DIST_I8", 0) != 0;
    v.free_later = num("SHARP_FREE_LATER", 1) != 0;
    v.front_overlap = num("SHARP_FRONT_OVERLAP", 0);
    v.tail_priority = num("SHARP_TAIL_PRIORITY", 1) != 0;
#endif
    if (const char *dl = env("SHARP_DEVICES")) {
        for (const char *q = dl; *q;) {
            char *end = nullptr;
            const long dvc = strtol(q, &end, 10);
            if (end == q) break;
            v.devices.push_back(static_cast<int>(dvc));
            q = *end == ',' ? end + 1 : end;
        }
    }
    return v;
}
static Knobs &knobs_storage() { static Knobs k = read_knobs(); return k; }
const Knobs &knobs() { return knobs_storage(); }
void reload_knobs() { knobs_storage() = read_knobs(); }

namespace {
struct StepMarks { std::mutex mu; std::vector<std::tuple<const char *, int, double>> v; };
StepMarks &step_marks() { static StepMarks *M = new StepMarks; return *M; }
}
void step_mark(const char *label, int id) {
    if (!knobs().step_marks) return;
    const double t = now_s();
    StepMarks &M = step_marks();
    std::lock_guard<std::mutex> lk(M.mu);
    M.v.emplace_back(label, id, t);
}
void step_marks_dump() {
    if (!knobs().step_marks) return;
// ... 201 lines not shown
```

Measured before the change: 3.137 million.

## Fuse ensemble mean into projection epilogue and compute cluster sums from Ct

```diff
diff --git a/include/sharp_hip.h b/include/sharp_hip.h
--- a/include/sharp_hip.h
+++ b/include/sharp_hip.h
@@ -30,6 +30,8 @@
 int sharp_projector_triplets(int handle, int k, int *gene, int *col, signed char *sign, long long *nnz);
 
 int sharp_project(int proj, const double *X, int m, int n, long long ld, int log_flag, double *E);
+int sharp_project_mean(int proj, const double *X, int m, int n, long long ld, int log_flag, const int *row_map, double *E, double *viE,
+                       int *fused);
 int sharp_project_dev(int proj, const float *dX, int m, int n, long long ld, int log_flag,
                       double *dE, long long ldE);
 int sharp_project_dev64(int proj, const double *dX, int m, int n, long long ld, int log_flag,
@@ -317,6 +319,10 @@
                             int symmetric, int fast, int nn_square, int want_nn, int polite, int ldc_pad, double *C, double *nn);
 int sharp_row_prep_batch(int count, const int *n, const int *p, const long long *lds, const int *mode, const double *src,
                          int all_feature_rows, double *Cr, double *Ct, double *nrm, double *D);
+int sharp_row_prep_batch_nocr(int count, const int *n, const int *p, const long long *lds, const int *mode, const double *src, double *Ct,
+                              double *nrm, double *D);
+int sharp_cluster_sums_batch(int count, const int *n, const int *p, const int *kmax, const double *src, const int *labels, double *CSt_cr,
+                             double *CSt_ct);
 
 int sharp_get_opt_hclust_batch(int count, const int *n, const int *p, const int *kind, const int *hmethod, const int *N_cluster,
                                const int *minN, const int *maxN, const double *sil_thre, const double *height_Ntimes, const double *mats,
diff --git a/sharp_amd/_abi.py b/sharp_amd/_abi.py
--- a/sharp_amd/_abi.py
+++ b/sharp_amd/_abi.py
@@ -20,6 +20,7 @@
     "sharp_projector_info": "i:ipppp",
     "sharp_projector_triplets": "i:iipppp",
     "sharp_project": "i:ipiilip",
+    "sharp_project_mean": "i:ipiilipppp",
     "sharp_project_dev": "i:ipiilipl",
     "sharp_project_dev64": "i:ipiilipl",
     "sharp_get_opt_hclust": "i:piiiiiiddppppppppp",
@@ -140,6 +141,8 @@
     "sharp_gemm_tn_f64": "i:pppiiiiii",
     "sharp_gemm_tn_f64_batch": "i:ipppppiiiiiiipp",
     "sharp_row_prep_batch": "i:ipppppipppp",
+    "sharp_row_prep_batch_nocr": "i:ipppppppp",
+    "sharp_cluster_sums_batch": "i:ippppppp",
     "sharp_get_opt_hclust_batch": "i:ippppppppppiipppppppppp",
     "sharp_hclust_batch_plan": "i:pip",
     "sharp_wMetaC_batch": "i:ipppppppppppppppppp",
diff --git a/sharp_amd/csrc/common.hpp b/sharp_amd/csrc/common.hpp
--- a/sharp_amd/csrc/common.hpp
+++ b/sharp_amd/csrc/common.hpp
@@ -84,6 +84,8 @@
     bool tail_priority = true;
     bool dist_i8 = false;
     bool stats_sums = true;
+    bool sums_ct = true;
+    bool rp_mean = true;
     bool stats_lane = true;
     bool hc_tri = false;
     bool hc_prep_early = true;
diff --git a/sharp_amd/csrc/driver.hip b/sharp_amd/csrc/driver.hip
--- a/sharp_amd/csrc/driver.hip
+++ b/sharp_amd/csrc/driver.hip
@@ -48,11 +48,13 @@
 
 struct DriverWs {
     DevBuf<double> E, Eb, viE_sh, viE_out;
+    DevBuf<double> viE_shb;
     DevBuf<int> pos, posb;
     hipEvent_t mean_go = nullptr, mean_done = nullptr;
     hipStream_t mean_stream = nullptr;
     DevBuf<double> Ebatch;
     DevBuf<int> posbatch;
+    DevBuf<double> viEbatch;
     DevBuf<double> fold_means, block_means;
     double *view_pinned = nullptr;
     size_t view_pinned_n = 0;
@@ -172,6 +174,7 @@
     std::shared_ptr<Projector> pr;
     long long ldE = 0;
     double *E = nullptr; int *dpos = nullptr;
+    double *viE = nullptr;
     std::vector<HcTask> tasks;
     std::shared_ptr<HcPrefetch> hc;
     bool matches(XRef X, int m_, int n_, long long ld_, int K_, int p_, int ng_, const SharpArgs &a, const HcParams &b) const {
@@ -219,7 +222,7 @@
 }
 
 static void large_front(LargeFront &F, const SharpArgs &a, bool ahead, double *E_into = nullptr, int *pos_into = nullptr,
-                        const Shuffle *same_size = nullptr) {
+                        const Shuffle *same_size = nullptr, double *viE_into = nullptr) {
     const int n = F.n, m = F.m, K = F.K, p = F.p;
     F.shuffle = n < 100000;
     std::vector<int> &pos = F.pos;
@@ -249,7 +252,17 @@
         if (F.shuffle) { dpos.ensure(n); dpos.upload(pos.data(), n); }
         F.E = E.p; F.dpos = F.shuffle ? dpos.p : nullptr;
     }
-    project_dev(*F.pr, F.dX, m, n, F.ld, a.flag, F.E, F.ldE, F.dpos, ahead_tok);
+    RpMeanOut mo;
+    if (!a.fpart && knobs().rp_mean && F.pr->groups.size() == 1) {
+        if (E_into) mo.viE = viE_into;
+        else {
+            DevBuf<double> &V = ahead ? dws().viE_shb : dws().viE_sh;
+            V.ensure(static_cast<size_t>(n) * p);
+            mo.viE = V.p;
+        }
+    }
+    project_dev(*F.pr, F.dX, m, n, F.ld, a.flag, F.E, F.ldE, F.dpos, ahead_tok, &mo);
+    F.viE = mo.written ? mo.viE : nullptr;
     if (a.fpart) {
         Ctx &c = ctx();
         hipLaunchKernelGGL(round1_kernel, dim3(c.num_cu * 8), dim3(256), 0, c.stream, F.E, static_cast<long long>(n) * F.ldE);
@@ -265,7 +278,7 @@
         }
 }
 
-static void enqueue_ensemble_mean(const double *E, long long ldE, int n, int p, int K, double *viE_sh, hipEvent_t after) {
+static void enqueue_ensemble_mean(const double *E, long long ldE, int n, int p, int K, double *viE_sh, hipEvent_t after, bool written = false) {
     Ctx &c = ctx();
     hipEvent_t &mean_done = dws().mean_done;
     hipStream_t &ms = dws().mean_stream;
@@ -279,7 +292,7 @@
     SHARP_HIP_CHECK(hipEventRecord(dws().mean_go, c.stream));
     SHARP_HIP_CHECK(hipStreamWaitEvent(ms, dws().mean_go, 0));
     if (after) SHARP_HIP_CHECK(hipStreamWaitEvent(ms, after, 0));
-    {
+    if (!written) {
         StreamScope scope(ms);
         ensemble_mean_dev(E, ldE, n, p, K, viE_sh);
     }
@@ -293,10 +306,13 @@
     const long long ldE = F.ldE;
     struct { double *p; } E{F.E};
     struct { int *p; } dpos{F.dpos};
-    DevBuf<double> &viE_sh = dws().viE_sh;
-    viE_sh.ensure(static_cast<size_t>(n) * p);
+    struct { double *p; } viE_sh{F.viE};
+    if (!F.viE) {
+        dws().viE_sh.ensure(static_cast<size_t>(n) * p);
+        viE_sh.p = dws().viE_sh.p;
+    }
     hipEvent_t &mean_done = dws().mean_done;
-    if (!hc_after_last_agglomeration_fired()) enqueue_ensemble_mean(E.p, ldE, n, p, K, viE_sh.p, nullptr);
+    if (F.viE || !hc_after_last_agglomeration_fired()) enqueue_ensemble_mean(E.p, ldE, n, p, K, viE_sh.p, nullptr, F.viE != nullptr);
     bool view_sent = false;
     if (a.view_to_host && !a.fpart) {
         DriverWs &W = dws();
@@ -452,6 +468,7 @@
             Fp = std::move(PF.f);
             std::swap(dws().E, dws().Eb);
             std::swap(dws().pos, dws().posb);
+            std::swap(dws().viE_sh, dws().viE_shb);
         } else {
             SHARP_HIP_CHECK(hipStreamSynchronize(PF.stream));
             PF.f.reset();
@@ -506,11 +523,11 @@
         HostTimer ht("base_clustering_total");
         if (F.hc) { hc_set_after_last_agglomeration(nullptr); hc_prefetch_stamp_block(*F.hc, a.block); hc_prefetch_finish(*F.hc, false, hr); }
         else {
-            dws().viE_sh.ensure(static_cast<size_t>(n) * p);
+            if (!F.viE) dws().viE_sh.ensure(static_cast<size_t>(n) * p);
             const double *Ep = F.E;
             const long long ldEp = F.ldE;
             double *vsh = dws().viE_sh.p;
-            if (knobs().mean_early) hc_set_after_last_agglomeration([=](hipEvent_t ev) { enqueue_ensemble_mean(Ep, ldEp, n, p, K, vsh, ev); });
+            if (knobs().mean_early && !F.viE) hc_set_after_last_agglomeration([=](hipEvent_t ev) { enqueue_ensemble_mean(Ep, ldEp, n, p, K, vsh, ev); });
             else hc_set_after_last_agglomeration(nullptr);
             for (HcTask &tk : F.tasks) tk.prm.dec_block = a.block;
             try { get_opt_hclust_batch(F.tasks, false, hr); } catch (...) { hc_set_after_last_agglomeration(nullptr); throw; }
@@ -707,6 +724,8 @@
     DriverWs &W = dws();
     W.Ebatch.ensure(static_cast<size_t>(rows) * ldE);
     W.posbatch.ensure(static_cast<size_t>(rows));
+    const bool rp_mean = knobs().rp_mean && get_projector(proj)->groups.size() == 1;
+    if (rp_mean) W.viEbatch.ensure(static_cast<size_t>(rows) * p);
     last_small().valid = false;
     std::vector<HcTask> tasks;
     std::vector<size_t> first(nbk + 1, 0);
@@ -734,7 +753,7 @@
     Shuffle same_size;
     const auto front_of = [&](int q) {
         if (fo >= 2 && q >= 2) ctx().rp_wgs_cap = 1;
-        large_front(*F[q], A[q], false, W.Ebatch.p + row0[q] * ldE, W.posbatch.p + row0[q], &same_size);
+        large_front(*F[q], A[q], false, W.Ebatch.p + row0[q] * ldE, W.posbatch.p + row0[q], &same_size, rp_mean ? W.viEbatch.p + row0[q] * p : nullptr);
         ctx().rp_wgs_cap = 0;
         if (F[q]->shuffle && static_cast<int>(same_size.pos.size()) != F[q]->n) { same_size.reind = F[q]->reind; same_size.pos = F[q]->pos; }
     };
@@ -925,10 +944,11 @@
         upload_release_staging();
         dws().Ebatch.release();
         dws().posbatch.release();
+        dws().viEbatch.release();
         if (dws().view_pinned) { (void)hipHostFree(dws().view_pinned); dws().view_pinned = nullptr; dws().view_pinned_n = 0; }
         rp_pc_trim();
         rp_trim();
-        if (cur_slot() != 0) { hc_release_workspaces(); dws().E.release(); dws().Eb.release(); dws().viE_sh.release(); dws().viE_out.release(); }
+        if (cur_slot() != 0) { hc_release_workspaces(); dws().E.release(); dws().Eb.release(); dws().viE_sh.release(); dws().viE_shb.release(); dws().viE_out.release(); }
     });
     pool_clear();
     SHARP_API_END
diff --git a/sharp_amd/csrc/hclust.hip b/sharp_amd/csrc/hclust.hip
--- a/sharp_amd/csrc/hclust.hip
+++ b/sharp_amd/csrc/hclust.hip
@@ -148,7 +148,7 @@
         SHARP_REQUIRE(tk.n <= kHcMaxN, "get_opt_hclust: more than 16384 observations in one clustering task is not supported");
         SHARP_REQUIRE(tk.prm.hmethod >= 1 && tk.prm.hmethod <= 8, "get_opt_hclust: unknown agglomeration method");
         M.n = tk.n; M.p = tk.symmetric ? tk.n : tk.p; M.nld = static_cast<int>(rup(tk.n, 128));
-        M.method = tk.prm.hmethod; M.symmetric = tk.symmetric ? (tk.distance ? 2 : 1) : 0; M.pad0 = 0;
+        M.method = tk.prm.hmethod; M.symmetric = tk.symmetric ? (tk.distance ? 2 : 1) : 0; M.no_cr = 0;
         if (tk.prm.N_cluster > 0) {
             SHARP_REQUIRE(tk.prm.N_cluster >= 2, "The given N.cluster is less than 2, which is not suitable for clustering!");
             SHARP_REQUIRE(tk.prm.N_cluster <= tk.n - 1, "N.cluster must be smaller than the number of observations");
@@ -162,7 +162,6 @@
         M.kpad = static_cast<int>(rup(M.kmax, 16));
         M.oD = oD; oD += static_cast<long long>(M.nld) * M.nld;
         M.oD0 = oD0; if (M.symmetric == 1) oD0 += static_cast<long long>(M.nld) * M.nld;
-        M.oCr = oCr; if (M.symmetric != 2) oCr += static_cast<long long>(M.n) * M.p;
         M.oCt = oCt; if (M.symmetric != 2) oCt += rup(M.p, 16) * M.nld;
         M.oNrm = oN; oN += M.n;
         M.oM = oM; oM += M.n;
@@ -175,6 +174,17 @@
         max_kpad = std::max(max_kpad, M.kpad);
     }
     J.oOut = oOut; J.oM = oM; J.oLab = oLab; J.max_n = max_n; J.max_p = max_p; J.max_nk = max_nk; J.max_kpad = max_kpad;
+    {
+        bool ct_sums = knobs().sums_ct && cluster_sums_by_kernel(max_nk > ml_min_levels(), max_kpad);
+#ifdef SHARP_LAB
+        if (knobs().dist_i8 && max_p <= 8192) ct_sums = false;
+#endif
+        for (HcMeta &M : metas) {
+            M.no_cr = ct_sums && row_prep_fused_path(M.symmetric, max_p);
+            M.oCr = M.no_cr ? 0 : oCr;
+            if (!M.no_cr && M.symmetric != 2) oCr += static_cast<long long>(M.n) * M.p;
+        }
+    }
     SHARP_REQUIRE(max_nk > ml_min_levels() ||
                   stats_lds_bytes(max_n, std::max(max_kpad, 64)) <= ST_LDS_MAX,
                   "get_opt_hclust: this many observations with this many candidate cluster numbers does not fit the silhouette kernel "
@@ -215,8 +225,8 @@
     for (int t = 0; t < T; ++t) {
         const HcTask &tk = tasks[i0 + t];
         const HcMeta &M = metas[t];
-        prep[t] = RowPrepTask{tk.d_mat, tk.ld, M.n, M.p, M.nld, static_cast<int>(rup(M.p, 16)), M.symmetric, W.Cr.p + M.oCr,
-                              W.Ct.p + M.oCt, W.nrm.p + M.oNrm, W.D.p + M.oD};
+        prep[t] = RowPrepTask{tk.d_mat, tk.ld, M.n, M.p, M.nld, static_cast<int>(rup(M.p, 16)), M.symmetric,
+                              M.no_cr ? nullptr : W.Cr.p + M.oCr, W.Ct.p + M.oCt, W.nrm.p + M.oNrm, W.D.p + M.oD};
     }
     W.prep.upload(prep.data(), T);
     typedef ChunkJob::Range Range;
@@ -377,8 +387,10 @@
         if (J.pipe && J.has_next) SHARP_HIP_CHECK(hipStreamWaitEvent(st, EV.gemm[J.next_slot], 0));
         if (J.pipe && J.next2_slot >= 0) SHARP_HIP_CHECK(hipStreamWaitEvent(st, EV.gemm[J.next2_slot], 0));
         if (J.seq_pending) { launch_sequential(true); J.seq_pending = false; }
-        const HcStatsRange stats{dmeta, Ts, max_n, max_p, J.max_nk, max_kpad, R.any_sym, W.gemm.p, R.off, R.cnt, W.ia.p, W.ib.p, W.lab.p,
-                                 W.H.p, W.Cr.p, W.CSt.p, W.T.p, W.G.p, W.Q.p, W.nrm.p, W.out.p};
+        bool any_no_cr = false, any_cr = false;
+        for (int t = R.t0; t < R.t1; ++t) { any_no_cr |= J.metas[t].no_cr != 0; any_cr |= J.metas[t].no_cr == 0; }
+        const HcStatsRange stats{dmeta, Ts, max_n, max_p, J.max_nk, max_kpad, R.any_sym, any_no_cr, any_cr, W.gemm.p, R.off, R.cnt, W.ia.p, W.ib.p,
+                                 W.lab.p, W.H.p, W.Cr.p, W.Ct.p, W.CSt.p, W.T.p, W.G.p, W.Q.p, W.nrm.p, W.out.p};
         const HcManyLevels many{&J.metas, &J.mlmetas, W.mlmeta.p, J.oM, J.ml_off, J.ml_cnt, J.mlt_off, J.mlt_cnt, W.mlr1.p, W.mlr2.p, W.mlcntF.p,
                                 W.mlcn2m.p, W.mlB.p, W.mlcn2F.p, W.mltot2.p, W.mlS.p};
         hclust_level_stats(stats, J.ml ? &many : nullptr);
diff --git a/sharp_amd/csrc/hclust_stats.hip b/sharp_amd/csrc/hclust_stats.hip
--- a/sharp_amd/csrc/hclust_stats.hip
+++ b/sharp_amd/csrc/hclust_stats.hip
@@ -1,6 +1,8 @@
 #include "hclust_task.hpp"
 
 #include <algorithm>
+#include <cstring>
+#include <string>
 #include <vector>
 
 #include "linalg.hpp"
@@ -64,7 +66,7 @@
                                                                      const double *__restrict__ Cr_all, double *__restrict__ CSt_all) {
     const HcMeta M = metas[blockIdx.y];
     const int j0 = blockIdx.x * 64;
-    if (j0 >= M.p) return;
+    if (M.no_cr || j0 >= M.p) return;
     extern __shared__ __attribute__((aligned(16))) unsigned char ss_sm[];
     double *acc = reinterpret_cast<double *>(ss_sm);
     const int tid = threadIdx.x, lane = tid & 63;
@@ -96,6 +98,76 @@
     __syncthreads();
     double *CSt = CSt_all + M.oCSt;
     for (int q = tid; q < kpad * 64; q += 64 * SS_WAVES) {
+        const int c = q >> 6, l = q & 63;
+        if (j0 + l >= p) continue;
+        double v = acc[c * 64 + l];
+#pragma unroll
+        for (int w = 1; w < SS_WAVES; ++w) v += acc[(w * kpad + c) * 64 + l];
+        CSt[static_cast<long long>(j0 + l) * kpad + c] = v;
+    }
+}
+
+template <int W>
+__global__ __launch_bounds__(64 * SS_WAVES) void cluster_sums_ct_kernel(const HcMeta *__restrict__ metas, const int *__restrict__ lab_all,
+                                                                        const double *__restrict__ Ct_all, double *__restrict__ CSt_all) {
+    constexpr int NT = 64 * SS_WAVES, LDT = W + 1;
+    constexpr int FSTEP = NT / W;
+    constexpr int PER = 64 / FSTEP;
+    static_assert(NT % W == 0 && 64 % FSTEP == 0 && W % 16 == 0 && 128 % W == 0 && W % SS_WAVES == 0, "tile shape");
+    const HcMeta M = metas[blockIdx.y];
+    const int j0 = blockIdx.x * 64;
+    if (!M.no_cr || j0 >= M.p) return;
+    extern __shared__ __attribute__((aligned(16))) unsigned char ss_sm[];
+    const int kpad = M.kpad, n = M.n, p = M.p;
+    unsigned char *lds_cursor = ss_sm;
+    CLUSTER_SUMS_CT_ARRAYS(LDS_CARVE, kpad, W)
+    const int tid = threadIdx.x, lane = tid & 63;
+    const int wave = __builtin_amdgcn_readfirstlane(tid >> 6);
+    for (int q = tid; q < SS_WAVES * kpad * 64; q += NT) acc[q] = 0.0;
+    const int *lab = lab_all + M.oLab + static_cast<long long>(M.nk - 1) * n;
+    const double *Ct = Ct_all + M.oCt;
+    const long long nld = M.nld;
+    const int cell = tid % W, f0 = tid / W;
+    double r[PER];
+    int rl = 1;
+    auto fetch = [&](int c0) {
+#pragma unroll
+        for (int u = 0; u < PER; ++u) {
+            const int q = j0 + f0 + u * FSTEP;
+            r[u] = q < p ? Ct[q * nld + c0 + cell] : 0.0;
+        }
+        if (tid < W) rl = c0 + tid < n ? lab[c0 + tid] : 1;
+    };
+    double *mine = acc + static_cast<size_t>(wave) * kpad * 64 + lane;
+    const double *trow = tile + lane * LDT;
+    fetch(0);
+    for (int c0 = 0; c0 < n; c0 += W) {
+#pragma unroll
+        for (int u = 0; u < PER; ++u) tile[(f0 + u * FSTEP) * LDT + cell] = r[u];
+        if (tid < W) tlab[tid] = rl;
+        __syncthreads();
+        if (c0 + W < n) fetch(c0 + W);
+        const int lim = min(W, n - c0);
+        int u = wave;
+        for (; u + 3 * SS_WAVES < lim; u += 4 * SS_WAVES) {
+            double x[4];
+            int c[4];
+#pragma unroll
+            for (int v = 0; v < 4; ++v) {
+                c[v] = __builtin_amdgcn_readfirstlane(tlab[u + v * SS_WAVES]) - 1;
+                x[v] = trow[u + v * SS_WAVES];
+            }
+#pragma unroll
+            for (int v = 0; v < 4; ++v) mine[c[v] * 64] += x[v];
+        }
+        for (; u < lim; u += SS_WAVES) {
+            const int c = __builtin_amdgcn_readfirstlane(tlab[u]) - 1;
+            mine[c * 64] += trow[u];
+        }
+        __syncthreads();
+    }
+    double *CSt = CSt_all + M.oCSt;
+    for (int q = tid; q < kpad * 64; q += NT) {
         const int c = q >> 6, l = q & 63;
         if (j0 + l >= p) continue;
         double v = acc[c * 64 + l];
@@ -520,6 +592,27 @@
     launch_check("ml_cells_kernel");
 }
 
+void launch_cluster_sums(const HcMeta *metas, int Ts, int max_p, int max_kpad, bool any_cr, bool any_no_cr, const int *lab, const double *Cr,
+                         const double *Ct, double *CSt) {
+    hipStream_t st = ctx().stream;
+    const dim3 grid((max_p + 63) / 64, Ts), block(64 * SS_WAVES);
+    if (any_cr) {
+        const size_t lds = cluster_sums_lds_bytes(max_kpad);
+        allow_dynamic_lds(cluster_sums_kernel, lds);
+        hipLaunchKernelGGL(cluster_sums_kernel, grid, block, lds, st, metas, lab, Cr, CSt);
+        launch_check("cluster_sums_kernel");
+    }
+    if (any_no_cr) {
+        const int W = cluster_sums_ct_tile(max_kpad);
+        const size_t lds = cluster_sums_ct_lds_bytes(max_kpad, W);
+        SHARP_REQUIRE(lds <= HR_LDS_CU, "cluster_sums_ct_kernel: more clusters than its LDS tables take");
+        const auto kern = W == 32 ? cluster_sums_ct_kernel<32> : cluster_sums_ct_kernel<16>;
+        allow_dynamic_lds(kern, lds);
+        hipLaunchKernelGGL(kern, grid, block, lds, st, metas, lab, Ct, CSt);
+        launch_check("cluster_sums_ct_kernel");
+    }
+}
+
 }
 
 void hclust_level_stats(const HcStatsRange &r, const HcManyLevels *ml) {
@@ -532,7 +625,8 @@
         hipLaunchKernelGGL(cutree_kernel, dim3(Ts), dim3(HC_THREADS), lds, st, r.metas, r.ia, r.ib, r.lab);
         launch_check("cutree_kernel");
     }
-    const bool sums = knobs().stats_sums && !ml && max_kpad <= SS_KMAX;
+    const bool sums = cluster_sums_by_kernel(ml != nullptr, max_kpad);
+    SHARP_REQUIRE(sums || !r.any_no_cr, "get_opt_hclust: a task without its row-major rows reached the skinny-GEMM cluster sums");
     if (!sums || r.any_sym) {
         KernelTimer tm("onehot");
         hipLaunchKernelGGL(onehot_kernel, dim3(64, Ts), dim3(256), 0, st, r.metas, r.lab, r.H);
@@ -540,10 +634,7 @@
     }
     if (sums) {
         KernelTimer tm("cluster_sums_gemm");
-        const size_t lds = cluster_sums_lds_bytes(max_kpad);
-        allow_dynamic_lds(cluster_sums_kernel, lds);
-        hipLaunchKernelGGL(cluster_sums_kernel, dim3((max_p + 63) / 64, Ts), dim3(64 * SS_WAVES), lds, st, r.metas, r.lab, r.Cr, r.CSt);
-        launch_check("cluster_sums_kernel");
+        launch_cluster_sums(r.metas, Ts, max_p, max_kpad, r.any_cr, r.any_no_cr, r.lab, r.Cr, r.Ct, r.CSt);
     } else if (r.cnt[1]) gemm_tn_f64_batched(r.gemm + r.off[1], r.cnt[1], max_p, max_kpad, "cluster_sums_gemm");
     if (ml) { many_levels_stats(r, *ml); return; }
     if (r.cnt[2]) gemm_tn_f64_batched(r.gemm + r.off[2], r.cnt[2], max_kpad, max_n, "row_cluster_dot_gemm");
@@ -562,3 +653,65 @@
 }
 
 }
+
+using namespace sharp;
+
+extern "C" {
+
+int sharp_cluster_sums_batch(int count, const int *n, const int *p, const int *kmax, const double *src, const int *labels, double *CSt_cr,
+                             double *CSt_ct) {
+    SHARP_API_BEGIN
+    ctx();
+    const std::string w = "sharp_cluster_sums_batch";
+    SHARP_REQUIRE(count >= 1, w + ": count must be at least 1");
+    SHARP_REQUIRE(n && p && kmax && src && labels && CSt_cr && CSt_ct, w + ": null argument");
+    std::vector<HcMeta> metas(count, HcMeta());
+    std::vector<RowPrepTask> prep(count);
+    long long oS = 0, oCt = 0, oN = 0, oCS = 0;
+    int max_n = 0, max_p = 0, max_kpad = 0;
+    for (int t = 0; t < count; ++t) {
+        SHARP_REQUIRE(n[t] >= 1 && p[t] >= 1 && p[t] <= kRowPrepFusedMaxP, w + ": every task needs n >= 1 and 1 <= p <= 512");
+        SHARP_REQUIRE(kmax[t] >= 1 && kmax[t] <= SS_KMAX, w + ": kmax must be between 1 and 144");
+        for (int i = 0; i < n[t]; ++i)
+            SHARP_REQUIRE(labels[oN + i] >= 1 && labels[oN + i] <= kmax[t], w + ": a label outside 1..kmax");
+        HcMeta &M = metas[t];
+        M.n = n[t]; M.p = p[t]; M.nld = (n[t] + 127) / 128 * 128;
+        M.kmin = M.kmax = kmax[t]; M.nk = 1; M.kpad = (kmax[t] + 15) / 16 * 16;
+        M.oCr = oS; M.oCt = oCt; M.oNrm = oN; M.oLab = oN; M.oCSt = oCS;
+        oS += static_cast<long long>(M.n) * M.p;
+        oCt += static_cast<long long>((M.p + 15) / 16 * 16) * M.nld;
+        oN += M.n;
+        oCS += static_cast<long long>(M.p) * M.kpad;
+        max_n = std::max(max_n, M.n); max_p = std::max(max_p, M.p); max_kpad = std::max(max_kpad, M.kpad);
+    }
+    const unsigned long long sentinel_bits = 0x7ff8c0de5eed0001ull;
+    double sentinel;
+    memcpy(&sentinel, &sentinel_bits, sizeof sentinel);
+    const std::vector<double> fill(oCS, sentinel);
+    DevBuf<double> dS(oS), dCr(oS), dCt(oCt), dN(oN), dA(oCS), dB(oCS);
+    DevBuf<int> dLab(oN);
+    dS.upload(src, oS);
+    dLab.upload(labels, oN);
+    dA.upload(fill.data(), oCS);
+    dB.upload(fill.data(), oCS);
+    for (int t = 0; t < count; ++t) {
+        const HcMeta &M = metas[t];
+        prep[t] = RowPrepTask{dS.p + M.oCr, M.p, M.n, M.p, M.nld, (M.p + 15) / 16 * 16, 0, dCr.p + M.oCr, dCt.p + M.oCt, dN.p + M.oNrm, nullptr};
+    }
+    DevBuf<RowPrepTask> dprep(count);
+    dprep.upload(prep.data(), count);
+    DevBuf<HcMeta> dmeta_cr(count), dmeta_ct(count);
+    std::vector<HcMeta> metas_ct(metas);
+    for (HcMeta &M : metas_ct) M.no_cr = 1;
+    dmeta_cr.upload(metas.data(), count);
+    dmeta_ct.upload(metas_ct.data(), count);
+    row_prep_batched(dprep.p, count, max_n, max_p, true);
+    launch_cluster_sums(dmeta_cr.p, count, max_p, max_kpad, true, false, dLab.p, dCr.p, dCt.p, dA.p);
+    launch_cluster_sums(dmeta_ct.p, count, max_p, max_kpad, false, true, dLab.p, dCr.p, dCt.p, dB.p);
+    dA.download(CSt_cr, oCS);
+    dB.download(CSt_ct, oCS);
+    stream_sync();
+    SHARP_API_END
+}
+
+}
diff --git a/sharp_amd/csrc/hclust_task.hpp b/sharp_amd/csrc/hclust_task.hpp
--- a/sharp_amd/csrc/hclust_task.hpp
+++ b/sharp_amd/csrc/hclust_task.hpp
@@ -9,7 +9,8 @@
 
 struct HcMeta {
     int n, p, nld, kmin, kmax, nk, kpad, method;
-    int symmetric, pad0;
+    int symmetric;
+    int no_cr;
     long long oD, oD0;
     long long oCr, oCt, oNrm;
     long long oM;
@@ -102,6 +103,17 @@
 }
 
 inline size_t cluster_sums_lds_bytes(int kpad) { return static_cast<size_t>(SS_WAVES) * kpad * 64 * 8; }
+#define CLUSTER_SUMS_CT_ARRAYS(X, kpad, W)                                                                                  \
+    X(double, acc, SS_WAVES * (kpad) * 64)                                                                                  \
+    X(double, tile, 64 * ((W) + 1))                                                                                         \
+    X(int, tlab, W)
+inline size_t cluster_sums_ct_lds_bytes(int kpad, int W) {
+    size_t lds_bytes = 0;
+    CLUSTER_SUMS_CT_ARRAYS(LDS_COUNT, kpad, W)
+    return lds_bytes;
+}
+inline int cluster_sums_ct_tile(int kpad) { return cluster_sums_ct_lds_bytes(kpad, 32) <= HR_LDS_CU ? 32 : 16; }
+static_assert(static_cast<size_t>(SS_WAVES) * SS_KMAX * 64 * 8 + 64 * 17 * 8 + 16 * 4 <= HR_LDS_CU, "cluster_sums_ct_kernel<16> fits at SS_KMAX");
 
 inline size_t stats_lds_bytes(int max_n, int kcap) {
     int npow2 = 1; while (npow2 < max_n) npow2 <<= 1;
@@ -164,12 +176,14 @@
     const HcMeta *metas;
     int tasks, max_n, max_p, max_nk, max_kpad;
     bool any_sym;
+    bool any_no_cr, any_cr;
     const GemmTask *gemm;
     const int *off, *cnt;
     const int *ia, *ib;
     int *lab;
-    double *H, *Cr, *CSt, *T, *G, *Q, *nrm, *out;
-};
+    double *H, *Cr, *Ct, *CSt, *T, *G, *Q, *nrm, *out;
+};
+inline bool cluster_sums_by_kernel(bool many_levels, int max_kpad) { return knobs().stats_sums && !many_levels && max_kpad <= SS_KMAX; }
 struct HcManyLevels {
     const std::vector<HcMeta> *metas;
     const std::vector<MlMeta> *mlmetas;
diff --git a/sharp_amd/csrc/linalg.hip b/sharp_amd/csrc/linalg.hip
--- a/sharp_amd/csrc/linalg.hip
+++ b/sharp_amd/csrc/linalg.hip
@@ -298,6 +298,7 @@
 }
 
 constexpr int RP_MAXV = 8;
+static_assert(64 * RP_MAXV == kRowPrepFusedMaxP, "linalg.hpp tells the callers which rows take the one-pass path");
 
 __device__ __forceinline__ bool fused_rows(const RowPrepTask &t) { return t.mode == 0 && t.p <= 64 * RP_MAXV; }
 
@@ -397,6 +398,7 @@
     extern __shared__ double rt_tile[];
     const int p = t.p, ldt = t.p_pad + 1;
     const int lane = threadIdx.x & 63, wave = threadIdx.x >> 6;
+    const bool store_cr = t.Cr != nullptr;
     for (int i = wave; i < RT_ROWS; i += 4) {
         const int row = r0 + i;
         double *trow = rt_tile + i * ldt;
@@ -428,7 +430,7 @@
 #pragma unroll
         for (int u = 0; u < RP_MAXV; ++u) {
             const int q = lane + 64 * u;
-            if (q < p) { const double v = xv[u] / nr; cr[q] = v; trow[q] = v; }
+            if (q < p) { const double v = xv[u] / nr; if (store_cr) cr[q] = v; trow[q] = v; }
             else if (q < t.p_pad) trow[q] = 0.0;
         }
         if (lane == 0) ((gdp)t.nrm)[row] = 1.0;
@@ -580,13 +582,12 @@
     SHARP_API_END
 }
 
-int sharp_row_prep_batch(int count, const int *n, const int *p, const long long *lds, const int *mode, const double *src,
-                         int all_feature_rows, double *Cr, double *Ct, double *nrm, double *D) {
-    SHARP_API_BEGIN
-    ctx();
-    const std::string w = "sharp_row_prep_batch";
-    SHARP_REQUIRE(count >= 1, w + ": count must be at least 1");
-    SHARP_REQUIRE(n && p && lds && mode && src && Cr && Ct && nrm && D, w + ": null argument");
+}
+
+namespace {
+
+void row_prep_batch_entry(const std::string &w, int count, const int *n, const int *p, const long long *lds, const int *mode, const double *src,
+                          int all_feature_rows, double *Cr, double *Ct, double *nrm, double *D) {
     std::vector<size_t> oS(count + 1, 0), oCr(count + 1, 0), oCt(count + 1, 0), oN(count + 1, 0), oD(count + 1, 0);
     int max_n = 0, max_p = 0;
     for (int t = 0; t < count; ++t) {
@@ -605,22 +606,48 @@
     SHARP_REQUIRE(oS[count] + oCr[count] + oCt[count] + oD[count] <= (size_t(1) << 31), w + ": more than 16 GB of inputs and results");
     DevBuf<double> dS(oS[count]), dCr, dCt, dN, dD;
     dS.upload(src, oS[count]);
-    alloc_sentinel(dCr, oCr[count]);
+    if (Cr) alloc_sentinel(dCr, oCr[count]);
     alloc_sentinel(dCt, oCt[count]);
     alloc_sentinel(dN, oN[count]);
     alloc_sentinel(dD, oD[count]);
     std::vector<RowPrepTask> tasks(count);
     for (int t = 0; t < count; ++t)
         tasks[t] = RowPrepTask{dS.p + oS[t], lds[t], n[t], p[t], static_cast<int>(rup_ll(n[t], 128)), static_cast<int>(rup_ll(p[t], 16)), mode[t],
-                               dCr.p + oCr[t], dCt.p + oCt[t], dN.p + oN[t], dD.p + oD[t]};
+                               Cr ? dCr.p + oCr[t] : nullptr, dCt.p + oCt[t], dN.p + oN[t], dD.p + oD[t]};
     DevBuf<RowPrepTask> dt(count);
     dt.upload(tasks.data(), count);
     row_prep_batched(dt.p, count, max_n, max_p, all_feature_rows != 0);
-    dCr.download(Cr, oCr[count]);
+    if (Cr) dCr.download(Cr, oCr[count]);
     dCt.download(Ct, oCt[count]);
     dN.download(nrm, oN[count]);
     dD.download(D, oD[count]);
+    stream_sync();
+}
+
+}
+
+extern "C" {
+
+int sharp_row_prep_batch(int count, const int *n, const int *p, const long long *lds, const int *mode, const double *src,
+                         int all_feature_rows, double *Cr, double *Ct, double *nrm, double *D) {
+    SHARP_API_BEGIN
+    ctx();
+    const std::string w = "sharp_row_prep_batch";
+    SHARP_REQUIRE(count >= 1, w + ": count must be at least 1");
+    SHARP_REQUIRE(n && p && lds && mode && src && Cr && Ct && nrm && D, w + ": null argument");
+    row_prep_batch_entry(w, count, n, p, lds, mode, src, all_feature_rows, Cr, Ct, nrm, D);
     SHARP_API_END
 }
 
-}
+int sharp_row_prep_batch_nocr(int count, const int *n, const int *p, const long long *lds, const int *mode, const double *src, double *Ct,
+                              double *nrm, double *D) {
+    SHARP_API_BEGIN
+    ctx();
+    const std::string w = "sharp_row_prep_batch_nocr";
+    SHARP_REQUIRE(count >= 1, w + ": count must be at least 1");
+    SHARP_REQUIRE(n && p && lds && mode && src && Ct && nrm && D, w + ": null argument");
+    row_prep_batch_entry(w, count, n, p, lds, mode, src, 1, nullptr, Ct, nrm, D);
+    SHARP_API_END
+}
+
+}
diff --git a/sharp_amd/csrc/linalg.hpp b/sharp_amd/csrc/linalg.hpp
--- a/sharp_amd/csrc/linalg.hpp
+++ b/sharp_amd/csrc/linalg.hpp
@@ -19,6 +19,8 @@
 void gemm_tn_f64_batched(const GemmTask *d_tasks, int count, int max_M, int max_N, const char *timer_name, bool fast = false,
                          bool symmetric = false);
 
+constexpr int kRowPrepFusedMaxP = 512;
+inline bool row_prep_fused_path(int mode, int max_p) { return mode == 0 && max_p <= kRowPrepFusedMaxP; }
 struct RowPrepTask {
     const double *src;
     long long lds;
diff --git a/sharp_amd/csrc/projector.hpp b/sharp_amd/csrc/projector.hpp
--- a/sharp_amd/csrc/projector.hpp
+++ b/sharp_amd/csrc/projector.hpp
@@ -88,14 +88,15 @@
 
 constexpr int RP_FIX_BITS = 44;
 std::shared_ptr<Projector> build_projector(int m, int p, int K, const double *seeds, const std::function<void()> *after_draw = nullptr);
+struct RpMeanOut { double *viE = nullptr; bool written = false; };
 void project_dev(const Projector &pr, XRef dX, int m, int n, long long ld, int log_flag, double *dE, long long ldE,
-                 const int *d_row_map, unsigned ahead_token = 0);
+                 const int *d_row_map, unsigned ahead_token = 0, RpMeanOut *mean = nullptr);
 unsigned rp_compact_ahead(XRef dX, int m, int n, long long ld, int log_flag);
 void rp_compact_ahead_drop();
 void rp_trim();
 bool rp_pc_eligible(XRef X, int m, long long ld);
 void project_dev_pc(const Projector &pr, const ProjectorGroup &g, XRef dX, int m, int n, long long ld, int log_flag, int fix_bits,
-                    double *dE, long long ldE, const int *d_row_map);
+                    double *dE, long long ldE, const int *d_row_map, double *d_mean = nullptr);
 void rp_pc_trim();
 void project_dev_dense(const Projector &pr, XRef dX, int m, int n, long long ld, int log_flag, double *dE, long long ldE,
                        const int *d_row_map);
diff --git a/sharp_amd/csrc/rp.hip b/sharp_amd/csrc/rp.hip
--- a/sharp_amd/csrc/rp.hip
+++ b/sharp_amd/csrc/rp.hip
@@ -1,3 +1,4 @@
+#include "meta.hpp"
 #include "projector.hpp"
 #include "upload.hpp"
 
@@ -282,8 +283,9 @@
 #endif
 
 void project_dev(const Projector &pr, XRef X, int m, int n, long long ld, int log_flag, double *dE, long long ldE,
-                 const int *d_row_map, unsigned ahead_token) {
+                 const int *d_row_map, unsigned ahead_token, RpMeanOut *mean) {
     struct DropAhead { ~DropAhead() { rp_compact_ahead_drop(); } } drop_ahead;
+    if (mean) mean->written = false;
     const float *dX = X.f32();
     SHARP_REQUIRE(m == pr.m, "project: gene count differs from the projector's");
     SHARP_REQUIRE(ld >= m, "project: leading dimension smaller than m");
@@ -313,7 +315,9 @@
     else launch_rp<GWV, SL, false>(g, pr, dX, m, n, ld, log_flag, fix_bits, dE, ldE, d_row_map)
         const bool fused = knobs().rp_kernel == 1;
         if (rp_pc_eligible(X, m, ld)) {
-            project_dev_pc(pr, g, X, m, n, ld, log_flag, fix_bits, dE, ldE, d_row_map);
+            const bool with_mean = mean && mean->viE && knobs().rp_mean && pr.groups.size() == 1 && g.k0 == 0 && g.ncomp == pr.K * pr.p;
+            project_dev_pc(pr, g, X, m, n, ld, log_flag, fix_bits, dE, ldE, d_row_map, with_mean ? mean->viE : nullptr);
+            if (with_mean) mean->written = true;
             continue;
         }
 #ifdef SHARP_LAB
@@ -408,6 +412,35 @@
     SHARP_API_END
 }
 
+int sharp_project_mean(int proj, const double *X, int m, int n, long long ld, int log_flag, const int *row_map, double *E, double *viE,
+                       int *fused) {
+    SHARP_API_BEGIN
+    auto pr = get_projector(proj);
+    SHARP_REQUIRE(X && E && viE && fused, "sharp_project_mean: null buffer");
+    SHARP_REQUIRE(ld >= m && n >= 1, "sharp_project_mean: ld < m or no cell");
+    if (row_map) {
+        std::vector<char> seen(n, 0);
+        for (int i = 0; i < n; ++i) {
+            SHARP_REQUIRE(row_map[i] >= 0 && row_map[i] < n && !seen[row_map[i]], "sharp_project_mean: row_map is not a permutation of 0 .. n - 1");
+            seen[row_map[i]] = 1;
+        }
+    }
+    HostBlock hb;
+    upload_block(X, m, n, ld, hb);
+    const long long ldE = static_cast<long long>(pr->K) * pr->p;
+    DevBuf<double> dE(static_cast<size_t>(ldE) * n), dV(static_cast<size_t>(pr->p) * n);
+    DevBuf<int> dmap;
+    if (row_map) { dmap.alloc(n); dmap.upload(row_map, n); }
+    RpMeanOut mo;
+    mo.viE = dV.p;
+    project_dev(*pr, hb.ref(), m, n, hb.ld, log_flag, dE.p, ldE, row_map ? dmap.p : nullptr, 0, &mo);
+    if (!mo.written) ensemble_mean_dev(dE.p, ldE, n, pr->p, pr->K, dV.p);
+    *fused = mo.written ? 1 : 0;
+    dE.download(E, static_cast<size_t>(ldE) * n);
+    dV.download(viE, static_cast<size_t>(pr->p) * n);
+    SHARP_API_END
+}
+
 int sharp_synth_fill_dev(unsigned seed, int m, long long cell0, int ncell, int G, int nmark, float *dX, long long ld) {
     SHARP_API_BEGIN
     SHARP_REQUIRE(G >= 1 && G <= 64 && nmark >= 1 && ld >= m, "sharp_synth_fill_dev: bad arguments");
diff --git a/sharp_amd/csrc/rp3.hip b/sharp_amd/csrc/rp3.hip
--- a/sharp_amd/csrc/rp3.hip
+++ b/sharp_amd/csrc/rp3.hip
@@ -52,6 +52,8 @@
     int cap;
     uint32_t *sw;
     long long *st;
+    double *mean;
+    int K, pdim;
 };
 
 typedef uint32_t pc_u4 __attribute__((ext_vector_type(4)));
@@ -119,10 +121,26 @@
         if (it >= 0 && wave >= NP) {
             const long long row = static_cast<long long>(static_cast<int>(ctl[2]));
             double *erow = P.E + row * P.ldE + P.comp0;
-            for (int c = tid - NP * 64; c < P.ncomp; c += PC_THREADS - NP * 64) {
-                long long a = static_cast<long long>(atomicExch(&acc[c], 0ull));
-                if constexpr (DUAL) a -= static_cast<long long>(atomicExch(&acc[P.neg_base + c], 0ull));
-                __builtin_nontemporal_store(P.out_scale * (P.val * (static_cast<double>(a) * P.inv_fix)), &erow[c]);
+            if (P.mean) {
+                double *mrow = P.mean + row * P.pdim;
+                for (int j = tid - NP * 64; j < P.pdim; j += PC_THREADS - NP * 64) {
+                    double s = 0.0;
+                    for (int k = 0; k < P.K; ++k) {
+                        const int c = k * P.pdim + j;
+                        long long a = static_cast<long long>(atomicExch(&acc[c], 0ull));
+                        if constexpr (DUAL) a -= static_cast<long long>(atomicExch(&acc[P.neg_base + c], 0ull));
+                        const double v = P.out_scale * (P.val * (static_cast<double>(a) * P.inv_fix));
+                        __builtin_nontemporal_store(v, &erow[c]);
+                        s += v;
+                    }
+                    __builtin_nontemporal_store(s / P.K, &mrow[j]);
+                }
+            } else {
+                for (int c = tid - NP * 64; c < P.ncomp; c += PC_THREADS - NP * 64) {
+                    long long a = static_cast<long long>(atomicExch(&acc[c], 0ull));
+                    if constexpr (DUAL) a -= static_cast<long long>(atomicExch(&acc[P.neg_base + c], 0ull));
+                    __builtin_nontemporal_store(P.out_scale * (P.val * (static_cast<double>(a) * P.inv_fix)), &erow[c]);
+                }
             }
             if (tid == NP * 64) ctl[it & 1] = 0u;
         }
@@ -462,9 +480,10 @@
 }
 
 void project_dev_pc(const Projector &pr, const ProjectorGroup &g, XRef dX, int m, int n, long long ld, int log_flag, int fix_bits,
-                    double *dE, long long ldE, const int *d_row_map) {
+                    double *dE, long long ldE, const int *d_row_map, double *d_mean) {
     Ctx &c = ctx();
     PcWs &W = pws();
+    SHARP_REQUIRE(!d_mean || (g.k0 == 0 && g.ncomp == pr.K * pr.p), "rp_pc_kernel: the ensemble mean needs all K projectors in one group");
     const double fix_scale = std::ldexp(1.0, fix_bits), inv_fix = std::ldexp(1.0, -fix_bits);
     if (W.fixtab.n == 0 || W.fixtab_key != fix_scale || W.fixtab_mode != log_flag) {
         W.fixtab.ensure(PC_TAB);
@@ -479,6 +498,7 @@
     P.inv_fix = inv_fix; P.val = pr.val; P.out_scale = 1.0 / std::sqrt(static_cast<double>(pr.p));
     P.E = dE; P.ldE = ldE; P.comp0 = g.k0 * pr.p; P.row_map = d_row_map;
     P.lcap = 0; P.cap = 0; P.sw = nullptr; P.st = nullptr;
+    P.mean = d_mean; P.K = pr.K; P.pdim = pr.p;
     KernelTimer t("rp_stage");
     KernelTimer t2("rp_pc");
     const int mode = g.neg_base > 0 ? 1 : 0;
diff --git a/sharp_amd/csrc/runtime.hip b/sharp_amd/csrc/runtime.hip
--- a/sharp_amd/csrc/runtime.hip
+++ b/sharp_amd/csrc/runtime.hip
@@ -315,6 +315,8 @@
     v.hc_finish_at = num("SHARP_HC_FINISH_AT", 15);
     v.hc_nn_gemm = num("SHARP_HC_NN_GEMM", 1) != 0;
     v.stats_lane = num("SHARP_STATS_LANE", 1) != 0;
+    v.sums_ct = num("SHARP_SUMS_CT", 1) != 0;
+    v.rp_mean = num("SHARP_RP_MEAN", 1) != 0;
     v.ml_min_levels = num("SHARP_ML_MIN_LEVELS", 0);
     v.proj_host = num("SHARP_PROJ_HOST", 0) == 1;
     v.rp_pc_wgs = std::max(1, num("SHARP_RP_PC_WGS", 2));
```

After: 3.296 million, median of 4. 1.05x the previous value.
